# control-toolbox/CTDirect.jl

Measured on AMD Instinct MI355X. Metric: NLP callback evals/s (constraints+sparse Jac), N-step Goddard, 1/2/4/8 GPU, higher is better.
Workload: dtype f64; 1 GPU; cfg2_weak: goddard / gauss_legendre_2, 10000 time steps per GPU (global grid 10000 steps, time-step sharded); fused cons!+jac_coord! on HBM-resident x; BASELINE.json configs[1] per GPU; nvar_per_gpu=110004, ncon_per_gpu=90004, nnzj_per_gpu=1110028

## Files before the change

### ctdirect.jl_amd/csrc/ctd_engine.hip

```cpp
#include <hip/hip_runtime.h>
#include <hip/hiprtc.h>
#include <dlfcn.h>

#include <cstdio>
#include <functional>
#include <map>
#include <mutex>
#include <cstdlib>
#include <cstring>
#include <memory>
#include <new>
#include <string>
#include <vector>

#include "../../include/ctdirect_hip.h"
#include "ctd_host.hpp"
#include "ctd_kernels.hpp"
#include "ctd_hess_kernels.hpp"
#include "ctd_hess_step.hpp"
#include "ctd_iter_kernels.hpp"
#include "ctd_prod_kernels.hpp"
#include "ctd_hprod_kernels.hpp"
#include "ctd_kkt_kernels.hpp"
#include "ctd_jit.hpp"

using namespace ctd;

namespace ctd {
#define CTD_EXTERN_ALL(ID, P) \
    CTD_EXTERN_LAUNCHERS(P) CTD_EXTERN_HESS(P) CTD_EXTERN_HESS_STEP(P) CTD_EXTERN_ITER(P) CTD_EXTERN_PROD(P) CTD_EXTERN_HPROD(P) CTD_EXTERN_KKT(P)
CTD_REGISTRY(CTD_EXTERN_ALL)
}

template <class T = double> struct DevBuf {
    T* p = nullptr;
    int64_t cap = 0;
    DevBuf() = default;
    DevBuf(const DevBuf&) = delete;
    DevBuf& operator=(const DevBuf&) = delete;
    ~DevBuf() { release(); }
    void release() { if (p) (void)hipFree(p); p = nullptr; cap = 0; }
    hipError_t ensure(int64_t n) {
        if (p && n <= cap) return hipSuccess;
        release();
        const hipError_t e = hipMalloc((void**)&p, sizeof(T) * (size_t)(n > 1 ? n : 1));
        if (e == hipSuccess) cap = n; else p = nullptr;
        return e;
    }
    int32_t grow(ctd_handle* h, int64_t need, const char* fn);
};

enum JitFamily { JIT_FIRST, JIT_BATCH, JIT_PROD, JIT_HPROD, JIT_HESS, JIT_PROD_SHARD, JIT_HPROD_SHARD, JIT_KKT, kJitFamilies };
struct JitModule {
    hipModule_t mod = nullptr;
    hipFunction_t f[5] = {};
};

struct ctd_handle {
    Model model;
    int device = -1;
    hipStream_t stream = nullptr;
    bool own_stream = false;
    int64_t step_begin = 0, step_end = 0;
    int tile = 0, block = 256;
    KParams kp;
    size_t lds_bytes = 0;
    int grid = 0;
    DevBuf<double> d_tau;
    DevBuf<uint32_t> d_tmpl, d_vtmpl;
    DevBuf<uint16_t> d_pos;
    DevBuf<int64_t> d_edge_idx;
    DevBuf<uint32_t> d_edge_code;
    DevBuf<> d_x, d_c, d_vals;
    DevBuf<> d_partial;
    DevBuf<> d_obj;
    DevBuf<> d_g;
    DevBuf<> d_gpartial;
    int obj_blocks = 0;
    hipEvent_t ev0 = nullptr, ev1 = nullptr;
    const RtOcp* rt = nullptr;
    JitModule jit[kJitFamilies];
    bool hess_ready = false;
    HParams hp;
    int hess_tile = 0;
    size_t hess_lds_bytes = 0;
    DevBuf<uint32_t> d_htptr, d_hterms, d_hvptr, d_hvterms, d_heptr, d_hevptr, d_heterms;
    DevBuf<int64_t> d_hedge_idx;
    DevBuf<double> d_hpair_c;
    DevBuf<uint32_t> d_hcpos, d_hzpos;
    DevBuf<int32_t> d_hssrc, d_hschunk;
    DevBuf<double> d_hsck;
    bool hess_step = false;
    SParams sp{};
    HParams hp_step{};
    size_t hess_step_lds = 0;
    DevBuf<uint32_t> d_htasks, d_hptasks, d_hbtasks;
    DevBuf<> d_hpartials, d_y, d_hvals;
    DevBuf<XHalo> d_halo;
    XHalo halo_host{};
    DevBuf<> d_stitch_send, d_stitch_recv;
    int64_t hpart_member = 0;
    double out_mb = 0.0;
    DevBuf<> d_ppartial, d_pdir, d_pout;
    DevBuf<> d_hppartial;
    DevBuf<> d_kktpartial, d_kdy, d_ksx, d_ksc, d_krc;
    std::string err;
};

constexpr double kWtMB = 64.0;
constexpr double kHessWtMB = 16.0;

static thread_local std::string g_create_err;

static int32_t fail(ctd_handle* h, int32_t code, const std::string& msg) {
    if (h) h->err = msg; else g_create_err = msg;
    return code;
}

#define HIP_TRY(h, expr)                                                                          \
    do {                                                                                          \
        hipError_t e_ = (expr);                                                                   \
        if (e_ != hipSuccess)                                                                     \
            return fail(h, CTD_EHIP, std::string(#expr) + ": " + hipGetErrorString(e_));          \
    } while (0)

struct DeviceGuard {
    int prev = -1;
    bool switched = false;
    hipError_t err = hipSuccess;
    DeviceGuard() = default;
    explicit DeviceGuard(int dev) { (void)bind(dev); }
    hipError_t bind(int dev) {
        err = hipGetDevice(&prev);
        if (err == hipSuccess && prev != dev) { err = hipSetDevice(dev); switched = (err == hipSuccess); }
        return err;
    }
    ~DeviceGuard() { if (switched) (void)hipSetDevice(prev); }
    DeviceGuard(const DeviceGuard&) = delete;
    DeviceGuard& operator=(const DeviceGuard&) = delete;
};

struct OnDevice {
    DeviceGuard dg;
    int32_t st = CTD_OK;
    explicit OnDevice(ctd_handle* h, const char* fn = nullptr) {
        if (!h) st = CTD_EINVAL;
        else if (h->device < 0)
            st = fail(h, CTD_ENODEVICE, std::string(fn ? fn : "") + (fn ? ": " : "") +
                                            "compute call on a host-only handle (device = -1); there is no CPU fallback");
        else if (dg.bind(h->device) != hipSuccess) st = fail(h, CTD_EHIP, std::string("dg_.err: ") + hipGetErrorString(dg.err));
    }
};

template <class T> int32_t DevBuf<T>::grow(ctd_handle* h, int64_t need, const char* fn) {
    if (need <= cap && p) return CTD_OK;
    hipStreamCaptureStatus cs = hipStreamCaptureStatusNone;
    if (hipStreamIsCapturing(h->stream, &cs) == hipSuccess && cs != hipStreamCaptureStatusNone)
        return fail(h, CTD_EINVAL, std::string(fn) + ": this batch needs larger partial-sum buffers, which cannot be allocated while the "
                                   "stream is capturing; make one call with the same batch size before the capture");
    (void)hipGetLastError();
    HIP_TRY(h, hipStreamSynchronize(h->stream));
    HIP_TRY(h, ensure(need));
    return CTD_OK;
}

template <class T> static hipError_t upload(DevBuf<T>& dst, const std::vector<T>& src) {
    dst.release();
    if (src.empty()) return hipSuccess;
    const hipError_t e = dst.ensure((int64_t)src.size());
    if (e != hipSuccess) return e;
    return hipMemcpy(dst.p, src.data(), src.size() * sizeof(T), hipMemcpyHostToDevice);
}

static int env_int(const char* name, int dflt) {
    const char* s = std::getenv(name);
    return (s && *s) ? std::atoi(s) : dflt;
}

static void destroy_handle(ctd_handle* h) {
    DeviceGuard dg;
    if (h->device >= 0) {
        (void)dg.bind(h->device);
        (void)hipStreamSynchronize(h->stream);
        if (h->ev0) (void)hipEventDestroy(h->ev0);
        if (h->ev1) (void)hipEventDestroy(h->ev1);
        if (h->own_stream && h->stream) (void)hipStreamDestroy(h->stream);
        for (JitModule& m : h->jit)
            if (m.mod) (void)hipModuleUnload(m.mod);
    }
    delete h;
}

namespace {
std::string jit_include_dir() {
    const char* env = std::getenv("CTD_JIT_INCLUDE");
    if (env && *env) return env;
    Dl_info info;
    if (dladdr((const void*)&destroy_handle, &info) && info.dli_fname) {
        std::string path(info.dli_fname);
        const size_t slash = path.find_last_of('/');
        return (slash == std::string::npos ? std::string(".") : path.substr(0, slash)) + "/csrc";
    }
    return "csrc";
}

std::mutex g_jit_mu;
std::map<std::string, std::pair<std::string, std::vector<std::string>>> g_jit_cache;

int32_t jit_compile(const RtOcp& ro, const char* header, const std::vector<std::string>& exprs, const char* fp_contract,
                    std::string& code, std::vector<std::string>& lowered, std::string& err) {
    std::string key = ro.name + "|" + std::to_string((size_t)&ro) + "|" + header;
    for (const std::string& e : exprs) key += "|" + e;
    std::vector<std::string> extra;
    if (const char* ex = std::getenv("CTD_JIT_EXTRA")) {
        std::string cur;
        for (const char* c = ex;; ++c) {
            if (*c == ' ' || *c == 0) { if (!cur.empty()) extra.push_back(cur); cur.clear(); if (*c == 0) break; }
// ... 40 lines not shown
    (void)hiprtcDestroyProgram(&prog);
    std::lock_guard<std::mutex> lk(g_jit_mu);
    g_jit_cache[key] = {code, lowered};
    return CTD_OK;
}

std::vector<std::string> jit_first_exprs(int sc, int s) {
    const std::string P = "ctd::UserOCP", a = std::to_string(sc), b = std::to_string((sc == SC_IRK || sc == SC_MIDPOINT) && s > 0 ? s : 1);
    return {"ctd::cons_jac_kernel<" + P + ", " + a + ", " + b + ", false>", "ctd::obj_partial_kernel<" + P + ", " + a + ">",
            "ctd::obj_finish_kernel<" + P + ">", "ctd::grad_units_kernel<" + P + ", " + a + ", " + b + ">",
            "ctd::grad_finish_kernel<" + P + ">"};
}
std::vector<std::string> jit_hess_exprs(int sc, int s) {
    const std::string P = "ctd::UserOCP", a = std::to_string(sc), b = std::to_string((sc == SC_IRK || sc == SC_MIDPOINT) && s > 0 ? s : 1);
    return {"ctd::hess_kernel<" + P + ", " + a + ", " + b + ", false>", "ctd::hess_finish_kernel<" + P + ">"};
}
std::vector<std::string> jit_batch_exprs(int sc, int s) {
    const std::string b = std::to_string((sc == SC_IRK || sc == SC_MIDPOINT) && s > 0 ? s : 1);
    return {"ctd::cons_jac_batch_kernel<ctd::UserOCP, " + std::to_string(sc) + ", " + b + ">"};
}
std::vector<std::string> prod_exprs(int sc, int s, const std::string& sh) {
    const std::string a = std::to_string(sc), b = std::to_string(sc == SC_IRK && s > 0 ? s : 1);
    return {"ctd::jprod_kernel<ctd::UserOCP, " + a + ", " + b + sh + ">", "ctd::jtprod_units_kernel<ctd::UserOCP, " + a + ", " + b + sh + ">",
            "ctd::jtprod_finish_kernel<ctd::UserOCP" + sh + ">"};
}
std::vector<std::string> hprod_exprs(int sc, int s, const std::string& sh) {
    const std::string a = std::to_string(sc), b = std::to_string(sc == SC_IRK && s > 0 ? s : 1);
    return {"ctd::hprod_units_kernel<ctd::UserOCP, " + a + ", " + b + sh + ">", "ctd::hprod_finish_kernel<ctd::UserOCP" + sh + ">"};
}
std::vector<std::string> jit_kkt_exprs(int sc, int s) {
    const std::string a = std::to_string(sc), b = std::to_string(sc == SC_IRK && s > 0 ? s : 1);
    return {"ctd::kktprod_units_kernel<ctd::UserOCP, " + a + ", " + b + ">", "ctd::kktprod_finish_kernel<ctd::UserOCP>"};
}
std::vector<std::string> jit_prod_exprs(int sc, int s) { return prod_exprs(sc, s, ""); }
std::vector<std::string> jit_hprod_exprs(int sc, int s) { return hprod_exprs(sc, s, ""); }
std::vector<std::string> jit_prod_shard_exprs(int sc, int s) { return prod_exprs(sc, s, ", true"); }
std::vector<std::string> jit_hprod_shard_exprs(int sc, int s) { return hprod_exprs(sc, s, ", true"); }

const struct { const char* header; const char* fp_contract; std::vector<std::string> (*exprs)(int sc, int s); } kJit[kJitFamilies] = {
    {"ctd_kernels.hpp", "off", jit_first_exprs},
    {"ctd_kernels.hpp", "off", jit_batch_exprs},
    {"ctd_prod_kernels.hpp", "off", jit_prod_exprs},
    {"ctd_hprod_kernels.hpp", "off", jit_hprod_exprs},
    {"ctd_hess_kernels.hpp", "fast", jit_hess_exprs},
    {"ctd_prod_kernels.hpp", "off", jit_prod_shard_exprs},
    {"ctd_hprod_kernels.hpp", "off", jit_hprod_shard_exprs},
    {"ctd_kkt_kernels.hpp", "off", jit_kkt_exprs},
};

hipError_t jit_launch(hipFunction_t f, int grid, int block, size_t lds, hipStream_t st, void** args, hipEvent_t e0 = nullptr,
                      hipEvent_t e1 = nullptr, int batch = 1) {
    if (e0 || e1)
        return hipExtModuleLaunchKernel(f, (uint32_t)grid * (uint32_t)block, (uint32_t)batch, 1, (uint32_t)block, 1, 1, lds, st, args, nullptr, e0, e1, 0);
    return hipModuleLaunchKernel(f, (uint32_t)grid, (uint32_t)batch, 1, (uint32_t)block, 1, 1, (uint32_t)lds, st, args, nullptr);
}
}

static int32_t jit_load(ctd_handle* h, JitFamily fam) {
    JitModule& m = h->jit[fam];
    if (!h->rt || m.mod) return CTD_OK;
    ctd_handle* eh = fam == JIT_FIRST ? nullptr : h;
    const Layout& L = h->model.L;
    std::string code, err;
    std::vector<std::string> names;
    const int32_t st = jit_compile(*h->rt, kJit[fam].header, kJit[fam].exprs(L.sc, L.sc == SC_MIDPOINT ? L.cs : L.s), kJit[fam].fp_contract,
                                   code, names, err);
    if (st) return fail(eh, st, err);
    hipError_t e = hipModuleLoadData(&m.mod, code.data());
    for (size_t i = 0; e == hipSuccess && i < names.size(); ++i) e = hipModuleGetFunction(&m.f[i], m.mod, names[i].c_str());
    if (e == hipSuccess) return CTD_OK;
    if (m.mod) (void)hipModuleUnload(m.mod);
    m = JitModule{};
    return fail(eh, CTD_EHIP, std::string(kJit[fam].header) + " module: " + hipGetErrorString(e));
}

template <class T> struct Staged { T* host; DevBuf<>& buf; int64_t n; };

template <class Enqueue>
static int32_t host_call(ctd_handle* h, std::initializer_list<Staged<const double>> in, Enqueue&& enqueue,
                         std::initializer_list<Staged<double>> out) {
    for (const auto& a : in) if (a.host) HIP_TRY(h, a.buf.ensure(a.n));
    for (const auto& a : out) if (a.host) HIP_TRY(h, a.buf.ensure(a.n));
    for (const auto& a : in) if (a.host) HIP_TRY(h, hipMemcpyAsync(a.buf.p, a.host, sizeof(double) * a.n, hipMemcpyHostToDevice, h->stream));
    if (const int32_t st = enqueue()) return st;
    for (const auto& a : out) if (a.host) HIP_TRY(h, hipMemcpyAsync(a.host, a.buf.p, sizeof(double) * a.n, hipMemcpyDeviceToHost, h->stream));
    HIP_TRY(h, hipStreamSynchronize(h->stream));
    return CTD_OK;
}

template <class K>
static int32_t enqueue_prod_units(ctd_handle* h, const char* fn, typename K::Params& a, int dirs, int jc, DevBuf<>& partial,
                                  const JitModule& jm, int f0, const double* x_dev, bool shard) {
    ProdParams& pp = K::prod(a);
    pp.nch = (int32_t)((dirs + jc - 1) / jc);
    const int64_t blocks = ((pp.unit_end - pp.unit_begin) * (int64_t)pp.nch + 255) / 256;
    if (blocks > 0x7fffffff) return fail(h, CTD_EINVAL, std::string(fn) + ": grid too large");
    pp.nblocks = (int32_t)blocks;
    const int32_t st = partial.grow(h, blocks * kMaxNV, fn);
    if (st) return st;
    pp.partial = partial.p;
    hipError_t e = hipErrorInvalidValue;
    if (h->rt) {
        void* args[] = {&a, &x_dev};
        e = jit_launch(jm.f[f0], (int)blocks, 256, 0, h->stream, args);
        if (e == hipSuccess) e = jit_launch(jm.f[f0 + 1], 1, 64, 0, h->stream, args);
    }
    for_problem(h->model.problem, [&](auto tag) {
        using P = typename decltype(tag)::type;
        if constexpr (K::kShardForm)
            e = shard ? launch_prod_units<P, K, true>(a, x_dev, h->stream) : launch_prod_units<P, K, false>(a, x_dev, h->stream);
        else e = launch_prod_units<P, K, false>(a, x_dev, h->stream);
    });
    if (e != hipSuccess) return fail(h, CTD_EHIP, std::string(fn) + ": kernel launch: " + hipGetErrorString(e));
    return CTD_OK;
}

extern "C" {

const char* ctd_strerror(int32_t st) {
    switch (st) {
        case CTD_OK: return "ok";
        case CTD_EINVAL: return "invalid argument";
        case CTD_EGRID: return "given time grid is not strictly increasing";
        case CTD_ESCHEME: return "unknown discretization method";
        case CTD_EPATTERN: return "sparsity pattern not available";
        case CTD_EPROBLEM: return "problem not in the compiled registry";
        case CTD_ENODEVICE: return "no HIP device bound to this handle (there is no CPU fallback)";
        case CTD_EHIP: return "HIP runtime error";
        case CTD_ENOMEM: return "out of memory";
        default: return "unknown status";
    }
}

const char* ctd_last_error(const ctd_handle* h) { return h ? h->err.c_str() : g_create_err.c_str(); }

int32_t ctd_create(const ctd_desc* desc, ctd_handle** out) {
    if (!desc || !out) return fail(nullptr, CTD_EINVAL, "ctd_create: null argument");
    *out = nullptr;
    struct Del { void operator()(ctd_handle* p) const { if (p) destroy_handle(p); } };
    std::unique_ptr<ctd_handle, Del> h(new (std::nothrow) ctd_handle());
    if (!h) return fail(nullptr, CTD_ENOMEM, "ctd_create: out of memory");
    HostDesc hd{desc->problem, desc->scheme, desc->pattern_mode, desc->grid_size, desc->time_grid, desc->time_grid_len,
                desc->control_steps > 1 ? desc->control_steps : 1, desc->value_order};
    if (desc->reserved0 != 0) return fail(nullptr, CTD_EINVAL, "ctd_create: ctd_desc.reserved0 must be 0 (zero-initialise the descriptor: memset / ctd_desc d = {0})");
    std::string err;
    int st;
    try {
        st = build_model(hd, h->model, err);
    } catch (const std::bad_alloc&) {
        return fail(nullptr, CTD_ENOMEM, "ctd_create: out of memory while building the model");
    }
    if (st) return fail(nullptr, st, err);
    const Model& mo = h->model;
    if (mo.L.cs > 3 && desc->device >= 0 && !runtime_ocp(mo.problem))
        return fail(nullptr, CTD_EINVAL, "ctd_create: control_steps > 3 needs an OCP registered at run time (ctd_register_ocp); the compiled registry holds the midpoint kernels for 1, 2 and 3 controls per step");
    h->step_begin = desc->step_begin;
    h->step_end = desc->step_end;
    if (h->step_begin == 0 && h->step_end == 0) h->step_end = mo.L.N;
    if (h->step_begin < 0 || h->step_end > mo.L.N || h->step_begin >= h->step_end)
        return fail(nullptr, CTD_EINVAL, "ctd_create: shard [step_begin, step_end) is not inside [0, N)");
    h->tile = env_int("CTD_TILE", 0);
    if (h->tile <= 0) h->tile = default_tile(mo, h->step_end - h->step_begin);
    int maxb = 256;
    for_problem(mo.problem, [&](auto tag) { maxb = decltype(tag)::type::MAXB; });
    h->rt = runtime_ocp(mo.problem);
    if (h->rt) maxb = h->rt->maxb;
    h->block = env_int("CTD_BLOCK", 0);
    if (h->block <= 0) {
        h->block = 256;
        const int64_t ntl = (h->step_end - h->step_begin + h->tile - 1) / h->tile;
        if (ntl <= 512 && mo.nch_dyn <= 1 && mo.Lseg > 0 && 320 / mo.Lseg > 256 / mo.Lseg && mo.Lseg * (320 / mo.Lseg) * 10 >= 320 * 9) h->block = 320;
    }
    if (h->block < 64 || (h->block % 64)) h->block = 256;
    if (h->block > maxb) h->block = maxb;
    mo.fill_kparams(h->kp, h->step_begin, h->step_end, h->tile);
    h->lds_bytes = (size_t)lds_doubles(h->kp) * sizeof(double);
    const int debug_stop = env_int("CTD_DEBUG_STOP", 0);
    const size_t lds_cap = h->rt ? 64 * 1024 : 80 * 1024;
    while (h->lds_bytes > lds_cap && h->tile > 1) {
        h->tile = (h->tile + 1) / 2;
        mo.fill_kparams(h->kp, h->step_begin, h->step_end, h->tile);
        h->lds_bytes = (size_t)lds_doubles(h->kp) * sizeof(double);
    }
    const bool long_mid = mo.L.sc == SC_MIDPOINT && mo.L.cs == 1;
    if (desc->device >= 0 && !h->rt && env_int("CTD_TILE", 0) <= 0 && mo.nch_dyn <= 1 && (mo.L.sc == SC_IRK || long_mid) && h->tile >= 16) {
        DeviceGuard dgq(desc->device);
        if (dgq.err == hipSuccess) {
            auto resident = [&](int tile, size_t& lds) {
                KParams kq;
                mo.fill_kparams(kq, h->step_begin, h->step_end, tile);
                lds = (size_t)lds_doubles(kq) * sizeof(double);
                int r = 0;
                for_problem(mo.problem, [&](auto tag) { r = occupancy_cons_jac<typename decltype(tag)::type>(kq, h->block, lds); });
                (void)hipGetLastError();
                return r;
            };
            size_t l0 = 0;
            const int r0 = resident(h->tile, l0);
            const int64_t ns = h->step_end - h->step_begin, cap = 256 * (int64_t)r0;
            if (r0 > 0 && (ns + h->tile - 1) / h->tile >= env_int("CTD_LONG_GRID_ROUNDS", 8) * cap && maxb >= 512 && env_int("CTD_BLOCK", 0) <= 0 &&
                env_int("CTD_LONG_GRID", 1)) {
                int tbest = h->tile;
                for (int tt = h->tile + 1; tt <= 256; ++tt) {
                    KParams kq;
                    mo.fill_kparams(kq, h->step_begin, h->step_end, tt);
                    if ((size_t)lds_doubles(kq) * sizeof(double) > (long_mid ? 74u : 64u) * 1024) break;
                    tbest = tt;
                }
                if (tbest > h->tile) {
                    h->tile = tbest;
                    h->block = 512;
                    mo.fill_kparams(h->kp, h->step_begin, h->step_end, h->tile);
                    h->lds_bytes = (size_t)lds_doubles(h->kp) * sizeof(double);
                }
            } else if (mo.L.sc == SC_IRK && r0 > 0 && (ns + h->tile - 1) / h->tile > cap) {
                int tmax = 48;
                for (; tmax > h->tile; --tmax) { size_t l = 0; if (resident(tmax, l) >= r0 && l <= lds_cap) break; }
                const int64_t rounds = (ns + (int64_t)tmax * cap - 1) / ((int64_t)tmax * cap);
                const int64_t tb = (ns + rounds * cap - 1) / (rounds * cap);
                if (tb > h->tile && tb <= tmax) {
                    h->tile = (int)tb;
                    mo.fill_kparams(h->kp, h->step_begin, h->step_end, h->tile);
                    h->lds_bytes = (size_t)lds_doubles(h->kp) * sizeof(double);
                }
            }
        }
    }
    h->grid = h->kp.ntiles + h->kp.has_edge;
    h->kp.debug_stop = debug_stop;
    h->out_mb = 8.0 * ((double)(h->step_end - h->step_begin) * (mo.L.cb + mo.Lseg + (double)mo.L.nv * mo.vr)) / 1.0e6;
    h->kp.wt_store = h->out_mb <= kWtMB ? 1 : 0;
    h->device = desc->device;
    if (h->device >= 0) {
        int ndev = 0;
        if (hipGetDeviceCount(&ndev) != hipSuccess || h->device >= ndev)
            return fail(nullptr, CTD_ENODEVICE, "ctd_create: HIP device not available");
        ctd_handle* hp = h.get();
        if (h->lds_bytes > 160 * 1024) return fail(nullptr, CTD_EINVAL, "ctd_create: tile does not fit the 160 KiB LDS");
        DeviceGuard dg_(hp->device); HIP_TRY(nullptr, dg_.err);
        if (desc->stream_mode == CTD_STREAM_GIVEN) { hp->stream = (hipStream_t)desc->stream; hp->own_stream = false; }
        else { HIP_TRY(nullptr, hipStreamCreateWithFlags(&hp->stream, hipStreamNonBlocking)); hp->own_stream = true; }
        HIP_TRY(nullptr, upload(hp->d_tau, mo.tau));
        HIP_TRY(nullptr, upload(hp->d_tmpl, mo.tmpl));
        HIP_TRY(nullptr, upload(hp->d_vtmpl, mo.vtmpl));
        HIP_TRY(nullptr, upload(hp->d_edge_idx, mo.edge_idx));
        HIP_TRY(nullptr, upload(hp->d_edge_code, mo.edge_code));
        hp->kp.tau = hp->d_tau.p;
        hp->kp.tmpl = hp->d_tmpl.p;
        hp->kp.vtmpl = hp->d_vtmpl.p;
        {
            const int S = mo.L.s, r_dyn = S * mo.nch_dyn, r_path = mo.nch_path;
            int lgT = 0;
            while ((1 << lgT) < hp->tile) ++lgT;
            const int leadbase = (((r_dyn + r_path) << lgT) + 63) & ~63;
            const int early_lanes = mo.n_early + mo.c_early + mo.L.nv * mo.vr_early;
            if (env_int("CTD_EARLY", 0) && mo.n_early > 0 && !hp->rt && mo.fused && hp->tile <= 32 && leadbase + 64 <= hp->block && early_lanes <= 64 &&
                mo.n_late > 0 && mo.n_late <= hp->block) {
                HIP_TRY(nullptr, upload(hp->d_pos, mo.pos_order));
                hp->kp.pos = hp->d_pos.p;
                hp->kp.n_late = mo.n_late; hp->kp.n_early = mo.n_early; hp->kp.c_early = mo.c_early; hp->kp.vr_early = mo.vr_early;
                hp->kp.div_late = make_fastdiv((uint32_t)mo.n_late);
            }
        }
        hp->kp.edge_idx = hp->d_edge_idx.p;
        hp->kp.edge_code = hp->d_edge_code.p;
        hp->obj_blocks = 256;
        HIP_TRY(nullptr, hp->d_partial.ensure(hp->obj_blocks));
        HIP_TRY(nullptr, hp->d_obj.ensure(1));
        HIP_TRY(nullptr, hipEventCreate(&hp->ev0));
        HIP_TRY(nullptr, hipEventCreate(&hp->ev1));
        if (hp->rt) {
            if (hp->lds_bytes > 64 * 1024) return fail(nullptr, CTD_EINVAL, "ctd_create: one step of this run-time OCP does not fit 64 KiB of LDS");
            const int32_t jst = jit_load(hp, JIT_FIRST);
            if (jst) return jst;
        }
        {
            const bool direct = mo.fused && mo.L.sc != SC_TRAPEZE;
            const int mt = env_int("CTD_MULTI_TILE", 0);
            if (!direct && mt > 0 && kMultiTileLoop && !hp->rt) {
                int per_cu = mt > 1 ? mt : 0, cus = 256;
                if (hipDeviceGetAttribute(&cus, hipDeviceAttributeMultiprocessorCount, hp->device) != hipSuccess) cus = 256;
                if (per_cu == 0) {
                    if (hp->rt) {
                        if (hipModuleOccupancyMaxActiveBlocksPerMultiprocessor(&per_cu, hp->jit[JIT_FIRST].f[0], hp->block, hp->lds_bytes) != hipSuccess) per_cu = 0;
                    } else {
                        for_problem(mo.problem, [&](auto tag) {
                            using P = typename decltype(tag)::type;
                            per_cu = occupancy_cons_jac<P>(hp->kp, hp->block, hp->lds_bytes);
                        });
                    }
                }
                const int64_t cap = (int64_t)per_cu * cus - hp->kp.has_edge;
                if (cap > 0 && hp->kp.ntiles > cap) {
                    hp->kp.wg_stride = (int)cap;
                    hp->grid = hp->kp.wg_stride + hp->kp.has_edge;
                }
            }
        }
    }
    *out = h.release();
    return CTD_OK;
}

int32_t ctd_register_ocp(const ctd_ocp_def* def, int32_t* problem_id) {
    if (!def || !problem_id) return fail(nullptr, CTD_EINVAL, "ctd_register_ocp: null argument");
    std::string err;
    int id = -1;
    const int st = register_runtime_ocp(def, &id, err);
    if (st) return fail(nullptr, st, "ctd_register_ocp: " + err);
    *problem_id = id;
    return CTD_OK;
}

int32_t ctd_ocp_source(int32_t problem_id, char* buf, int64_t cap) {
// ... 236 lines not shown
}
}

int32_t ctd_shard_steps(int64_t N, int32_t n_shards, int32_t k, int64_t* begin, int64_t* end) {
    if (N < 1 || n_shards < 1 || n_shards > N || k < 0 || k >= n_shards || !begin || !end) return CTD_EINVAL;
    *begin = shard_begin(N, n_shards, k);
    *end = k + 1 == n_shards ? N : shard_begin(N, n_shards, k + 1);
    return CTD_OK;
}

int32_t ctd_stitch_c(ctd_handle* h, void* nccl_comm, int32_t n_ranks, int32_t rank, double* c_dev) {
    if (!h) return CTD_EINVAL;
    if (h->device < 0) return fail(h, CTD_ENODEVICE, "host-only handle");
    if (!nccl_comm || !c_dev || n_ranks < 1 || rank < 0 || rank >= n_ranks) return fail(h, CTD_EINVAL, "ctd_stitch_c: bad argument");
    const Layout& L = h->model.L;
    const int64_t N = L.N;
    const int G = n_ranks;
    if (G > N || h->step_begin != shard_begin(N, G, rank) || h->step_end != (rank + 1 == G ? N : shard_begin(N, G, rank + 1)))
        return fail(h, CTD_EINVAL, "ctd_stitch_c: the handle's shard is not block `rank` of the balanced split of the grid over n_ranks (ctd_shard_steps)");
    nccl_resolve();
    if (!g_nccl_allgather) return fail(h, CTD_ERCCL, "ctd_stitch_c: librccl (ncclAllGather) not found in this process; set CTD_RCCL_LIB");
    DeviceGuard dg_(h->device); HIP_TRY(h, dg_.err);
    const int64_t tail = L.ncon - N * L.cb;
    auto check = [&](int rc, const char* what) -> int32_t {
        if (rc == 0) return CTD_OK;
        return fail(h, CTD_ERCCL, std::string(what) + ": " + (g_nccl_errstr ? g_nccl_errstr(rc) : "RCCL error ") + " (" + std::to_string(rc) + ")");
    };
    constexpr int kNcclDouble = 8;
    if (N % G == 0 && tail == 0) {
        const int64_t S = (N / G) * L.cb;
        return check(g_nccl_allgather(c_dev + rank * S, c_dev, (size_t)S, kNcclDouble, nccl_comm, h->stream), "ncclAllGather");
    }
    const int64_t smax = ((N + G - 1) / G) * L.cb + tail;
    if (h->d_stitch_recv.cap < (int64_t)G * smax) {
        h->d_stitch_send.release();
        h->d_stitch_recv.release();
        HIP_TRY(h, h->d_stitch_send.ensure(smax));
        HIP_TRY(h, h->d_stitch_recv.ensure((int64_t)G * smax));
        HIP_TRY(h, hipMemsetAsync(h->d_stitch_send.p, 0, sizeof(double) * smax, h->stream));
    }
    const int64_t own = (h->step_end - h->step_begin) * L.cb, mytail = rank + 1 == G ? tail : 0;
    const int64_t np = own + mytail;
    stitch_pack_kernel<<<(unsigned)((np + 255) / 256), 256, 0, h->stream>>>(c_dev, h->d_stitch_send.p, h->step_begin * L.cb, own, N * L.cb, mytail);
    HIP_TRY(h, hipGetLastError());
    const int32_t st = check(g_nccl_allgather(h->d_stitch_send.p, h->d_stitch_recv.p, (size_t)smax, kNcclDouble, nccl_comm, h->stream), "ncclAllGather");
    if (st) return st;
    stitch_unpack_kernel<<<(unsigned)((L.ncon + 255) / 256), 256, 0, h->stream>>>(h->d_stitch_recv.p, c_dev, L.ncon, N, L.cb, G, smax);
    HIP_TRY(h, hipGetLastError());
    return CTD_OK;
}

int32_t ctd_ipc_export(int32_t device, const void* dev_ptr, void* handle64, int64_t* offset) {
    if (!dev_ptr || !handle64 || !offset) return CTD_EINVAL;
    static_assert(sizeof(hipIpcMemHandle_t) == 64, "CTD_IPC_HANDLE_BYTES");
    DeviceGuard dg(device);
    hipError_t e = dg.err;
    hipDeviceptr_t base = nullptr;
    size_t size = 0;
    if (e == hipSuccess) e = hipMemGetAddressRange(&base, &size, (hipDeviceptr_t)dev_ptr);
    hipIpcMemHandle_t hd;
    if (e == hipSuccess) e = hipIpcGetMemHandle(&hd, (void*)base);
    if (e != hipSuccess) { g_create_err = std::string("ctd_ipc_export: ") + hipGetErrorString(e); (void)hipGetLastError(); return CTD_EHIP; }
    std::memcpy(handle64, &hd, sizeof(hd));
    *offset = (int64_t)((const char*)dev_ptr - (const char*)base);
    return CTD_OK;
}
int32_t ctd_ipc_open(int32_t device, const void* handle64, void** base) {
    if (!handle64 || !base) return CTD_EINVAL;
    *base = nullptr;
    DeviceGuard dg(device);
    hipError_t e = dg.err;
    hipIpcMemHandle_t hd;
    std::memcpy(&hd, handle64, sizeof(hd));
    if (e == hipSuccess) e = hipIpcOpenMemHandle(base, hd, hipIpcMemLazyEnablePeerAccess);
    if (e != hipSuccess) { g_create_err = std::string("ctd_ipc_open: ") + hipGetErrorString(e); (void)hipGetLastError(); return CTD_ERCCL; }
    return CTD_OK;
}
int32_t ctd_ipc_probe(int32_t device, const void* ptr, size_t bytes) {
    if (!ptr || bytes == 0 || bytes > 64) return CTD_EINVAL;
    DeviceGuard dg(device);
    hipError_t e = dg.err;
    void* tmp = nullptr;
    if (e == hipSuccess) e = hipMalloc(&tmp, 64);
    if (e == hipSuccess) e = hipMemcpy(tmp, ptr, bytes, hipMemcpyDeviceToDevice);
    if (e == hipSuccess) e = hipDeviceSynchronize();
    if (tmp) (void)hipFree(tmp);
    if (e != hipSuccess) { g_create_err = std::string("ctd_ipc_probe: ") + hipGetErrorString(e); (void)hipGetLastError(); return CTD_ERCCL; }
    return CTD_OK;
}
int32_t ctd_ipc_close(int32_t device, void* base) {
    if (!base) return CTD_OK;
    DeviceGuard dg(device);
    return (dg.err == hipSuccess && hipIpcCloseMemHandle(base) == hipSuccess) ? CTD_OK : CTD_EHIP;
}

int32_t ctd_launch_info(const ctd_handle* h, int64_t* o) {
    if (!h || !o) return CTD_EINVAL;
    o[0] = h->grid; o[1] = h->block; o[2] = (int64_t)h->lds_bytes; o[3] = h->tile; o[4] = h->model.Lseg;
    o[5] = (int64_t)h->model.edge_idx.size();
    o[6] = (h->model.fused && h->model.L.sc != SC_TRAPEZE) ? 1 : 0;
    o[7] = 0;
    if (h->device >= 0) {
        DeviceGuard dg(h->device);
        int per_cu = 0;
        if (dg.err == hipSuccess) {
            if (h->rt) { if (hipModuleOccupancyMaxActiveBlocksPerMultiprocessor(&per_cu, h->jit[JIT_FIRST].f[0], h->block, h->lds_bytes) != hipSuccess) per_cu = 0; }
            else for_problem(h->model.problem, [&](auto tag) {
                using P = typename decltype(tag)::type;
                per_cu = occupancy_cons_jac<P>(h->kp, h->block, h->lds_bytes);
            });
        }
        (void)hipGetLastError();
        o[7] = per_cu;
    }
    return CTD_OK;
}


struct Batch {
    int32_t n;
    int64_t ldx, ldy, ldc, ldv, ldg, ldh;
};

static int32_t enqueue_cons_jac(ctd_handle* h, const double* x_dev, double* c_dev, double* vals_dev, hipEvent_t te0 = nullptr,
                                hipEvent_t te1 = nullptr, const Batch* bt = nullptr) {
    const OnDevice on(h);
    if (on.st) return on.st;
    if (!x_dev) return fail(h, CTD_EINVAL, "x is null");
    KParams kp = h->kp;
    kp.c = c_dev;
    kp.vals = vals_dev;
    hipError_t e = hipErrorInvalidValue;
    if (bt) {
        BatchLd bl{bt->ldx, bt->ldc, bt->ldv};
        kp.wt_store = h->out_mb * bt->n <= kWtMB ? 1 : 0;
        if (h->rt) {
            if (const int32_t jst = jit_load(h, JIT_BATCH)) return jst;
            void* args[] = {&kp, &x_dev, &bl};
            e = jit_launch(h->jit[JIT_BATCH].f[0], h->grid, h->block, h->lds_bytes, h->stream, args, nullptr, nullptr, bt->n);
        }
        for_problem(h->model.problem, [&](auto tag) {
            using P = typename decltype(tag)::type;
            e = launch_cons_jac_batch<P>(kp, x_dev, bl, h->grid, h->block, h->lds_bytes, h->stream, bt->n);
        });
        if (e != hipSuccess) return fail(h, CTD_EHIP, std::string("kernel launch: ") + hipGetErrorString(e));
        return CTD_OK;
    }
    if (h->rt) {
        void* args[] = {&kp, &x_dev};
        e = jit_launch(h->jit[JIT_FIRST].f[0], h->grid, h->block, h->lds_bytes, h->stream, args, te0, te1);
    }
    for_problem(h->model.problem, [&](auto tag) {
        using P = typename decltype(tag)::type;
        e = launch_cons_jac<P>(kp, x_dev, h->grid, h->block, h->lds_bytes, h->stream, te0, te1);
    });
    if (e != hipSuccess) return fail(h, CTD_EHIP, std::string("kernel launch: ") + hipGetErrorString(e));
    return CTD_OK;
}

int32_t ctd_cons_jac_dev_async(ctd_handle* h, const double* x_dev, double* c_dev, double* vals_dev) {
    return enqueue_cons_jac(h, x_dev, c_dev, vals_dev);
}

int32_t ctd_set_stream(ctd_handle* h, void* stream) {
    if (!h) return CTD_EINVAL;
    if (h->device < 0) return fail(h, CTD_ENODEVICE, "host-only handle");
    if (h->own_stream && h->stream) { (void)hipStreamSynchronize(h->stream); (void)hipStreamDestroy(h->stream); }
    h->stream = (hipStream_t)stream;
    h->own_stream = false;
    return CTD_OK;
}

int32_t ctd_sync(ctd_handle* h) {
    if (!h) return CTD_EINVAL;
    if (h->device < 0) return fail(h, CTD_ENODEVICE, "host-only handle");
    HIP_TRY(h, hipStreamSynchronize(h->stream));
    return CTD_OK;
}

int32_t ctd_cons_jac_dev(ctd_handle* h, const double* x_dev, double* c_dev, double* vals_dev) {
    int32_t st = enqueue_cons_jac(h, x_dev, c_dev, vals_dev);
    if (st) return st;
    return ctd_sync(h);
}

static int32_t host_cons_jac(ctd_handle* h, const double* x, double* c, double* vals) {
    const OnDevice on(h);
    if (on.st) return on.st;
    if (!x) return fail(h, CTD_EINVAL, "x is null");
    const Model& mo = h->model;
    return host_call(h, {{x, h->d_x, mo.L.nvar}},
                     [&] { return enqueue_cons_jac(h, h->d_x.p, c ? h->d_c.p : nullptr, vals ? h->d_vals.p : nullptr); },
                     {{c, h->d_c, mo.L.ncon}, {vals, h->d_vals, mo.nnzj}});
}

int32_t ctd_host_alloc(void** ptr, size_t bytes) {
    if (!ptr) return CTD_EINVAL;
    *ptr = nullptr;
    const hipError_t e = hipHostMalloc(ptr, bytes ? bytes : 8, hipHostMallocDefault);
    if (e != hipSuccess) { g_create_err = std::string("ctd_host_alloc: ") + hipGetErrorString(e); return CTD_EHIP; }
    return CTD_OK;
}
int32_t ctd_host_free(void* ptr) {
    if (!ptr) return CTD_OK;
    return hipHostFree(ptr) == hipSuccess ? CTD_OK : CTD_EHIP;
}

int32_t ctd_cons(ctd_handle* h, const double* x, double* c) {
    if (h && !c) return fail(h, CTD_EINVAL, "c is null");
    return host_cons_jac(h, x, c, nullptr);
}
int32_t ctd_jac_coord(ctd_handle* h, const double* x, double* vals) {
    if (h && !vals) return fail(h, CTD_EINVAL, "vals is null");
    return host_cons_jac(h, x, nullptr, vals);
}
int32_t ctd_cons_jac(ctd_handle* h, const double* x, double* c, double* vals) {
    if (h && (!c || !vals)) return fail(h, CTD_EINVAL, "c or vals is null");
    return host_cons_jac(h, x, c, vals);
}

static int fill_obj_params(ctd_handle* h, double* f_dev, ObjParams& op);

static int32_t enqueue_obj(ctd_handle* h, const double* x_dev, double* f_dev, const Batch* bt = nullptr) {
    const OnDevice on(h);
    if (on.st) return on.st;
    if (!x_dev || !f_dev) return fail(h, CTD_EINVAL, "null argument");
    const Layout& L = h->model.L;
    ObjParams op;
    const int blocks = fill_obj_params(h, f_dev, op);
    const bool lagrange = h->model.info.lagrange;
    const int nb = bt ? bt->n : 1;
    if (bt) {
        const int32_t st = h->d_partial.grow(h, (int64_t)nb * (blocks > 0 ? blocks : 1), "ctd_obj_batch_dev_async");
        if (st) return st;
        op.partial = h->d_partial.p;
        op.ldx = bt->ldx;
    }
    hipError_t e = hipErrorInvalidValue;
    if (h->rt) {
        void* args[] = {&op, &x_dev};
        e = lagrange ? jit_launch(h->jit[JIT_FIRST].f[1], blocks, 256, 0, h->stream, args, nullptr, nullptr, nb) : hipSuccess;
        if (e == hipSuccess) e = jit_launch(h->jit[JIT_FIRST].f[2], 1, 64, 0, h->stream, args, nullptr, nullptr, nb);
    }
    for_problem(h->model.problem, [&](auto tag) {
        using P = typename decltype(tag)::type;
        e = launch_obj<P>(op, x_dev, lagrange ? blocks : 0, 256, h->stream, nb);
    });
    if (e != hipSuccess) return fail(h, CTD_EHIP, std::string("kernel launch: ") + hipGetErrorString(e));
    return CTD_OK;
}

static int fill_obj_params(ctd_handle* h, double* f_dev, ObjParams& op) {
    const Layout& L = h->model.L;
    std::memset(&op, 0, sizeof(op));
    op.L = L;
    op.tau = h->d_tau.p;
    const bool last = h->step_end == L.N;
    op.unit_begin = h->step_begin;
    op.unit_end = (L.sc == SC_TRAPEZE && last) ? L.N + 1 : h->step_end;
    op.add_mayer = last ? 1 : 0;
    op.partial = h->d_partial.p;
    op.out = f_dev;
    op.halo = h->kp.halo;
    op.near = h->kp.near;
    const int64_t units = op.unit_end - op.unit_begin;
    int blocks = (int)((units + 255) / 256);
    if (blocks > h->obj_blocks) blocks = h->obj_blocks;
    if (blocks < 1) blocks = 1;
    const bool lagrange = h->model.info.lagrange;
    op.nblocks = lagrange ? blocks : 0;
    return lagrange ? blocks : 0;
}

int32_t ctd_obj_dev_async(ctd_handle* h, const double* x_dev, double* f_dev) { return enqueue_obj(h, x_dev, f_dev); }

int32_t ctd_obj_dev(ctd_handle* h, const double* x_dev, double* f_host) {
    if (h && !f_host) return fail(h, CTD_EINVAL, "null argument");
    const OnDevice on(h);
    if (on.st) return on.st;
    return host_call(h, {}, [&] { return enqueue_obj(h, x_dev, h->d_obj.p); }, {{f_host, h->d_obj, 1}});
}

static int32_t enqueue_grad(ctd_handle* h, const double* x_dev, double* g_dev, GradParams* only_params = nullptr, bool shard = false,
                            const Batch* bt = nullptr);
int32_t ctd_grad_dev_async(ctd_handle* h, const double* x_dev, double* g_dev) { return enqueue_grad(h, x_dev, g_dev); }
int32_t ctd_grad_shard_dev_async(ctd_handle* h, const double* x_dev, double* g_dev) { return enqueue_grad(h, x_dev, g_dev, nullptr, true); }
int32_t ctd_grad_dev(ctd_handle* h, const double* x_dev, double* g_dev) {
    int32_t st = enqueue_grad(h, x_dev, g_dev);
    if (st) return st;
    HIP_TRY(h, hipStreamSynchronize(h->stream));
    return CTD_OK;
}

__global__ void zero_rows_kernel(double* __restrict__ p, int64_t ld, int64_t len) {
    double* row = p + (int64_t)blockIdx.y * ld;
    for (int64_t e = (int64_t)blockIdx.x * blockDim.x + threadIdx.x; e < len; e += (int64_t)gridDim.x * blockDim.x) row[e] = 0.0;
}

static int32_t enqueue_grad(ctd_handle* h, const double* x_dev, double* g_dev, GradParams* only_params, bool shard, const Batch* bt) {
    const OnDevice on(h);
    if (on.st) return on.st;
    if (!x_dev || !g_dev) return fail(h, CTD_EINVAL, "null argument");
    const Layout& L = h->model.L;
    const bool last = h->step_end == L.N, first = h->step_begin == 0;
    const int64_t all_units = (L.sc == SC_IRK) ? L.N : L.N + 1;
    const int64_t ub = shard ? h->step_begin : 0, ue = shard ? ((L.sc != SC_IRK && last) ? L.N + 1 : h->step_end) : all_units;
    const int64_t units = ue - ub;
// ... 945 lines not shown
```

### ctdirect.jl_amd/csrc/ctd_kernel_body.hpp

```cpp
#pragma once
#include "ctd_layout.hpp"


namespace ctd {

#if defined(CTD_SUBSTAMPS) && defined(__HIP_DEVICE_COMPILE__)
#ifndef CTD_SUB_WAVE0
#define CTD_SUB_WAVE0 0
#endif
#define CTD_SUB(kp, id)                                                                                              \
    do {                                                                                                             \
        __builtin_amdgcn_sched_barrier(0);                                                                           \
        __builtin_amdgcn_s_waitcnt(0);                                                                               \
        if ((kp).stamps && (threadIdx.x & 63) == 0 && threadIdx.x >= 64 * CTD_SUB_WAVE0 && threadIdx.x < 64 * CTD_SUB_WAVE0 + 128) \
            (kp).stamps[(size_t)gridDim.x * 12 + ((size_t)blockIdx.x * 2 + (threadIdx.x >> 6) - CTD_SUB_WAVE0) * 8 + (id)] = clock64(); \
        __builtin_amdgcn_sched_barrier(0);                                                                           \
    } while (0)
#else
#define CTD_SUB(kp, id) do { } while (0)
#endif
#if defined(CTD_SUBSTAMPS_EMIT) && defined(__HIP_DEVICE_COMPILE__)
#define CTD_SUBE(kp, id)                                                                                             \
    do {                                                                                                             \
        __builtin_amdgcn_sched_barrier(0);                                                                           \
        if ((kp).stamps && (threadIdx.x & 63) == 0 && threadIdx.x < 128)                                             \
            (kp).stamps[(size_t)gridDim.x * 12 + ((size_t)blockIdx.x * 2 + (threadIdx.x >> 6)) * 8 + (id)] = clock64(); \
        __builtin_amdgcn_sched_barrier(0);                                                                           \
    } while (0)
#else
#define CTD_SUBE(kp, id) do { } while (0)
#endif

struct BlockCtx {
    int is_edge;
    int edge_part;
    int direct;
    int nslots;
    int in_stride;
    int64_t a, b;
    int64_t lo;
    double* in;
    double* v;
    double* tau;
    double* rec;
    const uint32_t* codes;
    const uint32_t* vcodes;
    const XHalo* halo;
    const double* xu;
};

CTD_HD const XHalo* block_halo(const KParams& kp, const BlockCtx& cx) {
    if (!kp.halo) return nullptr;
    if (cx.is_edge) return kp.halo;
    return (cx.lo < kp.step_begin || cx.b + kp.HH >= kp.step_end) ? kp.halo : nullptr;
}

constexpr int kMaxStagedCodes = 1024;
CTD_HD bool codes_staged(const KParams& kp) { return kp.stage_codes != 0; }
inline int wgs_per_cu(int64_t lds_bytes) {
    const int64_t g = (lds_bytes + 1279) / 1280 * 1280;
    return g > 0 ? (int)((160 * 1024) / g) : 32;
}
CTD_HD int code_doubles(const KParams& kp) { return codes_staged(kp) ? (kp.Lseg + kp.L.nv * kp.vr + 1) / 2 : 0; }

CTD_HD int64_t slot_index(const KParams& kp, const BlockCtx& cx, int k) {
    return cx.is_edge ? kp.edge_steps[k] : cx.lo + k;
}

CTD_HD BlockCtx make_ctx(const KParams& kp, int block, double* lds) {
    BlockCtx cx;
    cx.direct = 0;
    const Layout& L = kp.L;
    cx.codes = codes_staged(kp) ? reinterpret_cast<const uint32_t*>(lds) : kp.tmpl;
    cx.vcodes = codes_staged(kp) ? cx.codes + kp.Lseg : kp.vtmpl;
    lds += code_doubles(kp);
    cx.edge_part = 0;
    if (block < kp.has_edge) {
        cx.is_edge = 1;
        cx.edge_part = block;
        cx.nslots = kp.n_edge_slots;
        cx.in_stride = edge_in_stride(L);
        cx.a = cx.b = cx.lo = 0;
        cx.in = lds;
        cx.v = cx.in + cx.nslots * cx.in_stride;
        cx.tau = cx.v + kMaxNV;
        cx.rec = cx.tau + 2 * kMaxEdgeSlots + 2;
    } else {
        const int tile = block - kp.has_edge;
        const int cap = kp.T + kp.HL + kp.HH;
        cx.is_edge = 0;
        cx.a = kp.step_begin + (int64_t)tile * kp.T;
        cx.b = cx.a + kp.T < kp.step_end ? cx.a + kp.T : kp.step_end;
        cx.lo = cx.a - kp.HL;
        cx.nslots = (int)(cx.b - cx.a) + kp.HL + kp.HH;
        cx.in_stride = tile_in_stride(L);
        cx.in = lds;
        cx.v = cx.in + (cap + 1) * tile_in_stride(L) + L.n + L.m;
        cx.tau = cx.v + kMaxNV;
        cx.rec = cx.tau + cap + 2;
    }
    cx.xu = nullptr;
    cx.halo = block_halo(kp, cx);
    return cx;
}

CTD_HD BlockCtx make_direct_ctx(const KParams& kp, int block, double* lds, const double* xu) {
    BlockCtx cx;
    const Layout& L = kp.L;
    cx.direct = 1;
    cx.codes = kp.tmpl;
    cx.vcodes = kp.vtmpl;
    cx.in_stride = L.blk;
    cx.v = const_cast<double*>(xu) + L.v_off;
    cx.tau = nullptr;
    cx.rec = lds + code_doubles(kp);
    cx.xu = xu;
    cx.halo = nullptr;
    cx.edge_part = 0;
    if (block < kp.has_edge) {
        cx.is_edge = 1;
        cx.edge_part = block;
        cx.nslots = kp.n_edge_slots;
        cx.a = cx.b = cx.lo = 0;
        cx.in = const_cast<double*>(xu);
        cx.halo = kp.halo;
        return cx;
    }
    const int tile = block - kp.has_edge;
    cx.is_edge = 0;
    cx.a = kp.step_begin + (int64_t)tile * kp.T;
    cx.b = cx.a + kp.T < kp.step_end ? cx.a + kp.T : kp.step_end;
    cx.lo = cx.a - kp.HL;
    cx.nslots = (int)(cx.b - cx.a) + kp.HL + kp.HH;
    cx.in = const_cast<double*>(xu) + cx.lo * (int64_t)L.blk;
    cx.halo = block_halo(kp, cx);
    return cx;
}

CTD_HD const double* slot_base(const KParams& kp, const BlockCtx& cx, int k) {
    if (cx.direct && cx.halo) {
        const int64_t g = slot_index(kp, cx, k) * (int64_t)cx.in_stride;
        return xnear(kp.near, cx.xu, g) + g;
    }
    if (cx.direct && cx.is_edge) return cx.in + kp.edge_steps[k] * (int64_t)cx.in_stride;
    return cx.in + k * cx.in_stride;
}
CTD_HD const double* slot_next(const KParams& kp, const BlockCtx& cx, int k) {
    if (cx.direct && cx.halo) {
        const int64_t g = (slot_index(kp, cx, k) + 1) * (int64_t)cx.in_stride;
        return xnear(kp.near, cx.xu, g) + g;
    }
    return slot_base(kp, cx, k) + ((cx.direct || cx.is_edge) ? kp.L.blk : cx.in_stride);
}
CTD_HD const double* slot_prev(const KParams& kp, const BlockCtx& cx, int k) {
    if (cx.direct && cx.halo) {
        const int64_t g = (slot_index(kp, cx, k) - 1) * (int64_t)cx.in_stride;
        return xnear(kp.near, cx.xu, g) + g;
    }
    return slot_base(kp, cx, k) - ((cx.direct || cx.is_edge) ? kp.L.blk : cx.in_stride);
}

inline int64_t lds_doubles(const KParams& kp) {
    const Layout& L = kp.L;
    const int64_t cap = kp.T + kp.HL + kp.HH;
    int64_t tile = code_doubles(kp) + (cap + 1) * tile_in_stride(L) + L.n + L.m + kMaxNV + cap + 2 + cap * kp.R.stride;
    int64_t edge = code_doubles(kp) + (int64_t)kp.n_edge_slots * edge_in_stride(L) + kMaxNV + 2 * kMaxEdgeSlots + 2 +
                   (int64_t)(kp.n_edge_slots + 1) * kp.R.stride + kp.R.bsize;
    return tile > edge ? tile : edge;
}

CTD_HD double tau_global(const KParams& kp, int64_t i) {
    if (i < 0) i = 0;
    if (i > kp.L.N) i = kp.L.N;
    return kp.tau ? kp.tau[i] : (double)i / (double)kp.L.N;
}
CTD_HD double slot_tau(const KParams& kp, const BlockCtx& cx, int k, int d) {
    if (cx.direct) return tau_global(kp, slot_index(kp, cx, k) + d);
    return cx.is_edge ? cx.tau[2 * k + d] : cx.tau[k + d];
}
CTD_HD double final_tau(const KParams& kp, const BlockCtx& cx) {
    return cx.direct ? tau_global(kp, kp.L.N) : cx.tau[2 * cx.nslots];
}

template <class P> CTD_HD double time_of(const KParams& kp, const double* v, double tau) {
    const double t0 = (P::IT0 >= 0) ? v[P::IT0 >= 0 ? P::IT0 : 0] : kp.L.t0;
    const double tf = (P::ITF >= 0) ? v[P::ITF >= 0 ? P::ITF : 0] : kp.L.tf;
    return t0 + tau * (tf - t0);
}
template <class P> CTD_HD double dtime_of(double tau, int k) {
    const double dt0 = (P::IT0 == k) ? 1.0 : 0.0;
    const double dtf = (P::ITF == k) ? 1.0 : 0.0;
    return dt0 + tau * (dtf - dt0);
}

template <class P> struct DynNZ {
    static constexpr bool sparse = false;
    static constexpr int nF = -1, nG = -1;
    CTD_HD static constexpr int fx(int, int) { return -1; }
    CTD_HD static constexpr int gu(int, int) { return -1; }
};
template <class P, int SC, int S> struct RL {
    static constexpr int cb = (SC == SC_IRK ? P::NX * (1 + S) : P::NX) + P::NPATH;
    static constexpr RecLayout R = make_rec_layout(P::NX, P::NU, P::NV, P::NPATH, P::NBC, SC == SC_IRK ? S : 0, cb,
                                                   SC == SC_MIDPOINT ? P::NU * S : P::NU, DynNZ<P>::nF, DynNZ<P>::nG);
    CTD_HD static constexpr int F(int r, int c) {
        if (DynNZ<P>::sparse) { const int s = DynNZ<P>::fx(r, c); return s < 0 ? -1 : R.oF + s; }
        return R.oF + r * R.ldx + c;
    }
    CTD_HD static constexpr int G(int r, int c, int jb = 0) {
        if (DynNZ<P>::sparse) { const int s = DynNZ<P>::gu(r, c); return s < 0 ? -1 : R.oG + jb * DynNZ<P>::nG + s; }
        return R.oG + r * R.ldg + jb * P::NU + c;
    }
};
template <int SC, int S> struct StagePoints { static constexpr int value = SC == SC_IRK ? S : 1; };

template <class P> struct Dirs {
    static constexpr int DYN = P::NX + P::NU + (P::DYN_T ? 1 : 0) + (P::DYN_V ? P::NV : 0);
    static constexpr int PATH = P::NX + P::NU + (P::PATH_T ? 1 : 0) + (P::PATH_V ? P::NV : 0);
    static constexpr int BND = 2 * P::NX + P::NV;
    static constexpr int DC = P::DC;
    static constexpr int NCH_DYN = (DYN + DC - 1) / DC;
    static constexpr int NCH_PATH = (PATH + DC - 1) / DC;
    static constexpr int NCH_BND = (BND + DC - 1) / DC;
    static constexpr bool FUSED = (NCH_DYN == 1) && (P::NPATH == 0 || NCH_PATH == 1);
    static constexpr bool FREE = (P::IT0 >= 0) || (P::ITF >= 0);
};

template <class P, int SC> struct DirectTile { static constexpr bool value = Dirs<P>::FUSED && SC != SC_TRAPEZE; };

CTD_HD void load_codes(const KParams& kp, const BlockCtx& cx, int tid, int nthr) {
    if (!codes_staged(kp)) return;
    uint32_t* dst = const_cast<uint32_t*>(cx.codes);
    for (int e = tid; e < kp.Lseg; e += nthr) dst[e] = kp.tmpl[e];
    const int nvc = kp.L.nv * kp.vr;
    for (int e = tid; e < nvc; e += nthr) dst[kp.Lseg + e] = kp.vtmpl[e];
}

template <class P, int SC, int S, bool LOAD_V = true>
CTD_HD void phase_load(const KParams& kp, const BlockCtx& cx, const double* __restrict__ xu, int tid, int nthr) {
    const Layout& L = kp.L;
    if (cx.is_edge) {
        const int per = cx.in_stride;
        for (int e = tid; e < cx.nslots * per; e += nthr) {
            const int k = e / per, o = e - k * per;
            int64_t g = kp.edge_steps[k] * L.blk + o;
            if (o >= L.blk + L.n + L.m)
                g = (kp.edge_steps[k] >= 1 ? kp.edge_steps[k] - 1 : 0) * (int64_t)L.blk + L.n + (o - (L.blk + L.n + L.m));
            cx.in[e] = (g < L.v_off) ? (cx.halo ? xnear(kp.near, xu, g) : xu)[g] : 0.0;
        }
        for (int e = tid; e <= 2 * cx.nslots; e += nthr)
            cx.tau[e] = (e == 2 * cx.nslots) ? tau_global(kp, L.N) : tau_global(kp, kp.edge_steps[e >> 1] + (e & 1));
    } else {
        const int64_t g0 = (cx.lo < 0 ? 0 : cx.lo) * (int64_t)L.blk;
        int64_t g1 = (cx.lo + cx.nslots) * (int64_t)L.blk + L.n + L.m;
        if (g1 > L.v_off) g1 = L.v_off;
        const double* __restrict__ src = xu + g0;
        const int cnt = (int)(g1 - g0);
        const int eo0 = (int)(g0 - cx.lo * (int64_t)L.blk), padw = cx.in_stride - L.blk;
        auto at = [&](int e) -> double& { const int eo = eo0 + e; return cx.in[eo + (int)fast_div((uint32_t)eo, kp.div_blk) * padw]; };
        const bool codes = LOAD_V && codes_staged(kp);
        const int nvc = kp.L.nv * kp.vr;
        if (cx.halo) {
            for (int e = tid; e < cnt; e += nthr) at(e) = xnear(kp.near, xu, g0 + e)[g0 + e];
            if (LOAD_V && tid < kMaxNV) cx.v[tid] = (tid < P::NV) ? xu[L.v_off + tid] : 0.0;
            if (codes) {
                uint32_t* cd = const_cast<uint32_t*>(cx.codes);
                for (int e = tid; e < kp.Lseg; e += nthr) cd[e] = kp.tmpl[e];
                for (int e = tid; e < nvc; e += nthr) cd[kp.Lseg + e] = kp.vtmpl[e];
            }
            for (int e = tid; e <= cx.nslots + 1; e += nthr) cx.tau[e] = tau_global(kp, cx.lo + e);
            return;
        }
        const double x0 = tid < cnt ? src[tid] : 0.0;
        const double x1 = tid + nthr < cnt ? src[tid + nthr] : 0.0;
        const double vv = (LOAD_V && tid < P::NV) ? xu[L.v_off + tid] : 0.0;
        const uint32_t c0 = (codes && tid < kp.Lseg) ? kp.tmpl[tid] : 0u;
        const uint32_t c1 = (codes && tid < nvc) ? kp.vtmpl[tid] : 0u;
        const double tau_e = tid <= cx.nslots + 1 ? tau_global(kp, cx.lo + tid) : 0.0;
        if (tid < cnt) at(tid) = x0;
        if (tid + nthr < cnt) at(tid + nthr) = x1;
        if (LOAD_V && tid < kMaxNV) cx.v[tid] = vv;
        if (codes) {
            uint32_t* cd = const_cast<uint32_t*>(cx.codes);
            if (tid < kp.Lseg) cd[tid] = c0;
            if (tid < nvc) cd[kp.Lseg + tid] = c1;
            for (int e = tid + nthr; e < kp.Lseg; e += nthr) cd[e] = kp.tmpl[e];
            for (int e = tid + nthr; e < nvc; e += nthr) cd[kp.Lseg + e] = kp.vtmpl[e];
        }
        for (int e = tid + 2 * nthr; e < cnt; e += nthr) at(e) = src[e];
        if (tid <= cx.nslots + 1) cx.tau[tid] = tau_e;
        for (int e = tid + nthr; e <= cx.nslots + 1; e += nthr) cx.tau[e] = tau_global(kp, cx.lo + e);
        return;
    }
    if (LOAD_V && tid < kMaxNV) cx.v[tid] = (tid < P::NV) ? xu[L.v_off + tid] : 0.0;
}

struct TileIn { double x0, x1, tau; };
template <class P>
CTD_HD TileIn load_issue(const KParams& kp, const BlockCtx& cx, const double* __restrict__ xu, int tid, int nthr) {
    TileIn t{0.0, 0.0, 0.0};
    if (cx.halo) return t;
    const Layout& L = kp.L;
    const int64_t g0 = (cx.lo < 0 ? 0 : cx.lo) * (int64_t)L.blk;
    int64_t g1 = (cx.lo + cx.nslots) * (int64_t)L.blk + L.n + L.m;
    if (g1 > L.v_off) g1 = L.v_off;
    const double* __restrict__ src = xu + g0;
    const int cnt = (int)(g1 - g0);
    if (tid < cnt) t.x0 = src[tid];
    if (tid + nthr < cnt) t.x1 = src[tid + nthr];
    if (tid <= cx.nslots + 1) t.tau = tau_global(kp, cx.lo + tid);
    return t;
}
template <class P, int SC, int S>
CTD_HD void load_commit(const KParams& kp, const BlockCtx& cx, const double* __restrict__ xu, const TileIn& t, int tid, int nthr) {
    if (cx.halo) { phase_load<P, SC, S, false>(kp, cx, xu, tid, nthr); return; }
    const Layout& L = kp.L;
    const int64_t g0 = (cx.lo < 0 ? 0 : cx.lo) * (int64_t)L.blk;
    int64_t g1 = (cx.lo + cx.nslots) * (int64_t)L.blk + L.n + L.m;
    if (g1 > L.v_off) g1 = L.v_off;
    const double* __restrict__ src = xu + g0;
    const int cnt = (int)(g1 - g0);
    const int eo0 = (int)(g0 - cx.lo * (int64_t)L.blk), padw = cx.in_stride - L.blk;
    auto at = [&](int e) -> double& { const int eo = eo0 + e; return cx.in[eo + (int)fast_div((uint32_t)eo, kp.div_blk) * padw]; };
    if (tid < cnt) at(tid) = t.x0;
    if (tid + nthr < cnt) at(tid + nthr) = t.x1;
    for (int e = tid + 2 * nthr; e < cnt; e += nthr) at(e) = src[e];
    if (tid <= cx.nslots + 1) cx.tau[tid] = t.tau;
    for (int e = tid + nthr; e <= cx.nslots + 1; e += nthr) cx.tau[e] = tau_global(kp, cx.lo + e);
}

template <class P> CTD_HD void fill_const_coefs(const KParams& kp, double* C) {
#pragma unroll
    for (int e = 0; e < kNC; ++e) C[e] = 0.0;
    C[C_ONE] = 1.0; C[C_NEG1] = -1.0;
#pragma unroll
    for (int j = 0; j < 3; ++j) C[C_B + j] = kp.L.b[j];
}

template <class P, int SC, int S>
CTD_HD void fin_lead(const KParams& kp, const BlockCtx& cx, int k, int row = -1) {
    constexpr int n = P::NX, nv = P::NV;
    const Layout& L = kp.L;
    constexpr RecLayout R = RL<P, SC, S>::R;
    const int64_t i = slot_index(kp, cx, k);
    double* rec = cx.rec + k * R.stride;
    double* C = rec + R.oC;
    if (row <= 0) fill_const_coefs<P>(kp, C);
    if (i < 0 || i >= L.N) return;
    const double tau0 = slot_tau(kp, cx, k, 0), tau1 = slot_tau(kp, cx, k, 1);
    const double h = time_of<P>(kp, cx.v, tau1) - time_of<P>(kp, cx.v, tau0);
    if (SC == SC_IRK) {
        const double* base = slot_base(kp, cx, k);
        const double* nxt = slot_next(kp, cx, k);
        const double* K = base + n + L.cu;
        if (row <= 0) {
#pragma unroll
            for (int j = 0; j < S; ++j) {
#pragma unroll
                for (int l = 0; l < S; ++l) C[C_HA + 3 * j + l] = -(h * L.a[3 * j + l]);
                C[C_HB + j] = -(h * L.b[j]);
            }
        }
        if (row >= 0) {
            const int r = row;
            double sumbk = L.b[0] * K[r];
#pragma unroll
            for (int j = 1; j < S; ++j) sumbk = sumbk + L.b[j] * K[j * n + r];
            rec[R.oR + r] = nxt[r] - (base[r] + h * sumbk);
#pragma unroll
            for (int kk = 0; kk < nv; ++kk) {
                const double dh = Dirs<P>::FREE ? dtime_of<P>(tau1, kk) - dtime_of<P>(tau0, kk) : 0.0;
                rec[R.oSv + r * nv + kk] = -(dh * sumbk);
            }
            return;
        }
#pragma unroll
        for (int r = 0; r < n; ++r) {
            double sumbk = L.b[0] * K[r];
#pragma unroll
            for (int j = 1; j < S; ++j) sumbk = sumbk + L.b[j] * K[j * n + r];
            rec[R.oR + r] = nxt[r] - (base[r] + h * sumbk);
#pragma unroll
            for (int kk = 0; kk < nv; ++kk) {
                const double dh = Dirs<P>::FREE ? dtime_of<P>(tau1, kk) - dtime_of<P>(tau0, kk) : 0.0;
                rec[R.oSv + r * nv + kk] = -(dh * sumbk);
            }
        }
    } else if (SC == SC_MIDPOINT) {
        C[C_NHH] = -(0.5 * (h / (double)S));
        C[C_NH] = -(h / (double)S);
    } else {
        C[C_NHH] = -(0.5 * h);
    }
}

template <class P, int SC, int S>
CTD_HD void fin_stage(const KParams& kp, const BlockCtx& cx, int k, int j, double* ev, int r0 = 0, int rstep = 1) {
    constexpr int n = P::NX, nv = P::NV;
    auto mine = [&](int r) { return rstep == 1 || (r % rstep) == r0; };
    constexpr bool FREE = Dirs<P>::FREE;
    const Layout& L = kp.L;
    constexpr RecLayout R = RL<P, SC, S>::R;
    const int64_t i = slot_index(kp, cx, k);
    if (i < 0) return;
    if (SC == SC_TRAPEZE ? (i > L.N) : (i >= L.N)) return;
    double* rec = cx.rec + k * R.stride;
    const double* base = slot_base(kp, cx, k);
    const double tau0 = slot_tau(kp, cx, k, 0), tau1 = slot_tau(kp, cx, k, 1);
    double dti[nv > 0 ? nv : 1], dh[nv > 0 ? nv : 1];
#pragma unroll
    for (int kk = 0; kk < nv; ++kk) {
        dti[kk] = FREE ? dtime_of<P>(tau0, kk) : 0.0;
        dh[kk] = FREE ? dtime_of<P>(tau1, kk) - dti[kk] : 0.0;
    }
    if (SC == SC_IRK) {
        const double* K = base + n + L.cu;
#pragma unroll
        for (int r = 0; r < n; ++r)
            if (mine(r)) rec[R.oR + n + j * n + r] = K[j * n + r] - ev[R.of + r];
#pragma unroll
        for (int kk = 0; kk < nv; ++kk) {
            double dx[n > 0 ? n : 1];
#pragma unroll
            for (int c = 0; c < n; ++c) {
                double acc = 0.0;
#pragma unroll
                for (int l = 0; l < S; ++l) acc = acc + (dh[kk] * butcher_a<S>(L, j, l)) * K[l * n + c];
                dx[c] = acc;
            }
            const double dtij = dti[kk] + butcher_c<S>(L, j) * dh[kk];
#pragma unroll
            for (int r = 0; r < n; ++r) {
                if (!mine(r)) continue;
                double w = P::DYN_V ? ev[R.oW + r * nv + kk] : 0.0;
                if (P::DYN_T && FREE) w = w + ev[R.oft + r] * dtij;
                if (FREE) {
#pragma unroll
                    for (int c = 0; c < n; ++c)
                        if (RL<P, SC, S>::F(r, c) >= 0) w = w + ev[RL<P, SC, S>::F(r, c)] * dx[c];
                }
                ev[R.oW + r * nv + kk] = w;
            }
        }
    } else if (SC == SC_MIDPOINT) {
        const double h = (time_of<P>(kp, cx.v, tau1) - time_of<P>(kp, cx.v, tau0)) / (double)S;
        const double* nxt = slot_next(kp, cx, k);
#pragma unroll
        for (int r = 0; r < n; ++r) {
            if (!mine(r)) continue;
            const double f = ev[R.of + r];
            rec[R.oR + r] = nxt[r] - (base[r] + h * f);
#pragma unroll
            for (int kk = 0; kk < nv; ++kk) {
                double w = P::DYN_V ? ev[R.oW + r * nv + kk] : 0.0;
                if (P::DYN_T && FREE)
                    w = w + ev[R.oft + r] * (L.euler == 0 ? 0.5 * (dti[kk] + (dti[kk] + dh[kk])) : (L.euler == 1 ? dti[kk] : dti[kk] + dh[kk]));
                ev[R.oW + r * nv + kk] = w;
                rec[R.oSv + r * nv + kk] = -((S > 1 ? dh[kk] / (double)S : dh[kk]) * f + h * w);
            }
        }
    } else {
#pragma unroll
        for (int r = 0; r < n; ++r)
#pragma unroll
            for (int kk = 0; kk < nv; ++kk) {
                if (!mine(r)) continue;
                double w = P::DYN_V ? ev[R.oW + r * nv + kk] : 0.0;
                if (P::DYN_T && FREE) w = w + ev[R.oft + r] * dti[kk];
                ev[R.oW + r * nv + kk] = w;
            }
    }
}

template <class P, int S>
CTD_HD void fin_stage_row(const KParams& kp, const BlockCtx& cx, int k, int j, int r) {
    constexpr int n = P::NX, nv = P::NV;
    constexpr bool FREE = Dirs<P>::FREE;
    constexpr RecLayout R = RL<P, SC_IRK, S>::R;
    const Layout& L = kp.L;
    const int64_t i = slot_index(kp, cx, k);
    if (i < 0 || i >= L.N) return;
    double* rec = cx.rec + k * R.stride;
    double* ev = rec + R.oEval + j * R.eval_sz;
    const double* K = slot_base(kp, cx, k) + n + L.cu;
    const double tau0 = slot_tau(kp, cx, k, 0), tau1 = slot_tau(kp, cx, k, 1);
    rec[R.oR + n + j * n + r] = K[j * n + r] - ev[R.of + r];
#pragma unroll
    for (int kk = 0; kk < nv; ++kk) {
        const double dti = FREE ? dtime_of<P>(tau0, kk) : 0.0;
        const double dh = FREE ? dtime_of<P>(tau1, kk) - dti : 0.0;
        double w = P::DYN_V ? ev[R.oW + r * nv + kk] : 0.0;
        if (P::DYN_T && FREE) w = w + ev[R.oft + r] * (dti + butcher_c<S>(L, j) * dh);
        if (FREE) {
#pragma unroll
            for (int c = 0; c < n; ++c) {
                double acc = 0.0;
#pragma unroll
                for (int l = 0; l < S; ++l) acc = acc + (dh * butcher_a<S>(L, j, l)) * K[l * n + c];
                const int sl = RL<P, SC_IRK, S>::F(r, c);
                if (sl >= 0) w = w + ev[sl] * acc;
            }
        }
        ev[R.oW + r * nv + kk] = w;
    }
}

template <class P, int SC, int S>
CTD_HD void fin_path(const KParams& kp, double* rec, double tau) {
    constexpr int nv = P::NV, np = P::NPATH;
    constexpr RecLayout R = RL<P, SC, S>::R;
#pragma unroll
    for (int r = 0; r < np; ++r)
#pragma unroll
        for (int kk = 0; kk < nv; ++kk) {
            double pv = P::PATH_V ? rec[R.oPv + r * nv + kk] : 0.0;
            if (P::PATH_T && Dirs<P>::FREE) pv = pv + rec[R.oPt + r] * dtime_of<P>(tau, kk);
            rec[R.oPv + r * nv + kk] = pv;
        }
}

template <class P>
CTD_HD void fin_trapeze_step(const KParams& kp, const BlockCtx& cx, int k) {
    constexpr int n = P::NX, nv = P::NV;
    const Layout& L = kp.L;
    constexpr RecLayout R = RL<P, SC_TRAPEZE, 1>::R;
    const int64_t i = slot_index(kp, cx, k);
    if (i < 0 || i >= L.N || k + 1 >= cx.nslots) return;
    if (slot_index(kp, cx, k + 1) != i + 1) return;
    double* rec = cx.rec + k * R.stride;
    const double* nxt = rec + R.stride;
    const double* base = slot_base(kp, cx, k);
    const double* xnext = slot_next(kp, cx, k);
    const double tau0 = slot_tau(kp, cx, k, 0), tau1 = slot_tau(kp, cx, k, 1);
    const double half_h = 0.5 * (time_of<P>(kp, cx.v, tau1) - time_of<P>(kp, cx.v, tau0));
    const double* e0 = rec + R.oEval;
    const double* e1 = nxt + R.oEval;
#pragma unroll
    for (int r = 0; r < n; ++r) {
        const double fs = e0[R.of + r] + e1[R.of + r];
        rec[R.oR + r] = xnext[r] - (base[r] + half_h * fs);
#pragma unroll
        for (int kk = 0; kk < nv; ++kk) {
            const double dhalf = Dirs<P>::FREE ? 0.5 * (dtime_of<P>(tau1, kk) - dtime_of<P>(tau0, kk)) : 0.0;
            rec[R.oSv + r * nv + kk] = -(dhalf * fs + half_h * (e0[R.oW + r * nv + kk] + e1[R.oW + r * nv + kk]));
        }
    }
}

template <class P, int S> CTD_HD void node_control(const KParams& kp, const double* base, double* u) {
    const Layout& L = kp.L;
    if (L.stagewise) {
#pragma unroll
        for (int c = 0; c < P::NU; ++c) u[c] = L.b[0] * base[P::NX + c];
#pragma unroll
        for (int j = 1; j < S; ++j)
#pragma unroll
            for (int c = 0; c < P::NU; ++c) u[c] = u[c] + L.b[j] * base[P::NX + j * P::NU + c];
    } else {
#pragma unroll
        for (int c = 0; c < P::NU; ++c) u[c] = base[P::NX + c];
    }
}

template <class P, int S> CTD_HD void path_control(const KParams& kp, const BlockCtx& cx, int k, int64_t i, double* u) {
    const Layout& L = kp.L;
    const double* base = slot_base(kp, cx, k);
    if (L.euler == 2 && i >= 1 && (cx.is_edge || k >= 1)) {
        const double* up = (cx.is_edge && !cx.direct) ? base + L.blk + P::NX + P::NU : slot_prev(kp, cx, k) + P::NX;
#pragma unroll
        for (int c = 0; c < P::NU; ++c) u[c] = up[c];
    } else {
        node_control<P, S>(kp, base, u);
    }
}

template <class P> struct SymDyn {
    static constexpr bool value = P::HAS_SYM_DYN;
    static constexpr int parts = P::DYN_PARTS;
    CTD_HD static void eval(const double* p, double* ev) { if constexpr (P::HAS_SYM_DYN) P::dyn_sym(p, ev); }
    CTD_HD static void eval_part(int q, const double* p, double* ev) {
        if constexpr (P::HAS_SYM_DYN && P::DYN_PARTS > 1) P::dyn_sym_part(q, p, ev);
        else eval(p, ev);
    }
};
template <class P> struct SymPath {
    static constexpr bool value = P::HAS_SYM_PATH;
    CTD_HD static void eval(const double* p, double* px, double* val) { if constexpr (P::HAS_SYM_PATH) P::path_sym(p, px, val); }
};
template <class P> struct SymLag {
    static constexpr bool value = P::HAS_SYM_LAG;
    CTD_HD static void eval(const double* p, double* out) { if constexpr (P::HAS_SYM_LAG) P::lag_sym(p, out); }
};
template <class P> struct SymStage;
template <class P> struct SymPathH { static constexpr bool value = false; CTD_HD static void eval(const double*, double*) {} };

template <class P, class RLT, bool SPLIT>
CTD_HD void eval_point(const KParams& kp, const double* vv, int q, double t, const double* xv, const double* uv, double* ev) {
    constexpr int n = P::NX, m = P::NU, nv = P::NV, DC = P::DC;
    using D = Dual<DC>;
    constexpr RecLayout R = RLT::R;
    struct { const double* v; } cx{vv};
    if constexpr (SymDyn<P>::value) {
        constexpr bool split = SPLIT && SymDyn<P>::parts > 1 && SymDyn<P>::parts == Dirs<P>::NCH_DYN;
        if (!split && q != 0) return;
        CTD_SUB(kp, 6);
        double prm[1 + n + m + nv];
        prm[0] = t;
#pragma unroll
        for (int c = 0; c < n; ++c) prm[1 + c] = xv[c];
#pragma unroll
        for (int c = 0; c < m; ++c) prm[1 + n + c] = uv[c];
#pragma unroll
        for (int c = 0; c < nv; ++c) prm[1 + n + m + c] = cx.v[c];
        if constexpr (split) SymDyn<P>::eval_part(q, prm, ev);
        else SymDyn<P>::eval(prm, ev);
        return;
    }
    D X[n > 0 ? n : 1], U[m > 0 ? m : 1], V[nv > 0 ? nv : 1], Tt, out[n > 0 ? n : 1];
    const int g0 = q * DC;
    constexpr int gT = n + m, gV = n + m + (P::DYN_T ? 1 : 0);
#pragma unroll
    for (int c = 0; c < n; ++c) {
        X[c].v = xv[c];
#pragma unroll
        for (int d = 0; d < DC; ++d) X[c].d[d] = (g0 + d == c) ? 1.0 : 0.0;
    }
#pragma unroll
    for (int c = 0; c < m; ++c) {
        U[c].v = uv[c];
#pragma unroll
        for (int d = 0; d < DC; ++d) U[c].d[d] = (g0 + d == n + c) ? 1.0 : 0.0;
    }
    Tt.v = t;
#pragma unroll
    for (int d = 0; d < DC; ++d) Tt.d[d] = (P::DYN_T && g0 + d == gT) ? 1.0 : 0.0;
#pragma unroll
    for (int c = 0; c < nv; ++c) {
        V[c].v = cx.v[c];
#pragma unroll
        for (int d = 0; d < DC; ++d) V[c].d[d] = (P::DYN_V && g0 + d == gV + c) ? 1.0 : 0.0;
    }
    P::template dynamics<D>(out, Tt, X, U, V);
#pragma unroll
    for (int d = 0; d < DC; ++d) {
        const int g = g0 + d;
        if (g < n) {
#pragma unroll
            for (int r = 0; r < n; ++r) ev[R.oF + r * R.ldx + g] = out[r].d[d];
        } else if (g < n + m) {
#pragma unroll
            for (int r = 0; r < n; ++r) ev[R.oG + r * R.ldg + (g - n)] = out[r].d[d];
        } else if (P::DYN_T && g == n + m) {
#pragma unroll
            for (int r = 0; r < n; ++r) ev[R.oft + r] = out[r].d[d];
        } else if (P::DYN_V && g < Dirs<P>::DYN) {
            const int kk = g - n - m - (P::DYN_T ? 1 : 0);
#pragma unroll
            for (int r = 0; r < n; ++r) ev[R.oW + r * nv + kk] = out[r].d[d];
        }
    }
    if (q == 0) {
#pragma unroll
        for (int r = 0; r < n; ++r) ev[R.of + r] = out[r].v;
    }
}

template <class P, int SC, int S, bool SPLIT = false>
CTD_HD void eval_dynamics(const KParams& kp, const BlockCtx& cx, int k, int j, int q, double* ev) {
    constexpr int n = P::NX, m = P::NU, nv = P::NV;
    const Layout& L = kp.L;
    constexpr RecLayout R = RL<P, SC, S>::R;
    const int64_t i = slot_index(kp, cx, k);
    if (i < 0) return;
    if (SC == SC_TRAPEZE ? (i > L.N) : (i >= L.N)) return;
    const double* base = slot_base(kp, cx, k);
    const double ti = time_of<P>(kp, cx.v, slot_tau(kp, cx, k, 0));
    double xv[n > 0 ? n : 1], uv[m > 0 ? m : 1];
    double t;
    if (SC == SC_TRAPEZE) {
        t = ti;
#pragma unroll
        for (int c = 0; c < n; ++c) xv[c] = base[c];
#pragma unroll
        for (int c = 0; c < m; ++c) uv[c] = base[n + c];
    } else if (SC == SC_MIDPOINT) {
        const double tip1 = time_of<P>(kp, cx.v, slot_tau(kp, cx, k, 1));
        const double* nxt = slot_next(kp, cx, k);
        if (L.euler == 0) {
            t = 0.5 * (ti + tip1);
#pragma unroll
            for (int c = 0; c < n; ++c) xv[c] = 0.5 * (base[c] + nxt[c]);
        } else {
            t = (L.euler == 1) ? ti : tip1;
#pragma unroll
            for (int c = 0; c < n; ++c) xv[c] = (L.euler == 1) ? base[c] : nxt[c];
        }
#pragma unroll
        for (int c = 0; c < m; ++c) uv[c] = base[n + c];
    } else {
        const double h = time_of<P>(kp, cx.v, slot_tau(kp, cx, k, 1)) - ti;
        t = ti + butcher_c<S>(L, j) * h;
        const double* K = base + n + L.cu;
#pragma unroll
        for (int c = 0; c < n; ++c) {
            double x = base[c];
#pragma unroll
            for (int l = 0; l < S; ++l) x = x + h * butcher_a<S>(L, j, l) * K[l * n + c];
            xv[c] = x;
        }
        const double* U = base + n + (L.stagewise ? j * m : 0);
#pragma unroll
        for (int c = 0; c < m; ++c) uv[c] = U[c];
    }
    if constexpr (SC == SC_MIDPOINT && S > 1) {
        using RL1 = RL<P, SC_MIDPOINT, 1>;
        constexpr RecLayout R1 = RL1::R;
        constexpr int DC = P::DC, NP = Dirs<P>::NCH_DYN;
        constexpr bool sym = SymDyn<P>::value;
        constexpr bool symsplit = sym && SPLIT && SymDyn<P>::parts > 1 && SymDyn<P>::parts == NP;
        constexpr int gT = n + m, gV = n + m + (P::DYN_T ? 1 : 0);
        if (sym && !symsplit && q != 0) return;
        auto dir = [&](int g) { return sym || (g >= q * DC && g < (q + 1) * DC); };
        for (int jj = 0; jj < S; ++jj) {
            double tmp[R1.eval_sz];
#pragma unroll
            for (int e = 0; e < R1.eval_sz; ++e) tmp[e] = 0.0;
#pragma unroll
            for (int c = 0; c < m; ++c) uv[c] = base[n + jj * m + c];
            eval_point<P, RL1, SPLIT>(kp, cx.v, q, t, xv, uv, tmp);
#pragma unroll
            for (int r = 0; r < n; ++r) {
                if (symsplit && (r % NP) != q) continue;
#pragma unroll
                for (int c = 0; c < n; ++c)
                        if (dir(c) && RL1::F(r, c) >= 0)
                        ev[RL<P, SC, S>::F(r, c)] = (jj == 0 ? 0.0 : ev[RL<P, SC, S>::F(r, c)]) + tmp[RL1::F(r, c)];
#pragma unroll
                for (int c = 0; c < m; ++c)
                    if (dir(n + c) && RL1::G(r, c) >= 0) ev[RL<P, SC, S>::G(r, c, jj)] = tmp[RL1::G(r, c)];
                if (P::DYN_T && dir(gT)) ev[R.oft + r] = (jj == 0 ? 0.0 : ev[R.oft + r]) + tmp[R1.oft + r];
                if (P::DYN_V) {
#pragma unroll
                    for (int kk = 0; kk < nv; ++kk)
                        if (dir(gV + kk)) ev[R.oW + r * nv + kk] = (jj == 0 ? 0.0 : ev[R.oW + r * nv + kk]) + tmp[R1.oW + r * nv + kk];
                }
                if (sym || q == 0) ev[R.of + r] = (jj == 0 ? 0.0 : ev[R.of + r]) + tmp[R1.of + r];
            }
        }
        return;
    }
    eval_point<P, RL<P, SC, S>, SPLIT>(kp, cx.v, q, t, xv, uv, ev);
}

template <class P, int SC, int S>
CTD_HD void eval_path(const KParams& kp, double* rec, double t, const double* xv, const double* uv, const double* vv, int q,
                      int value_off) {
    constexpr int n = P::NX, m = P::NU, nv = P::NV, np = P::NPATH, DC = P::DC;
    using D = Dual<DC>;
    constexpr RecLayout R = RL<P, SC, S>::R;
    if constexpr (SymPath<P>::value) {
        if (q != 0) return;
        double prm[1 + n + m + nv];
        prm[0] = t;
#pragma unroll
        for (int c = 0; c < n; ++c) prm[1 + c] = xv[c];
#pragma unroll
        for (int c = 0; c < m; ++c) prm[1 + n + c] = uv[c];
#pragma unroll
        for (int c = 0; c < nv; ++c) prm[1 + n + m + c] = vv[c];
        SymPath<P>::eval(prm, rec + R.oPx, rec + value_off);
        return;
    }
    D X[n > 0 ? n : 1], U[m > 0 ? m : 1], V[nv > 0 ? nv : 1], Tt, out[np > 0 ? np : 1];
    const int g0 = q * DC;
    constexpr int gT = n + m, gV = n + m + (P::PATH_T ? 1 : 0);
#pragma unroll
    for (int c = 0; c < n; ++c) {
        X[c].v = xv[c];
#pragma unroll
        for (int d = 0; d < DC; ++d) X[c].d[d] = (g0 + d == c) ? 1.0 : 0.0;
    }
#pragma unroll
    for (int c = 0; c < m; ++c) {
        U[c].v = uv[c];
#pragma unroll
        for (int d = 0; d < DC; ++d) U[c].d[d] = (g0 + d == n + c) ? 1.0 : 0.0;
    }
    Tt.v = t;
#pragma unroll
    for (int d = 0; d < DC; ++d) Tt.d[d] = (P::PATH_T && g0 + d == gT) ? 1.0 : 0.0;
#pragma unroll
    for (int c = 0; c < nv; ++c) {
        V[c].v = vv[c];
#pragma unroll
        for (int d = 0; d < DC; ++d) V[c].d[d] = (P::PATH_V && g0 + d == gV + c) ? 1.0 : 0.0;
    }
    P::template path<D>(out, Tt, X, U, V);
#pragma unroll
    for (int d = 0; d < DC; ++d) {
        const int g = g0 + d;
        if (g < n) {
#pragma unroll
            for (int r = 0; r < np; ++r) rec[R.oPx + r * R.ldx + g] = out[r].d[d];
        } else if (g < n + m) {
#pragma unroll
            for (int r = 0; r < np; ++r) rec[R.oPu + r * R.ldu + (g - n)] = out[r].d[d];
        } else if (P::PATH_T && g == n + m) {
#pragma unroll
            for (int r = 0; r < np; ++r) rec[R.oPt + r] = out[r].d[d];
        } else if (P::PATH_V && g < Dirs<P>::PATH) {
            const int kk = g - n - m - (P::PATH_T ? 1 : 0);
#pragma unroll
            for (int r = 0; r < np; ++r) rec[R.oPv + r * nv + kk] = out[r].d[d];
        }
    }
    if (q == 0) {
#pragma unroll
        for (int r = 0; r < np; ++r) rec[value_off + r] = out[r].v;
    }
}

template <class P, int SC, int S, bool REG = false>
CTD_HD void eval_step_path(const KParams& kp, const BlockCtx& cx, int k, int q) {
    constexpr int n = P::NX, m = P::NU, np = P::NPATH;
    constexpr RecLayout R = RL<P, SC, S>::R;
    constexpr int eqs = RL<P, SC, S>::cb - P::NPATH;
    const Layout& L = kp.L;
    const int64_t i = slot_index(kp, cx, k);
    if (i < 0 || i >= L.N) return;
    const double* base = slot_base(kp, cx, k);
    double uv[m > 0 ? m : 1];
    path_control<P, S>(kp, cx, k, i, uv);
    double xv[n > 0 ? n : 1];
#pragma unroll
    for (int c = 0; c < n; ++c) xv[c] = base[c];
    double* rec = cx.rec + k * R.stride;
    const double tau = slot_tau(kp, cx, k, 0);
    if constexpr (REG) {
        double lrec[R.oR + eqs + (np > 0 ? np : 1)];
#pragma unroll
        for (int e = R.oPx; e < R.oR; ++e) lrec[e] = 0.0;
        eval_path<P, SC, S>(kp, lrec, time_of<P>(kp, cx.v, tau), xv, uv, cx.v, q, R.oR + eqs);
        if (Dirs<P>::FUSED) fin_path<P, SC, S>(kp, lrec, tau);
#pragma unroll
        for (int e = R.oPx; e < R.oR; ++e) rec[e] = lrec[e];
#pragma unroll
        for (int r = 0; r < np; ++r) rec[R.oR + eqs + r] = lrec[R.oR + eqs + r];
    } else {
        eval_path<P, SC, S>(kp, rec, time_of<P>(kp, cx.v, tau), xv, uv, cx.v, q, R.oR + L.eqs);
        if (Dirs<P>::FUSED) fin_path<P, SC, S>(kp, rec, tau);
    }
}

template <class P, int SC, int S>
CTD_HD void eval_final_path(const KParams& kp, const BlockCtx& cx, int q) {
    constexpr int n = P::NX, m = P::NU;
    constexpr RecLayout R = RL<P, SC, S>::R;
    const Layout& L = kp.L;
    const double* base = slot_base(kp, cx, kp.edge_slot_last);
    const double* nxt = slot_next(kp, cx, kp.edge_slot_last);
    double xv[n > 0 ? n : 1], uv[m > 0 ? m : 1];
#pragma unroll
    for (int c = 0; c < n; ++c) xv[c] = nxt[c];
    if (SC == SC_TRAPEZE) {
#pragma unroll
        for (int c = 0; c < m; ++c) uv[c] = nxt[n + c];
    } else node_control<P, S>(kp, base, uv);
    double* rec = cx.rec + kp.edge_fp * R.stride;
    const double tau = final_tau(kp, cx);
    eval_path<P, SC, S>(kp, rec, time_of<P>(kp, cx.v, tau), xv, uv, cx.v, q, R.oR);
    if (Dirs<P>::FUSED) fin_path<P, SC, S>(kp, rec, tau);
}

template <class P, int SC, int S>
CTD_HD void eval_boundary(const KParams& kp, const BlockCtx& cx, int q) {
    constexpr int n = P::NX, nv = P::NV, nb = P::NBC, DC = P::DC;
    using D = Dual<DC>;
    const Layout& L = kp.L;
    constexpr RecLayout R = RL<P, SC, S>::R;
    const double* b0 = slot_base(kp, cx, kp.edge_slot_first);
    const double* bf = slot_next(kp, cx, kp.edge_slot_last);
    D X0[n > 0 ? n : 1], XF[n > 0 ? n : 1], V[nv > 0 ? nv : 1], out[nb > 0 ? nb : 1];
    const int g0 = q * DC;
#pragma unroll
    for (int c = 0; c < n; ++c) {
        X0[c].v = b0[c];
        XF[c].v = bf[c];
#pragma unroll
        for (int d = 0; d < DC; ++d) {
            X0[c].d[d] = (g0 + d == c) ? 1.0 : 0.0;
            XF[c].d[d] = (g0 + d == n + c) ? 1.0 : 0.0;
        }
    }
#pragma unroll
    for (int c = 0; c < nv; ++c) {
        V[c].v = cx.v[c];
#pragma unroll
        for (int d = 0; d < DC; ++d) V[c].d[d] = (g0 + d == 2 * n + c) ? 1.0 : 0.0;
    }
    P::template boundary<D>(out, X0, XF, V);
    double* rec = cx.rec + kp.edge_b * R.stride;
#pragma unroll
    for (int d = 0; d < DC; ++d) {
        const int g = g0 + d;
        if (g < n) {
#pragma unroll
            for (int r = 0; r < nb; ++r) rec[R.oB0 + r * R.ldx + g] = out[r].d[d];
        } else if (g < 2 * n) {
#pragma unroll
            for (int r = 0; r < nb; ++r) rec[R.oBf + r * R.ldx + (g - n)] = out[r].d[d];
        } else if (g < 2 * n + nv) {
#pragma unroll
            for (int r = 0; r < nb; ++r) rec[R.oBv + r * nv + (g - 2 * n)] = out[r].d[d];
        }
    }
    if (q == 0) {
#pragma unroll
        for (int r = 0; r < nb; ++r) rec[R.oBval + r] = out[r].v;
    }
}

template <class P, int SC, int S = 1> struct RegEval {
    static constexpr bool value = DirectTile<P, SC>::value && (P::NX * (P::NX + P::NU * (SC == SC_MIDPOINT ? S : 1) + P::NV + 2) <= 64);
};

template <class P, int SC, int S>
CTD_HD bool fin_folded(const BlockCtx& cx) {
    constexpr bool path_ok = P::NPATH == 0 || SymPath<P>::value || Dirs<P>::NCH_PATH == 1;
    return !Dirs<P>::FUSED && SymDyn<P>::value && path_ok && !cx.is_edge;
}

constexpr int kSplitMinParts = 4;

template <class P, int SC, int S>
CTD_HD bool edge_sym_layout(const BlockCtx& cx, int nthr) {
    constexpr int r_path = (P::NPATH > 0) ? Dirs<P>::NCH_PATH : 0;
    constexpr int n_b = (P::NBC > 0) ? Dirs<P>::NCH_BND : 0;
    constexpr bool parts = SymDyn<P>::parts >= kSplitMinParts && SymDyn<P>::parts == Dirs<P>::NCH_DYN;
    return SymDyn<P>::value && !Dirs<P>::FUSED && cx.is_edge && cx.nslots <= 8 && nthr >= 256 && r_path <= 4 && n_b <= 32 &&
           StagePoints<SC, S>::value * 8 <= 32 && (!parts || Dirs<P>::NCH_DYN * 64 <= nthr);
}

template <class P, int SC, int S>
CTD_HD bool split_eval(const BlockCtx& cx, int nthr) {
    constexpr bool ok = SymDyn<P>::value && SymDyn<P>::parts >= kSplitMinParts && SymDyn<P>::parts == Dirs<P>::NCH_DYN && !Dirs<P>::FUSED;
    constexpr int NP = Dirs<P>::NCH_DYN;
    constexpr int r_path = (P::NPATH > 0) ? Dirs<P>::NCH_PATH : 0;
    return ok && !cx.is_edge && StagePoints<SC, S>::value * cx.nslots + ((P::NPATH > 0) ? cx.nslots : 0) <= 64 && r_path <= NP && NP * 64 <= nthr;
}

CTD_HD void emit_store(double* p, double v, int wt = 0) {
#if defined(__HIP_DEVICE_COMPILE__)
    if (wt) { __hip_atomic_store(p, v, __ATOMIC_RELAXED, __HIP_MEMORY_SCOPE_AGENT); return; }
#endif
    *p = v;
}

template <bool B> CTD_HD double* out_c(const KParams& kp, const BatchLd& bl) { return member_out<B>(kp.c, bl.ldc); }
template <bool B> CTD_HD double* out_vals(const KParams& kp, const BatchLd& bl) { return member_out<B>(kp.vals, bl.ldv); }

template <int NB> struct EmitPreT { uint32_t b; uint32_t v[kMaxNV]; int64_t eidx; uint32_t more[NB > 1 ? NB - 1 : 1]; int kpos; uint32_t eb; int ek; int have; };
using EmitPre = EmitPreT<1>;
template <class P, int SC, int S, int NB, bool B = false>
CTD_HD void early_emit(const KParams& kp, const BlockCtx& cx, int l, const EmitPreT<NB>& pre, const BatchLd bl = BatchLd{}) {
    constexpr RecLayout R = RL<P, SC, S>::R;
    const int stride = R.stride;
    const int nsteps = (int)(cx.b - cx.a), slot0 = (int)(cx.a - cx.lo);
    const int ne = kp.n_early, nc = kp.c_early, vre = kp.vr_early;
    if (l < ne) {
        if (!kp.vals) return;
        const int64_t ra = cx.a > kp.reg_first ? cx.a : kp.reg_first, rb = cx.b < kp.reg_last ? cx.b : kp.reg_last;
        const int nreg = (int)(rb - ra);
        if (nreg <= 0) return;
        const uint32_t code = pre.eb;
        const int bt = code_beta(code);
        const double beta = bt == 0 ? 0.0 : (bt == 1 ? 1.0 : -1.0);
        const int sl0 = (int)(ra - cx.lo);
        const double* pc = cx.rec + sl0 * stride + R.oC + code_ci(code);
        const double* pd = cx.rec + sl0 * stride + code_di(code);
        double* out = out_vals<B>(kp, bl) + kp.seg_base + (ra - kp.reg_first) * (int64_t)kp.Lseg + pre.ek;
        const int last = nreg - 1;
        for (int s0 = 0; s0 < nreg; s0 += 4) {
            double a[4], b[4];
#pragma unroll
            for (int u = 0; u < 4; ++u) {
                const int s = s0 + u < last ? s0 + u : last;
                a[u] = pc[s * stride];
                b[u] = pd[s * stride];
            }
#pragma unroll
            for (int u = 0; u < 4; ++u)
                if (s0 + u < nreg) emit_store(&out[(s0 + u) * kp.Lseg], a[u] * b[u] + beta, kp.wt_store);
        }
    } else if (l < ne + nc) {
        if (!kp.c) return;
        const int r = l - ne;
        double* out = out_c<B>(kp, bl) + cx.a * (int64_t)kp.L.cb + r;
        const double* src = cx.rec + slot0 * stride + R.oR + r;
        for (int s = 0; s < nsteps; ++s) emit_store(&out[s * kp.L.cb], src[s * stride], kp.wt_store);
    } else if (l < ne + nc + P::NV * vre) {
        if (!kp.vals) return;
        const int e = l - ne - nc, kk = e / vre;
        const uint32_t code = pre.eb;
        const double* pc = cx.rec + slot0 * stride + R.oC + code_ci(code);
        const double* pd = cx.rec + slot0 * stride + code_di(code);
        double* out = out_vals<B>(kp, bl) + kp.vcol_base[kk] + cx.a * (int64_t)kp.vr + pre.ek;
        for (int s = 0; s < nsteps; ++s) emit_store(&out[s * kp.vr], pc[s * stride] * pd[s * stride], kp.wt_store);
    }
}

template <class P, int SC, int S> CTD_HD int early_leadbase(const KParams& kp) {
    constexpr int r_dyn = StagePoints<SC, S>::value * Dirs<P>::NCH_DYN, r_path = (P::NPATH > 0) ? Dirs<P>::NCH_PATH : 0;
    int lgT = 0;
    while ((1 << lgT) < kp.T) ++lgT;
    return (((r_dyn + r_path) << lgT) + 63) & ~63;
}

template <class P, int SC, int S, bool REG = false, int NB = 1, bool B = false>
CTD_HD void phase_eval(const KParams& kp, const BlockCtx& cx, int tid, int nthr, const EmitPreT<NB>* epre = nullptr,
                       const BatchLd bl = BatchLd{}) {
    constexpr bool FUSED = Dirs<P>::FUSED;
    constexpr RecLayout R = RL<P, SC, S>::R;
    const int ns = cx.nslots;
    constexpr int r_dyn = StagePoints<SC, S>::value * Dirs<P>::NCH_DYN;
    constexpr int r_path = (P::NPATH > 0) ? Dirs<P>::NCH_PATH : 0;
    constexpr int r_lead = FUSED ? 1 : 0;
    if (cx.is_edge) {
        constexpr int n_fp = (P::NPATH > 0) ? Dirs<P>::NCH_PATH : 0;
        constexpr int n_b = (P::NBC > 0) ? Dirs<P>::NCH_BND : 0;
        if constexpr (SymDyn<P>::value && !FUSED) {
            if (edge_sym_layout<P, SC, S>(cx, nthr)) {
                constexpr int NP = Dirs<P>::NCH_DYN;
                constexpr bool parts = SymDyn<P>::parts >= kSplitMinParts && SymDyn<P>::parts == NP;
                constexpr int NPW = parts ? NP : 1;
                const int wave = tid >> 6, l = tid & 63;
                if (wave < NPW && l < StagePoints<SC, S>::value * 8) {
                    const int j = l >> 3, k = l & 7;
                    if (k < ns) {
                        double* ev = cx.rec + k * R.stride + R.oEval + j * R.eval_sz;
                        if constexpr (parts) {
                            eval_dynamics<P, SC, S, true>(kp, cx, k, j, wave, ev);
                            fin_stage<P, SC, S>(kp, cx, k, j, ev, wave, NP);
                        } else {
                            eval_dynamics<P, SC, S>(kp, cx, k, j, 0, ev);
                            fin_stage<P, SC, S>(kp, cx, k, j, ev);
                        }
                    }
                } else if (l >= 32) {
                    const int a = wave - (parts ? 0 : 1), t = l - 32;
                    if (a == 0) { if (t < r_path * 8 && (t & 7) < ns) eval_step_path<P, SC, S>(kp, cx, t & 7, t >> 3); }
                    else if (a == 1) {
                        if (t < n_fp) eval_final_path<P, SC, S>(kp, cx, t);
                        else if (t >= 8 && t < 10) fill_const_coefs<P>(kp, cx.rec + (t == 8 ? kp.edge_fp : kp.edge_b) * R.stride + R.oC);
                    } else if (a == 2) { if (t < n_b) eval_boundary<P, SC, S>(kp, cx, t); }
                }
                for (int k = tid; k < ns + 2; k += nthr) cx.rec[k * R.stride] = 1.0;
                return;
            }
        }
        constexpr int seg0 = 0;
        constexpr int seg1 = seg0 + ((r_dyn * 8 + 63) & ~63);
        constexpr int seg2 = seg1 + ((r_path * 8 + n_fp + 63) & ~63);
        constexpr int seg3 = seg2 + ((r_lead * 8 + 2 + 63) & ~63);
        constexpr int segE = seg3 + ((n_b + 63) & ~63);
        const bool wide = ns <= 8 && segE <= nthr;
        const int total = wide ? segE : (r_dyn + r_path + r_lead) * ns + n_fp + n_b + 2;
        for (int task = tid; task < total; task += nthr) {
            int kind, k = 0, role = 0;
            if (wide) {
                if (task < seg1) { const int l = task - seg0; kind = 0; role = l >> 3; k = l & 7; if (role >= r_dyn) continue; }
                else if (task < seg2) {
                    const int l = task - seg1;
                    if (l < r_path * 8) { kind = 1; role = l >> 3; k = l & 7; }
                    else if (l < r_path * 8 + n_fp) { kind = 3; role = l - r_path * 8; }
                    else continue;
                } else if (task < seg3) {
                    const int l = task - seg2;
                    if (l < r_lead * 8) { kind = 2; k = l & 7; }
                    else if (l < r_lead * 8 + 2) { kind = 5; role = l - r_lead * 8; }
                    else continue;
                } else { const int l = task - seg3; if (l >= n_b) continue; kind = 4; role = l; }
                if (k >= ns) continue;
            } else {
                int t = task;
                if (t < r_dyn * ns) { kind = 0; role = t / ns; k = t - role * ns; }
                else if ((t -= r_dyn * ns) < r_path * ns) { kind = 1; role = t / ns; k = t - role * ns; }
                else if ((t -= r_path * ns) < r_lead * ns) { kind = 2; k = t; }
                else if ((t -= r_lead * ns) < n_fp) { kind = 3; role = t; }
                else if ((t -= n_fp) < n_b) { kind = 4; role = t; }
                else { kind = 5; role = t - n_b; }
            }
            if (kind == 0) {
                const int j = role / Dirs<P>::NCH_DYN, q = role % Dirs<P>::NCH_DYN;
                double* ev = cx.rec + k * R.stride + R.oEval + j * R.eval_sz;
                eval_dynamics<P, SC, S>(kp, cx, k, j, q, ev);
                if (FUSED) fin_stage<P, SC, S>(kp, cx, k, j, ev);
            } else if (kind == 1) eval_step_path<P, SC, S>(kp, cx, k, role);
            else if (kind == 2) fin_lead<P, SC, S>(kp, cx, k);
            else if (kind == 3) eval_final_path<P, SC, S>(kp, cx, role);
            else if (kind == 4) eval_boundary<P, SC, S>(kp, cx, role);
            else fill_const_coefs<P>(kp, cx.rec + (role == 0 ? kp.edge_fp : kp.edge_b) * R.stride + R.oC);
        }
        for (int k = tid; k < ns + 2; k += nthr) cx.rec[k * R.stride] = 1.0;
        return;
    }
    CTD_SUB(kp, 0);
    if constexpr (SymDyn<P>::value && SymDyn<P>::parts >= kSplitMinParts && SymDyn<P>::parts == Dirs<P>::NCH_DYN && !FUSED) {
        if (split_eval<P, SC, S>(cx, nthr)) {
            constexpr int NP = Dirs<P>::NCH_DYN;
            const int nd = StagePoints<SC, S>::value * ns;
            const int wave = tid >> 6, l = tid & 63;
            const bool fold = fin_folded<P, SC, S>(cx);
            auto fin_path_slot = [&](int k) {
                const int64_t i = slot_index(kp, cx, k);
                if (i >= 0 && i < kp.L.N) fin_path<P, SC, S>(kp, cx.rec + k * R.stride, slot_tau(kp, cx, k, 0));
            };
            if (wave < NP) {
#if !defined(CTD_ABL) || CTD_ABL != 2
                if (l < nd) {
                    const int j = l / ns, k = l - j * ns;
                    double* ev = cx.rec + k * R.stride + R.oEval + j * R.eval_sz;
                    eval_dynamics<P, SC, S, true>(kp, cx, k, j, wave, ev);
                    if (fold) fin_stage<P, SC, S>(kp, cx, k, j, ev, wave, NP);
                }
#endif
                CTD_SUB(kp, 2);
#if !defined(CTD_ABL) || CTD_ABL != 3
                if (SC == SC_IRK) {
                    if (l < nd)
                        for (int t = l * NP + wave; t < ns * P::NX; t += nd * NP) fin_lead<P, SC, S>(kp, cx, t / P::NX, t % P::NX);
                } else if (l < ns && wave == NP - 1) {
                    fin_lead<P, SC, S>(kp, cx, l);
                }
#endif
                CTD_SUB(kp, 3);
#if !defined(CTD_ABL) || CTD_ABL != 1
                if (l >= nd && l < nd + ns) {
                    constexpr int PW = NP > 1 ? 1 : 0;
                    if (SymPath<P>::value ? wave == PW : wave < r_path) {
                        eval_step_path<P, SC, S>(kp, cx, l - nd, SymPath<P>::value ? 0 : wave);
                        if (fold) fin_path_slot(l - nd);
                    }
                }
#endif
                CTD_SUB(kp, 4);
            }
            for (int k = tid; k < ns; k += nthr) cx.rec[k * R.stride] = 1.0;
            CTD_SUB(kp, 5);
            return;
        }
    }
    const int lg = ns <= 1 ? 0 : 32 - __builtin_clz((unsigned)(ns - 1));
    const int mask = (1 << lg) - 1;
    if constexpr (FUSED && SC == SC_IRK) {
        if (kp.n_early > 0 && epre != nullptr) {
            int lgT = 0;
            while ((1 << lgT) < kp.T) ++lgT;
            const int nb = (r_dyn + r_path) << lgT, leadbase = (nb + 63) & ~63;
            const int tmask = (1 << lgT) - 1;
            if (tid < nb) {
                const int k = tid & tmask, role = tid >> lgT;
                if (k < ns) {
                    if (role < r_dyn) {
                        const int j = role / Dirs<P>::NCH_DYN, q = role % Dirs<P>::NCH_DYN;
                        double* ev = cx.rec + k * R.stride + R.oEval + j * R.eval_sz;
                        if constexpr (REG) {
                            double evr[R.eval_sz];
#pragma unroll
                            for (int e = 0; e < R.eval_sz; ++e) evr[e] = 0.0;
                            eval_dynamics<P, SC, S>(kp, cx, k, j, q, evr);
                            fin_stage<P, SC, S>(kp, cx, k, j, evr);
                            const int64_t i = slot_index(kp, cx, k);
                            if (i >= 0 && i < kp.L.N) {
#pragma unroll
                                for (int e = 0; e < R.eval_sz; ++e) ev[e] = evr[e];
                            }
                        } else {
                            eval_dynamics<P, SC, S>(kp, cx, k, j, q, ev);
                            fin_stage<P, SC, S>(kp, cx, k, j, ev);
                        }
                    } else {
                        eval_step_path<P, SC, S, REG>(kp, cx, k, role - r_dyn);
                    }
                }
            } else if ((tid >> 6) == (leadbase >> 6)) {
                const int k = tid - leadbase;
                if (k < ns) {
                    fin_lead<P, SC, S>(kp, cx, k);
                    cx.rec[k * R.stride] = 1.0;
                }
#if defined(__HIP_DEVICE_COMPILE__)
                __builtin_amdgcn_fence(__ATOMIC_RELEASE, "wavefront");
                __builtin_amdgcn_wave_barrier();
                __builtin_amdgcn_fence(__ATOMIC_ACQUIRE, "wavefront");
                early_emit<P, SC, S, NB, B>(kp, cx, tid & 63, *epre, bl);
#endif
            }
            for (int k = tid; k < ns; k += nthr) cx.rec[k * R.stride] = 1.0;
            return;
        }
    }
    const bool fold_g = fin_folded<P, SC, S>(cx);
    const int total = (r_dyn + r_path + ((FUSED || fold_g) ? 1 : 0)) << lg;
    for (int task = tid; task < total; task += nthr) {
        const int k = task & mask, role = task >> lg;
        if (k >= ns) continue;
        if (role < r_dyn) {
            const int j = role / Dirs<P>::NCH_DYN, q = role % Dirs<P>::NCH_DYN;
            double* ev = cx.rec + k * R.stride + R.oEval + j * R.eval_sz;
            if constexpr (REG) {
                double evr[R.eval_sz];
#pragma unroll
                for (int e = 0; e < R.eval_sz; ++e) evr[e] = 0.0;
                CTD_SUB(kp, 1);
                eval_dynamics<P, SC, S>(kp, cx, k, j, q, evr);
                CTD_SUB(kp, 2);
                fin_stage<P, SC, S>(kp, cx, k, j, evr);
                CTD_SUB(kp, 3);
                const int64_t i = slot_index(kp, cx, k);
                if (i >= 0 && i < kp.L.N) {
#pragma unroll
                    for (int e = 0; e < R.eval_sz; ++e) ev[e] = evr[e];
                }
                CTD_SUB(kp, 4);
            } else {
                eval_dynamics<P, SC, S>(kp, cx, k, j, q, ev);
                if (FUSED || (fold_g && q == 0)) fin_stage<P, SC, S>(kp, cx, k, j, ev);
            }
        } else if (role < r_dyn + r_path) {
            eval_step_path<P, SC, S, REG>(kp, cx, k, role - r_dyn);
            if (fold_g) {
                const int64_t i = slot_index(kp, cx, k);
                if (i >= 0 && i < kp.L.N) fin_path<P, SC, S>(kp, cx.rec + k * R.stride, slot_tau(kp, cx, k, 0));
            }
        } else {
            CTD_SUB(kp, 1);
            fin_lead<P, SC, S>(kp, cx, k);
            CTD_SUB(kp, 4);
        }
    }
    for (int k = tid; k < ns; k += nthr) cx.rec[k * R.stride] = 1.0;
    CTD_SUB(kp, 5);
}

template <class P, int SC, int S>
CTD_HD void phase_fin(const KParams& kp, const BlockCtx& cx, int tid, int nthr) {
    if (Dirs<P>::FUSED) return;
    if (fin_folded<P, SC, S>(cx)) return;
    constexpr RecLayout R = RL<P, SC, S>::R;
    const int ns = cx.nslots;
    constexpr int rows = (SC == SC_IRK && P::NX > 4) ? P::NX : 1;
    const bool split = split_eval<P, SC, S>(cx, nthr);
    const bool esl = edge_sym_layout<P, SC, S>(cx, nthr);
    const int n_stage = esl ? 0 : StagePoints<SC, S>::value * ns * rows, n_lead = split ? 0 : ns, n_path = (P::NPATH > 0 && !split) ? ns : 0;
    const int n_fp = (cx.is_edge && P::NPATH > 0) ? 1 : 0;
    for (int task = tid; task < n_stage + n_lead + n_path + n_fp; task += nthr) {
        int t = task;
        if (t < n_stage) {
            const int k = t % ns, jr = t / ns;
            if (rows > 1) fin_stage_row<P, S>(kp, cx, k, jr / rows, jr % rows);
            else fin_stage<P, SC, S>(kp, cx, k, jr, cx.rec + k * R.stride + R.oEval + jr * R.eval_sz);
            if (split && P::NPATH > 0 && jr == 0) {
                const int64_t i = slot_index(kp, cx, k);
                if (i >= 0 && i < kp.L.N) fin_path<P, SC, S>(kp, cx.rec + k * R.stride, slot_tau(kp, cx, k, 0));
            }
            continue;
        }
        t -= n_stage;
        if (t < n_lead) { fin_lead<P, SC, S>(kp, cx, t); continue; }
        t -= n_lead;
        if (t < n_path) {
            const int64_t i = slot_index(kp, cx, t);
            if (i >= 0 && i < kp.L.N) fin_path<P, SC, S>(kp, cx.rec + t * R.stride, slot_tau(kp, cx, t, 0));
            continue;
        }
        fin_path<P, SC, S>(kp, cx.rec + kp.edge_fp * R.stride, final_tau(kp, cx));
    }
}

template <class P, int SC, int S>
CTD_HD void phase_fin2(const KParams& kp, const BlockCtx& cx, int tid, int nthr) {
    if (SC == SC_TRAPEZE && !cx.is_edge)
        for (int k = tid; k < cx.nslots; k += nthr) fin_trapeze_step<P>(kp, cx, k);
}

CTD_HD double eval_code(int oC, const double* rec_c, const double* rec_d, uint32_t code) {
    const double coef = rec_c[oC + code_ci(code)];
    const double data = rec_d[code_di(code)];
    const int bt = code_beta(code);
    const double beta = bt == 0 ? 0.0 : (bt == 1 ? 1.0 : -1.0);
    return coef * data + beta;
}

CTD_HD int edge_share_begin(const KParams& kp, const BlockCtx& cx, int ntot) {
    const int E = kp.has_edge > 1 ? kp.has_edge : 1, per = (ntot + E - 1) / E;
    const int lo = cx.edge_part * per;
    return lo < ntot ? lo : ntot;
}
CTD_HD int edge_share_end(const KParams& kp, const BlockCtx& cx, int ntot) {
    const int E = kp.has_edge > 1 ? kp.has_edge : 1, per = (ntot + E - 1) / E;
    const int hi = (cx.edge_part + 1) * per;
    return hi < ntot ? hi : ntot;
}

template <class P, int SC, int S> struct EmitN {
    static constexpr int n = P::NX, m = P::NU, nv = P::NV, p = P::NPATH, s = SC == SC_IRK ? S : 0;
    static constexpr int seg = SC == SC_IRK ? n * (2 * n + s * n + nv) + s * n * (n + s * m + s * n + nv) + p * (n + s * m + nv)
                                            : n * (2 * n + 2 * m * (SC == SC_MIDPOINT ? S : 1) + nv) + p * (n + 2 * m + nv);
#ifndef CTD_PRE_MAX
#define CTD_PRE_MAX 1
#endif
    static constexpr int value = (seg + 255) / 256 < 1 ? 1 : ((seg + 255) / 256 > CTD_PRE_MAX ? CTD_PRE_MAX : (seg + 255) / 256);
};
template <class P, int NB = 1>
CTD_HD EmitPreT<NB> emit_prefetch(const KParams& kp, const BlockCtx& cx, int tid, int nthr) {
    EmitPreT<NB> pre;
    pre.b = 0u;
    pre.eidx = 0;
    pre.have = 1;
    pre.kpos = 0; pre.eb = 0u; pre.ek = 0;
#pragma unroll
    for (int q = 0; q < (NB > 1 ? NB - 1 : 1); ++q) pre.more[q] = 0u;
#pragma unroll
    for (int kk = 0; kk < kMaxNV; ++kk) pre.v[kk] = 0u;
    if (cx.is_edge) {
        const int n1 = kp.edge_end - kp.edge_begin, ntot = n1 + (kp.edge2_end - kp.edge2_begin);
        const int w = edge_share_begin(kp, cx, ntot) + tid;
        if (w < edge_share_end(kp, cx, ntot)) {
            const int e = w < n1 ? kp.edge_begin + w : kp.edge2_begin + (w - n1);
            pre.b = kp.edge_code[e];
            pre.eidx = kp.edge_idx[e];
        }
        return pre;
    }
    const int Ls = kp.Lseg;
    pre.kpos = 0; pre.eb = 0u; pre.ek = 0;
    if (kp.n_early > 0) {
        const int q = tid - (int)fast_div((uint32_t)tid, kp.div_late) * kp.n_late;
        pre.kpos = kp.pos[q];
        pre.b = kp.tmpl[pre.kpos];
        const int l = tid & 63;
        if (l < kp.n_early) { pre.ek = kp.pos[kp.n_late + l]; pre.eb = kp.tmpl[pre.ek]; }
        else if (l >= kp.n_early + kp.c_early && l < kp.n_early + kp.c_early + P::NV * kp.vr_early) {
            const int e = l - kp.n_early - kp.c_early, kk = e / kp.vr_early;
            pre.ek = e - kk * kp.vr_early;
            pre.eb = kp.vtmpl[kk * kp.vr + pre.ek];
        }
    } else if (Ls > 0 && Ls <= nthr) {
        const int k = tid - (int)fast_div((uint32_t)tid, kp.div_Lseg) * Ls;
        pre.b = kp.tmpl[k];
    } else if (Ls > nthr) {
        pre.b = kp.tmpl[tid];
        if constexpr (NB > 1) {
#pragma unroll
            for (int q = 0; q < NB - 1; ++q)
                if (tid + (q + 1) * nthr < Ls) pre.more[q] = kp.tmpl[tid + (q + 1) * nthr];
        }
    }
    const int vr = kp.vr;
#pragma unroll
    for (int kk = 0; kk < kMaxNV; ++kk) {
        if (kk < P::NV && vr > 0 && vr <= nthr) {
            const int k = tid - (int)fast_div((uint32_t)tid, kp.div_vr) * vr;
            pre.v[kk] = kp.vtmpl[kk * vr + k];
        }
    }
    return pre;
}

template <class P, int SC, int S, int NB = 1, bool B = false>
CTD_HD void phase_emit_impl(const KParams& kp, const BlockCtx& cx, int tid, int nthr, const EmitPreT<NB> pre_v, const bool hp,
                            const BatchLd bl = BatchLd{}) {
    const Layout& L = kp.L;
    constexpr RecLayout R = RL<P, SC, S>::R;
    const EmitPreT<NB>* pre_ = &pre_v;
    if (cx.is_edge) {
        const int n1 = kp.edge_end - kp.edge_begin, nall = n1 + (kp.edge2_end - kp.edge2_begin);
        const int wlo = edge_share_begin(kp, cx, nall), ntot = edge_share_end(kp, cx, nall);
        for (int w0 = wlo + tid; w0 < ntot; w0 += 4 * nthr) {
            uint32_t code[4];
            int64_t idx[4];
#pragma unroll
            for (int u = 0; u < 4; ++u) {
                const int w = w0 + u * nthr;
                const int e = w < n1 ? kp.edge_begin + w : kp.edge2_begin + (w - n1);
                const bool have = hp && w == wlo + tid;
                code[u] = have ? pre_->b : (w < ntot ? kp.edge_code[e] : 0u);
                idx[u] = have ? pre_->eidx : (w < ntot ? kp.edge_idx[e] : 0);
            }
#pragma unroll
            for (int u = 0; u < 4; ++u) {
                if (w0 + u * nthr >= ntot) break;
                const double val = eval_code(R.oC, cx.rec + code_crec(code[u]) * R.stride, cx.rec + code_drec_raw(code[u]) * R.stride, code[u]);
                if (idx[u] & kEdgeCBit) { if (kp.c) out_c<B>(kp, bl)[idx[u] & ~kEdgeCBit] = val; }
                else if (kp.vals) out_vals<B>(kp, bl)[idx[u]] = val;
            }
        }
        return;
    }
    const int nsteps = (int)(cx.b - cx.a);
    const int slot0 = (int)(cx.a - cx.lo);
    CTD_SUBE(kp, 0);
    const int stride = R.stride;
    if (kp.c) {
        const int cb = L.cb;
        double* out = out_c<B>(kp, bl) + cx.a * (int64_t)cb;
        const int par = (int)fast_div((uint32_t)nthr, kp.div_cb);
        if (par >= 1) {
            if (tid < par * cb) {
                const int g = (int)fast_div((uint32_t)tid, kp.div_cb), r = tid - g * cb;
                const double* src = cx.rec + (slot0 + g) * stride + R.oR + r;
                if (r >= kp.c_early)
                    for (int s = g; s < nsteps; s += par, src += par * stride) emit_store(&out[s * cb + r], *src, kp.wt_store);
            }
        } else {
            for (int r = tid; r < cb; r += nthr) {
                const double* src = cx.rec + slot0 * stride + R.oR + r;
                for (int s = 0; s < nsteps; ++s, src += stride) emit_store(&out[s * cb + r], *src, kp.wt_store);
            }
        }
    }
    CTD_SUBE(kp, 1);
    if (!kp.vals) return;
    {
        const int64_t ra = cx.a > kp.reg_first ? cx.a : kp.reg_first;
        const int64_t rb = cx.b < kp.reg_last ? cx.b : kp.reg_last;
        if (rb > ra) {
            const int Ls = kp.Lseg;
            const int nreg = (int)(rb - ra);
            double* out = out_vals<B>(kp, bl) + kp.seg_base + (ra - kp.reg_first) * (int64_t)Ls;
            const int sl0 = (int)(ra - cx.lo);
            const bool late_only = kp.n_early > 0;
            const int Lw = late_only ? kp.n_late : Ls;
            const int par = (int)fast_div((uint32_t)nthr, late_only ? kp.div_late : kp.div_Lseg);
            if (par >= 1) {
                if (tid < par * Lw) {
                    const int g = (int)fast_div((uint32_t)tid, late_only ? kp.div_late : kp.div_Lseg);
                    const int k = late_only ? (hp ? pre_->kpos : (int)kp.pos[tid - g * Lw]) : tid - g * Ls;
                    const uint32_t code = hp ? pre_->b : cx.codes[k];
                    const int bt = code_beta(code);
                    const double beta = bt == 0 ? 0.0 : (bt == 1 ? 1.0 : -1.0);
                    const double* pc = cx.rec + (sl0 - code_crec(code)) * stride + R.oC + code_ci(code);
                    const double* pd = cx.rec + (sl0 - code_drec(code)) * stride + code_di(code);
                    const int last = nreg - 1;
                    for (int s0 = g; s0 < nreg; s0 += 4 * par) {
                        double a[4], b[4];
#pragma unroll
                        for (int u = 0; u < 4; ++u) {
                            const int s = s0 + u * par < last ? s0 + u * par : last;
                            a[u] = pc[s * stride];
                            b[u] = pd[s * stride];
                        }
#pragma unroll
                        for (int u = 0; u < 4; ++u) {
                            const int s = s0 + u * par;
                            if (s < nreg) emit_store(&out[s * Ls + k], a[u] * b[u] + beta, kp.wt_store);
                        }
                    }
                }
            } else {
                uint32_t code = (hp && tid < Ls) ? pre_->b : (tid < Ls ? cx.codes[tid] : 0u);
                int q = 0;
                for (int k = tid; k < Ls; k += nthr, ++q) {
                    uint32_t nxt = 0u;
                    bool have = false;
                    if constexpr (NB > 1) {
                        if (hp && q < NB - 1) {
                            have = true;
#pragma unroll
                            for (int e = 0; e < NB - 1; ++e)
                                if (e == q) nxt = pre_->more[e];
                        }
                    }
                    if (!have) nxt = k + nthr < Ls ? cx.codes[k + nthr] : 0u;
                    const int bt = code_beta(code);
                    const double beta = bt == 0 ? 0.0 : (bt == 1 ? 1.0 : -1.0);
                    const double* pc = cx.rec + (sl0 - code_crec(code)) * stride + R.oC + code_ci(code);
                    const double* pd = cx.rec + (sl0 - code_drec(code)) * stride + code_di(code);
                    const int last = nreg - 1;
                    for (int s0 = 0; s0 < nreg; s0 += 4) {
                        double a[4], b[4];
#pragma unroll
                        for (int u = 0; u < 4; ++u) {
                            const int s = s0 + u < last ? s0 + u : last;
                            a[u] = pc[s * stride];
                            b[u] = pd[s * stride];
                        }
#pragma unroll
                        for (int u = 0; u < 4; ++u)
                            if (s0 + u < nreg) emit_store(&out[(s0 + u) * Ls + k], a[u] * b[u] + beta, kp.wt_store);
                    }
                    code = nxt;
                }
            }
        }
    }
    CTD_SUBE(kp, 2);
    if (kp.vr > 0) {
        const int vr = kp.vr;
        const int par = (int)fast_div((uint32_t)nthr, kp.div_vr);
#pragma unroll
        for (int kk = 0; kk < P::NV; ++kk) {
            double* out = out_vals<B>(kp, bl) + kp.vcol_base[kk] + cx.a * (int64_t)vr;
            const uint32_t* codes = cx.vcodes + kk * vr;
            if (par >= 1) {
                if (tid < par * vr) {
                    const int g = (int)fast_div((uint32_t)tid, kp.div_vr), k = tid - g * vr;
                    const uint32_t code = hp ? pre_->v[kk] : codes[k];
                    const double* pc = cx.rec + (slot0 + g) * stride + R.oC + code_ci(code);
                    const double* pd = cx.rec + (slot0 + g) * stride + code_di(code);
                    const int adv = par * stride;
                    if (k >= kp.vr_early)
                        for (int s = g; s < nsteps; s += par, pc += adv, pd += adv) emit_store(&out[s * vr + k], (*pc) * (*pd), kp.wt_store);
                }
            } else {
                for (int k = tid; k < vr; k += nthr) {
                    const uint32_t code = codes[k];
                    const double* pc = cx.rec + slot0 * stride + R.oC + code_ci(code);
                    const double* pd = cx.rec + slot0 * stride + code_di(code);
                    for (int s = 0; s < nsteps; ++s, pc += stride, pd += stride) emit_store(&out[s * vr + k], (*pc) * (*pd), kp.wt_store);
                }
            }
        }
    }
    CTD_SUBE(kp, 3);
}
template <class P, int SC, int S, int NB = 1, bool B = false>
CTD_HD void phase_emit(const KParams& kp, const BlockCtx& cx, int tid, int nthr, const EmitPreT<NB>* pre = nullptr,
                       const BatchLd bl = BatchLd{}) {
    if (pre != nullptr) phase_emit_impl<P, SC, S, NB, B>(kp, cx, tid, nthr, *pre, pre->have != 0, bl);
    else phase_emit_impl<P, SC, S, NB, B>(kp, cx, tid, nthr, EmitPreT<NB>{}, false, bl);
}

}

#if !defined(__HIPCC_RTC__)
#include "ctd_problems.hpp"
#include "ctd_sym_registry.hpp"
#endif
```

### ctdirect.jl_amd/csrc/ctd_kernels.hpp

```cpp
#pragma once
#if !defined(__HIPCC_RTC__)
#include <hip/hip_runtime.h>
#include <hip/hip_ext.h>
#endif

#include "ctd_kernel_body.hpp"
#if !defined(__HIPCC_RTC__)
#include "ctd_problems.hpp"
#endif

namespace ctd {

#ifndef CTD_MULTI_TILE_LOOP
#define CTD_MULTI_TILE_LOOP 0
#endif
constexpr bool kMultiTileLoop = CTD_MULTI_TILE_LOOP != 0;

template <bool DBG>
__device__ __forceinline__ void ctd_stamp(const KParams& kp, int slot) {
    if constexpr (DBG) {
        if (kp.stamps && threadIdx.x == 0) {
            unsigned long long* p = kp.stamps + ((size_t)blockIdx.x * 6 + slot) * 2;
            p[0] = wall_clock64();
            p[1] = clock64();
        }
    }
}

template <int S>
__device__ __forceinline__ void ctd_pin_kernargs(const KParams& kp, const double* xu) {
#if defined(__HIP_DEVICE_COMPILE__)
    asm volatile("" ::"s"(kp.has_edge), "s"(kp.ntiles), "s"(kp.T), "s"(kp.HL), "s"(kp.HH), "s"(kp.step_begin),
                 "s"(kp.step_end), "s"(kp.L.blk), "s"(kp.L.N), "s"(kp.L.v_off), "s"(kp.L.cu), "s"(kp.L.stagewise), "s"(kp.L.nv),
                 "s"(kp.L.cb), "s"(kp.L.eqs), "s"(kp.L.euler), "s"(kp.tau), "s"(kp.L.t0), "s"(kp.L.tf), "s"(xu), "s"(blockDim.x));
    asm volatile("" ::"s"(kp.tmpl), "s"(kp.vtmpl), "s"(kp.Lseg), "s"(kp.vr), "s"(kp.div_cb.M), "s"(kp.div_Lseg.M), "s"(kp.div_vr.M),
                 "s"(kp.div_cb.d), "s"(kp.div_Lseg.d), "s"(kp.div_vr.d), "s"(kp.seg_base), "s"(kp.reg_first), "s"(kp.reg_last),
                 "s"(kp.vcol_base[0]), "s"(kp.c), "s"(kp.vals), "s"(kp.halo), "s"(kp.pos), "s"(kp.n_early), "s"(kp.n_late));
    if (S >= 1) asm volatile("" ::"s"(kp.L.a[0]), "s"(kp.L.b[0]), "s"(kp.L.c[0]));
    if (S >= 2) asm volatile("" ::"s"(kp.L.a[1]), "s"(kp.L.a[3]), "s"(kp.L.a[4]), "s"(kp.L.b[1]), "s"(kp.L.c[1]));
    if (S >= 3) asm volatile("" ::"s"(kp.L.a[2]), "s"(kp.L.a[5]), "s"(kp.L.a[6]), "s"(kp.L.a[7]), "s"(kp.L.a[8]), "s"(kp.L.b[2]), "s"(kp.L.c[2]));
#endif
}

__device__ __forceinline__ void ctd_pin_emit_kernargs(const KParams& kp) {
#if defined(__HIP_DEVICE_COMPILE__)
    asm volatile("" ::"s"(kp.c), "s"(kp.vals), "s"(kp.L.cb), "s"(kp.Lseg), "s"(kp.vr), "s"(kp.div_cb.M), "s"(kp.div_Lseg.M), "s"(kp.div_vr.M),
                 "s"(kp.div_cb.d), "s"(kp.div_Lseg.d), "s"(kp.div_vr.d), "s"(kp.seg_base), "s"(kp.reg_first), "s"(kp.reg_last),
                 "s"(kp.vcol_base[0]), "s"(kp.n_early), "s"(kp.c_early), "s"(kp.vr_early), "s"(kp.n_late), "s"(kp.div_late.M), "s"(kp.div_late.d));
#endif
}

template <class P, int SC, int S, bool DBG, bool B = false>
__device__ __forceinline__ void cons_jac_body(const KParams& kp, const double* __restrict__ xu, int block, double* ctd_lds,
                                              const BatchLd bl = BatchLd{}) {
    if constexpr (B) xu += batch_member() * bl.ldx;
    ctd_pin_kernargs<SC == SC_IRK ? S : 0>(kp, xu);
    ctd_stamp<DBG>(kp, 0);
    if (DBG && kp.debug_stop == 1) return;
    const int tid = (int)threadIdx.x, nthr = (int)blockDim.x;
    if constexpr (DirectTile<P, SC>::value) {
        const BlockCtx cx = make_direct_ctx(kp, block, ctd_lds, xu);
        const EmitPre pre = emit_prefetch<P>(kp, cx, tid, nthr);
        ctd_stamp<DBG>(kp, 1);
        phase_eval<P, SC, S, RegEval<P, SC, S>::value, 1, B>(kp, cx, tid, nthr, &pre, bl);
        ctd_pin_emit_kernargs(kp);
        __syncthreads();
        ctd_stamp<DBG>(kp, 2);
        ctd_stamp<DBG>(kp, 3);
        if (DBG && kp.debug_stop >= 2 && kp.debug_stop <= 4) return;
        phase_emit<P, SC, S, 1, B>(kp, cx, tid, nthr, &pre, bl);
        ctd_stamp<DBG>(kp, 4);
        if (DBG && kp.stamps) {
            __builtin_amdgcn_s_waitcnt(0);
            __syncthreads();
            ctd_stamp<DBG>(kp, 5);
        }
        return;
    }
    BlockCtx cx = make_ctx(kp, block, ctd_lds);
    constexpr int NB = EmitN<P, SC, S>::value;
    EmitPreT<NB> pre = {};
    const bool use_pre = !cx.is_edge && !codes_staged(kp);
    if (use_pre) pre = emit_prefetch<P, NB>(kp, cx, tid, nthr);
    phase_load<P, SC, S>(kp, cx, xu, tid, nthr);
    const int nblk = kp.ntiles + kp.has_edge;
    for (;;) {
        __syncthreads();
        ctd_stamp<DBG>(kp, 1);
        if (DBG && kp.debug_stop == 2) return;
        phase_eval<P, SC, S, false, 1, B>(kp, cx, tid, nthr, nullptr, bl);
        ctd_pin_emit_kernargs(kp);
        __syncthreads();
        ctd_stamp<DBG>(kp, 2);
        if (DBG && kp.debug_stop == 3) return;
        if (!Dirs<P>::FUSED && !fin_folded<P, SC, S>(cx)) {
            phase_fin<P, SC, S>(kp, cx, tid, nthr);
            __syncthreads();
        }
        if (SC == SC_TRAPEZE) {
            phase_fin2<P, SC, S>(kp, cx, tid, nthr);
            __syncthreads();
        }
        ctd_stamp<DBG>(kp, 3);
        if (DBG && kp.debug_stop == 4) return;
        block += kp.wg_stride;
        const bool more = kMultiTileLoop && kp.wg_stride > 0 && !cx.is_edge && block < nblk;
        BlockCtx nx = cx;
        TileIn tin{0.0, 0.0, 0.0};
        if (more) {
            nx = make_ctx(kp, block, ctd_lds);
            tin = load_issue<P>(kp, nx, xu, tid, nthr);
        }
        phase_emit_impl<P, SC, S, NB, B>(kp, cx, tid, nthr, pre, use_pre, bl);
        ctd_stamp<DBG>(kp, 4);
        if (!more) break;
        load_commit<P, SC, S>(kp, nx, xu, tin, tid, nthr);
        cx = nx;
    }
    if (DBG && kp.stamps) {
        __builtin_amdgcn_s_waitcnt(0);
        __syncthreads();
        ctd_stamp<DBG>(kp, 5);
    }
}

template <class P, int SC, int S> struct MinWaves {
    static constexpr int value = (P::NX <= 12 && !(SC == SC_MIDPOINT && S > 1)) ? 4 : 1;
};

template <class P, int SC, int S, bool DBG>
__global__ void __launch_bounds__(P::MAXB, (MinWaves<P, SC, S>::value)) cons_jac_kernel(const KParams kp, const double* __restrict__ xu) {
    extern __shared__ double ctd_lds[];
    cons_jac_body<P, SC, S, DBG>(kp, xu, (int)blockIdx.x, ctd_lds);
}
template <class P, int SC, int S>
__global__ void __launch_bounds__(P::MAXB, (MinWaves<P, SC, S>::value)) cons_jac_batch_kernel(const KParams kp, const double* __restrict__ xu,
                                                                                          const BatchLd bl) {
    extern __shared__ double ctd_lds[];
    cons_jac_body<P, SC, S, false, true>(kp, xu, (int)blockIdx.x, ctd_lds, bl);
}

struct ObjParams {
    Layout L;
    const double* tau;
    int64_t unit_begin, unit_end;
    int32_t add_mayer;
    double* partial;
    double* out;
    int32_t nblocks;
    const XHalo* halo;
    XNear near;
    int64_t ldx;
};

template <class P> __device__ double obj_time(const ObjParams& op, const double* v, int64_t i) {
    const double t0 = (P::IT0 >= 0) ? v[P::IT0 >= 0 ? P::IT0 : 0] : op.L.t0;
    const double tf = (P::ITF >= 0) ? v[P::ITF >= 0 ? P::ITF : 0] : op.L.tf;
    const double tau = op.tau ? op.tau[i] : (double)i / (double)op.L.N;
    return t0 + tau * (tf - t0);
}

template <class P, int SC>
__device__ double lagrange_unit(const ObjParams& op, const double* __restrict__ xu, const double* v, int64_t i) {
    constexpr int n = P::NX, m = P::NU;
    const Layout& L = op.L;
    const double* base = xu + i * (int64_t)L.blk;
    const int64_t gn = (i + 1) * (int64_t)L.blk;
    const double* nxt = ((op.halo && i + 1 >= op.unit_end) ? xnear(op.near, xu, gn) : xu) + gn;
    double x[n > 0 ? n : 1], u[m > 0 ? m : 1];
    if (SC == SC_TRAPEZE) {
        double w;
        if (i == 0) w = (obj_time<P>(op, v, 1) - obj_time<P>(op, v, 0)) / 2.0;
        else if (i == L.N) w = (obj_time<P>(op, v, L.N) - obj_time<P>(op, v, L.N - 1)) / 2.0;
        else w = (obj_time<P>(op, v, i + 1) - obj_time<P>(op, v, i - 1)) / 2.0;
        for (int c = 0; c < n; ++c) x[c] = base[c];
        for (int c = 0; c < m; ++c) u[c] = base[n + c];
        return w * P::template lagrange<double>(obj_time<P>(op, v, i), x, u, v);
    }
    const double ti = obj_time<P>(op, v, i), tip1 = obj_time<P>(op, v, i + 1);
    const double h = tip1 - ti;
    if (SC == SC_MIDPOINT) {
        if (L.cs > 1) {
            const double hi = h / (double)L.cs;
            for (int c = 0; c < n; ++c) x[c] = 0.5 * (base[c] + nxt[c]);
            double val = 0.0;
            for (int j = 1; j <= L.cs; ++j) {
                for (int c = 0; c < m; ++c) u[c] = base[n + (j - 1) * m + c];
                const double term = hi * P::template lagrange<double>(ti + ((double)j - 0.5) * hi, x, u, v);
                val = (j == 1) ? term : val + term;
            }
            return val;
        }
        for (int c = 0; c < m; ++c) u[c] = base[n + c];
        if (L.euler == 0) {
            for (int c = 0; c < n; ++c) x[c] = 0.5 * (base[c] + nxt[c]);
            return h * P::template lagrange<double>(0.5 * (ti + tip1), x, u, v);
        }
        for (int c = 0; c < n; ++c) x[c] = (L.euler == 1) ? base[c] : nxt[c];
        return h * P::template lagrange<double>(L.euler == 1 ? ti : tip1, x, u, v);
    }
    const double* K = base + n + L.cu;
    double local = 0.0;
    for (int j = 0; j < L.s; ++j) {
        for (int c = 0; c < n; ++c) {
            double xc = base[c];
            for (int l = 0; l < L.s; ++l) xc = xc + h * L.a[3 * j + l] * K[l * n + c];
            x[c] = xc;
        }
        const double* U = base + n + (L.stagewise ? j * m : 0);
        for (int c = 0; c < m; ++c) u[c] = U[c];
        const double term = L.b[j] * P::template lagrange<double>(ti + L.c[j] * h, x, u, v);
        local = (j == 0) ? term : local + term;
    }
    return h * local;
}

template <class P, int SC>
__device__ __forceinline__ void obj_partial_body(const ObjParams& op, const double* __restrict__ xu, int block, int nblocks, double* wsum,
                                                 int64_t mb = 0) {
    double v[P::NV > 0 ? P::NV : 1];
    for (int k = 0; k < P::NV; ++k) v[k] = xu[op.L.v_off + k];
    double acc = 0.0;
    if (P::HAS_LAGRANGE) {
        for (int64_t i = op.unit_begin + (int64_t)block * blockDim.x + threadIdx.x; i < op.unit_end;
             i += (int64_t)nblocks * blockDim.x)
            acc += lagrange_unit<P, SC>(op, xu, v, i);
    }
    for (int off = 32; off > 0; off >>= 1) acc += __shfl_down(acc, off, 64);
    const int lane = threadIdx.x & 63, wave = threadIdx.x >> 6;
    if (lane == 0) wsum[wave] = acc;
    __syncthreads();
    if (threadIdx.x == 0) {
        double s = 0.0;
        for (int w = 0; w < (int)(blockDim.x >> 6); ++w) s += wsum[w];
        op.partial[mb * nblocks + block] = s;
    }
}
template <class P, int SC>
__global__ void __launch_bounds__(256) obj_partial_kernel(const ObjParams op, const double* __restrict__ xu) {
    __shared__ double wsum[4];
    const int64_t mb = batch_member();
    obj_partial_body<P, SC>(op, xu + mb * op.ldx, (int)blockIdx.x, (int)gridDim.x, wsum, mb);
}

template <class P>
__device__ __forceinline__ void obj_finish_body(const ObjParams& op, const double* __restrict__ xu, int64_t mb = 0) {
    if (threadIdx.x >= 64) return;
    const double* part = op.partial + mb * op.nblocks;
    double s = 0.0;
    for (int b = threadIdx.x; b < op.nblocks; b += 64) s += part[b];
    for (int off = 32; off > 0; off >>= 1) s += __shfl_down(s, off, 64);
    if (threadIdx.x != 0) return;
    double mayer = 0.0;
    if (P::HAS_MAYER && op.add_mayer) {
        constexpr int n = P::NX, nv = P::NV;
        double x0[n > 0 ? n : 1], xf[n > 0 ? n : 1], v[nv > 0 ? nv : 1];
        const int64_t gf = op.L.N * (int64_t)op.L.blk;
        const double* xa = op.halo ? xnear(op.near, xu, 0) : xu;
        const double* xb = op.halo ? xnear(op.near, xu, gf) : xu;
        for (int c = 0; c < n; ++c) { x0[c] = xa[c]; xf[c] = xb[gf + c]; }
        for (int k = 0; k < nv; ++k) v[k] = xu[op.L.v_off + k];
        mayer = P::template mayer<double>(x0, xf, v);
    }
    op.out[mb] = mayer + s;
}
template <class P>
__global__ void obj_finish_kernel(const ObjParams op, const double* __restrict__ xu) {
    if (blockIdx.x != 0) return;
    const int64_t mb = batch_member();
    obj_finish_body<P>(op, xu + mb * op.ldx, mb);
}

struct GradParams {
    Layout L;
    const double* tau;
    double* g;
    double* partial;
    int32_t nblocks;
    int64_t unit_begin, unit_end;
    int32_t owns_first, owns_last;
    const XHalo* halo;
    XNear near;
    int64_t ldx, ldg;
};
CTD_HD const double* grad_block(const GradParams& gp, const double* xu, int64_t st) {
    const int64_t g = st * (int64_t)gp.L.blk;
// ... 163 lines not shown
                                const double d0 = FREE ? dtime_of<P>(t0, k) : 0.0, d1 = FREE ? dtime_of<P>(t1, k) : 0.0;
                                const double dhi = (d1 - d0) / cs;
                                gv[k] = gv[k] + dhi * val + hi * ((P::LAG_V ? lv[k] : 0.0) + ((P::LAG_T && FREE) ? lt * (d0 + w * dhi) : 0.0));
                            }
                        }
                    }
                }
            } else {
            if (i < L.N) {
                const double t0 = grad_tau<P>(gp, i), t1 = grad_tau<P>(gp, i + 1);
                const double ta = grad_time<P>(gp, v, t0), tb = grad_time<P>(gp, v, t1), h = tb - ta;
                for (int c = 0; c < n; ++c) x[c] = L.euler == 0 ? 0.5 * (base[c] + nextb[c]) : (L.euler == 1 ? base[c] : nextb[c]);
                for (int c = 0; c < m; ++c) u[c] = base[n + c];
                lagrange_partials<P, 0>(L.euler == 0 ? 0.5 * (ta + tb) : (L.euler == 1 ? ta : tb), x, u, v, val, lx, lu, lt, lv);
                if (wa != 0.0) for (int c = 0; c < n; ++c) gx[c] = h * (wa * lx[c]);
                for (int c = 0; c < m; ++c) g[i * L.blk + n + c] = h * lu[c];
                for (int k = 0; k < nv; ++k) {
                    const double d0 = FREE ? dtime_of<P>(t0, k) : 0.0, d1 = FREE ? dtime_of<P>(t1, k) : 0.0;
                    const double dts = L.euler == 0 ? 0.5 * (d0 + d1) : (L.euler == 1 ? d0 : d1);
                    gv[k] = (d1 - d0) * val + h * ((P::LAG_V ? lv[k] : 0.0) + ((P::LAG_T && FREE) ? lt * dts : 0.0));
                }
            }
            if (i >= 1 && wb != 0.0) {
                const double* pb = grad_block(gp, xu, i - 1);
                const double ta = grad_time<P>(gp, v, grad_tau<P>(gp, i - 1)), tb = grad_time<P>(gp, v, grad_tau<P>(gp, i));
                const double h = tb - ta;
                for (int c = 0; c < n; ++c) x[c] = L.euler == 0 ? 0.5 * (pb[c] + base[c]) : base[c];
                for (int c = 0; c < m; ++c) u[c] = pb[n + c];
                double val2 = 0.0, lt2 = 0.0, lu2[m > 0 ? m : 1], lv2[nv > 0 ? nv : 1];
                lagrange_partials<P, 0>(L.euler == 0 ? 0.5 * (ta + tb) : tb, x, u, v, val2, lx, lu2, lt2, lv2);
                for (int c = 0; c < n; ++c) gx[c] = gx[c] + h * (wb * lx[c]);
            }
            }
            for (int c = 0; c < n; ++c) g[i * L.blk + c] = gx[c];
        } else {
            const double t0 = grad_tau<P>(gp, i), t1 = grad_tau<P>(gp, i + 1);
            const double ti = grad_time<P>(gp, v, t0), h = grad_time<P>(gp, v, t1) - ti;
            const double* K = base + n + L.cu;
            double gx[n > 0 ? n : 1], gK[S][n > 0 ? n : 1], gu[m > 0 ? m : 1];
            for (int c = 0; c < n; ++c) { gx[c] = 0.0; for (int l = 0; l < S; ++l) gK[l][c] = 0.0; }
            for (int c = 0; c < m; ++c) gu[c] = 0.0;
            double sum_bl = 0.0;
#pragma unroll 1
            for (int j = 0; j < S; ++j) {
                double sa[n > 0 ? n : 1];
                for (int c = 0; c < n; ++c) {
                    double xc = base[c], acc = 0.0;
#pragma unroll
                    for (int l = 0; l < S; ++l) { xc = xc + h * L.a[3 * j + l] * K[l * n + c]; acc = acc + L.a[3 * j + l] * K[l * n + c]; }
                    x[c] = xc; sa[c] = acc;
                }
                const double* U = base + n + (L.stagewise ? j * m : 0);
                for (int c = 0; c < m; ++c) u[c] = U[c];
                lagrange_partials<P, 0>(ti + L.c[j] * h, x, u, v, val, lx, lu, lt, lv);
                const double hb = h * L.b[j];
                for (int c = 0; c < n; ++c) {
                    gx[c] = gx[c] + hb * lx[c];
#pragma unroll
                    for (int l = 0; l < S; ++l) gK[l][c] = gK[l][c] + hb * (h * L.a[3 * j + l]) * lx[c];
                }
                if (L.stagewise) { for (int c = 0; c < m; ++c) g[i * L.blk + n + j * m + c] = hb * lu[c]; }
                else { for (int c = 0; c < m; ++c) gu[c] = gu[c] + hb * lu[c]; }
                sum_bl = sum_bl + L.b[j] * val;
                for (int k = 0; k < nv; ++k) {
                    const double d0 = FREE ? dtime_of<P>(t0, k) : 0.0, dh = FREE ? dtime_of<P>(t1, k) - d0 : 0.0;
                    double e = P::LAG_V ? lv[k] : 0.0;
                    if (P::LAG_T && FREE) e = e + lt * (d0 + L.c[j] * dh);
                    if (FREE) for (int c = 0; c < n; ++c) e = e + lx[c] * (dh * sa[c]);
                    gv[k] = gv[k] + hb * e;
                }
            }
            for (int k = 0; k < nv; ++k) {
                const double dh = FREE ? dtime_of<P>(t1, k) - dtime_of<P>(t0, k) : 0.0;
                gv[k] = gv[k] + dh * sum_bl;
            }
            for (int c = 0; c < n; ++c) g[i * L.blk + c] = gx[c];
            if (!L.stagewise) for (int c = 0; c < m; ++c) g[i * L.blk + n + c] = gu[c];
#pragma unroll
            for (int l = 0; l < S; ++l)
                for (int c = 0; c < n; ++c) g[i * L.blk + n + L.cu + l * n + c] = gK[l][c];
        }
    }
    const int lane = threadIdx.x & 63, wave = threadIdx.x >> 6;
    for (int k = 0; k < nv; ++k) {
        double a = gv[k];
        for (int off = 32; off > 0; off >>= 1) a += __shfl_down(a, off, 64);
        if (lane == 0) wsum[wave][k] = a;
    }
    __syncthreads();
    if (threadIdx.x == 0)
        for (int k = 0; k < nv; ++k) {
            double sacc = 0.0;
            for (int w = 0; w < (int)(blockDim.x >> 6); ++w) sacc += wsum[w][k];
            gp.partial[((size_t)mb * gp.nblocks + block) * kMaxNV + k] = sacc;
        }
}
template <class P, int SC, int S>
__global__ void __launch_bounds__(256) __attribute__((amdgpu_waves_per_eu(2))) grad_units_kernel(const GradParams gp, const double* __restrict__ xu) {
    __shared__ double wsum[4][kMaxNV];
    const int64_t mb = batch_member();
    grad_units_body<P, SC, S>(gp, xu + mb * gp.ldx, (int)blockIdx.x, wsum, mb);
}

template <class P>
__device__ __forceinline__ void grad_finish_body(const GradParams& gp, const double* __restrict__ xu, int64_t mb = 0) {
    if (threadIdx.x >= 64) return;
    constexpr int n = P::NX, nv = P::NV;
    const Layout& L = gp.L;
    const double* part = gp.partial + (size_t)mb * gp.nblocks * kMaxNV;
    double* const g = gp.g + mb * gp.ldg;
    double gvs[nv > 0 ? nv : 1];
    for (int k = 0; k < nv; ++k) {
        double sacc = 0.0;
        for (int b = threadIdx.x; b < gp.nblocks; b += 64) sacc += part[(size_t)b * kMaxNV + k];
        for (int off = 32; off > 0; off >>= 1) sacc += __shfl_down(sacc, off, 64);
        gvs[k] = sacc;
    }
    if (threadIdx.x != 0) return;
    if (P::HAS_MAYER && (gp.owns_first || gp.owns_last)) {
        double x0[n > 0 ? n : 1], xf[n > 0 ? n : 1], v[nv > 0 ? nv : 1], g0x[n > 0 ? n : 1], gfx[n > 0 ? n : 1], gmv[nv > 0 ? nv : 1];
        const double* b0 = grad_block(gp, xu, 0);
        const double* bf = grad_block(gp, xu, L.N);
        for (int c = 0; c < n; ++c) { x0[c] = b0[c]; xf[c] = bf[c]; g0x[c] = 0.0; gfx[c] = 0.0; }
        for (int k = 0; k < nv; ++k) { v[k] = xu[L.v_off + k]; gmv[k] = 0.0; }
        mayer_partials<P, 0>(x0, xf, v, g0x, gfx, gmv);
        for (int c = 0; c < n; ++c) {
            if (gp.owns_first) g[c] += g0x[c];
            if (gp.owns_last) g[L.N * (int64_t)L.blk + c] += gfx[c];
        }
        if (gp.owns_last) for (int k = 0; k < nv; ++k) gvs[k] += gmv[k];
    }
    for (int k = 0; k < nv; ++k) g[L.v_off + k] = gvs[k];
}
template <class P>
__global__ void grad_finish_kernel(const GradParams gp, const double* __restrict__ xu) {
    if (blockIdx.x != 0) return;
    const int64_t mb = batch_member();
    grad_finish_body<P>(gp, xu + mb * gp.ldx, mb);
}

#if !defined(__HIPCC_RTC__)
template <class P>
hipError_t launch_grad(const GradParams& gp, const double* xu, int grid, hipStream_t st, int batch) {
    const dim3 g(grid > 0 ? grid : 1, batch);
    if (grid > 0)
        for_scheme<false>(gp.L, [&](auto t) { grad_units_kernel<P, t.sc, t.s><<<g, 256, 0, st>>>(gp, xu); });
    grad_finish_kernel<P><<<dim3(1, batch), 64, 0, st>>>(gp, xu);
    return hipGetLastError();
}

#endif

#if !defined(__HIPCC_RTC__)
template <class P, int SC, int S, bool DBG>
hipError_t launch_variant_dbg(const KParams& kp, const double* xu, int grid, int block, size_t lds_bytes, hipStream_t st,
                              hipEvent_t e0, hipEvent_t e1) {
    if (lds_bytes > 64 * 1024) {
        hipError_t e = hipFuncSetAttribute((const void*)cons_jac_kernel<P, SC, S, DBG>, hipFuncAttributeMaxDynamicSharedMemorySize,
                                           (int)lds_bytes);
        if (e != hipSuccess) return e;
    }
    if (e0 || e1) hipExtLaunchKernelGGL((cons_jac_kernel<P, SC, S, DBG>), dim3(grid), dim3(block), lds_bytes, st, e0, e1, 0, kp, xu);
    else cons_jac_kernel<P, SC, S, DBG><<<grid, block, lds_bytes, st>>>(kp, xu);
    return hipGetLastError();
}
template <class P, int SC, int S>
hipError_t launch_variant(const KParams& kp, const double* xu, int grid, int block, size_t lds_bytes, hipStream_t st,
                          hipEvent_t e0, hipEvent_t e1) {
    if (kp.stamps || kp.debug_stop) return launch_variant_dbg<P, SC, S, true>(kp, xu, grid, block, lds_bytes, st, e0, e1);
    return launch_variant_dbg<P, SC, S, false>(kp, xu, grid, block, lds_bytes, st, e0, e1);
}

template <class P>
hipError_t launch_cons_jac(const KParams& kp, const double* xu, int grid, int block, size_t lds_bytes, hipStream_t st,
                           hipEvent_t e0, hipEvent_t e1) {
    hipError_t e = hipErrorInvalidValue;
    for_scheme<true>(kp.L, [&](auto t) { e = launch_variant<P, t.sc, t.s>(kp, xu, grid, block, lds_bytes, st, e0, e1); });
    return e;
}

template <class P, int SC, int S>
int occupancy_variant(int block, size_t lds_bytes) {
    int nb = 0;
    if (lds_bytes > 64 * 1024 &&
        hipFuncSetAttribute((const void*)cons_jac_kernel<P, SC, S, false>, hipFuncAttributeMaxDynamicSharedMemorySize, (int)lds_bytes) != hipSuccess)
        return 0;
    if (hipOccupancyMaxActiveBlocksPerMultiprocessor(&nb, cons_jac_kernel<P, SC, S, false>, block, lds_bytes) != hipSuccess) return 0;
    return nb;
}
template <class P, int SC, int S>
hipError_t launch_variant_batch(const KParams& kp, const double* xu, const BatchLd& bl, int grid, int block, size_t lds_bytes, hipStream_t st,
                                int batch) {
    if (lds_bytes > 64 * 1024) {
        hipError_t e = hipFuncSetAttribute((const void*)cons_jac_batch_kernel<P, SC, S>, hipFuncAttributeMaxDynamicSharedMemorySize, (int)lds_bytes);
        if (e != hipSuccess) return e;
    }
    cons_jac_batch_kernel<P, SC, S><<<dim3(grid, batch), block, lds_bytes, st>>>(kp, xu, bl);
    return hipGetLastError();
}
template <class P>
hipError_t launch_cons_jac_batch(const KParams& kp, const double* xu, const BatchLd& bl, int grid, int block, size_t lds_bytes,
                                 hipStream_t st, int batch) {
    hipError_t e = hipErrorInvalidValue;
    for_scheme<true>(kp.L, [&](auto t) { e = launch_variant_batch<P, t.sc, t.s>(kp, xu, bl, grid, block, lds_bytes, st, batch); });
    return e;
}

template <class P>
int occupancy_cons_jac(const KParams& kp, int block, size_t lds_bytes) {
    int nb = 0;
    for_scheme<true>(kp.L, [&](auto t) { nb = occupancy_variant<P, t.sc, t.s>(block, lds_bytes); });
    return nb;
}

template <class P>
hipError_t launch_obj(const ObjParams& op, const double* xu, int grid, int block, hipStream_t st, int batch) {
    const dim3 g(grid > 0 ? grid : 1, batch);
    if (grid > 0)
        for_scheme<false>(op.L, [&](auto t) { obj_partial_kernel<P, t.sc><<<g, block, 0, st>>>(op, xu); });
    obj_finish_kernel<P><<<dim3(1, batch), 64, 0, st>>>(op, xu);
    return hipGetLastError();
}

#define CTD_INSTANTIATE_LAUNCHERS(P)                                                                                       \
    template hipError_t launch_cons_jac<P>(const KParams&, const double*, int, int, size_t, hipStream_t, hipEvent_t, \
                                           hipEvent_t);                                                                    \
    template hipError_t launch_cons_jac_batch<P>(const KParams&, const double*, const BatchLd&, int, int, size_t, hipStream_t, int); \
    template hipError_t launch_obj<P>(const ObjParams&, const double*, int, int, hipStream_t, int);                  \
    template int occupancy_cons_jac<P>(const KParams&, int, size_t);                                                 \
    template hipError_t launch_grad<P>(const GradParams&, const double*, int, hipStream_t, int);
#define CTD_EXTERN_LAUNCHERS(P)                                                                                            \
    extern template hipError_t launch_cons_jac<P>(const KParams&, const double*, int, int, size_t, hipStream_t,      \
                                                  hipEvent_t, hipEvent_t);                                                 \
    extern template hipError_t launch_cons_jac_batch<P>(const KParams&, const double*, const BatchLd&, int, int, size_t, hipStream_t, \
                                                        int);                                                                      \
    extern template hipError_t launch_obj<P>(const ObjParams&, const double*, int, int, hipStream_t, int);          \
    extern template int occupancy_cons_jac<P>(const KParams&, int, size_t);                                         \
    extern template hipError_t launch_grad<P>(const GradParams&, const double*, int, hipStream_t, int);

#endif

}
```

Measured before the change: 166,000 evals/s.

## Add lean kernel variant with compile-time layout and Butcher constants, no halo paths

Adds a LEAN template instantiation of the fused constraint+Jacobian kernel. It folds layout sizes (blk, cu, cb, eqs) and the Gauss-Legendre Butcher coefficients into compile-time constants instead of reading them from kernel arguments. It also drops the halo/xnear branches and uses branchless edge-step selection. The lean path is chosen at launch when there is no halo and no early steps, and ctd_create checks that the static layout matches the model. The aim is fewer scalar loads, divisions and branches per slot, at the cost of doubling the kernel instantiations and more code size.

Result: faster. 179,600 evals/s, median of 6 (+8.2%).

```diff
diff --git a/ctdirect.jl_amd/csrc/ctd_engine.hip b/ctdirect.jl_amd/csrc/ctd_engine.hip
--- a/ctdirect.jl_amd/csrc/ctd_engine.hip
+++ b/ctdirect.jl_amd/csrc/ctd_engine.hip
@@ -63,6 +63,7 @@
     bool own_stream = false;
     int64_t step_begin = 0, step_end = 0;
     int tile = 0, block = 256;
+    int lean_ok = 1;
     KParams kp;
     size_t lds_bytes = 0;
     int grid = 0;
@@ -409,6 +410,14 @@
     }
     if (st) return fail(nullptr, st, err);
     const Model& mo = h->model;
+    if (!runtime_ocp(mo.problem)) {
+        const char* bad = nullptr;
+        for_problem(mo.problem, [&](auto tag) {
+            using P = typename decltype(tag)::type;
+            for_scheme<true>(mo.L, [&](auto t) { bad = static_layout_mismatch<P, t.sc, t.s>(mo.L); });
+        });
+        if (bad) return fail(nullptr, CTD_EINVAL, std::string("ctd_create: the static layout of the kernel instantiation differs from the model's layout in field '") + bad + "'");
+    }
     if (mo.L.cs > 3 && desc->device >= 0 && !runtime_ocp(mo.problem))
         return fail(nullptr, CTD_EINVAL, "ctd_create: control_steps > 3 needs an OCP registered at run time (ctd_register_ocp); the compiled registry holds the midpoint kernels for 1, 2 and 3 controls per step");
     h->step_begin = desc->step_begin;
@@ -417,6 +426,7 @@
     if (h->step_begin < 0 || h->step_end > mo.L.N || h->step_begin >= h->step_end)
         return fail(nullptr, CTD_EINVAL, "ctd_create: shard [step_begin, step_end) is not inside [0, N)");
     h->tile = env_int("CTD_TILE", 0);
+    h->lean_ok = env_int("CTD_LEAN", 1) ? 1 : 0;
     if (h->tile <= 0) h->tile = default_tile(mo, h->step_end - h->step_begin);
     int maxb = 256;
     for_problem(mo.problem, [&](auto tag) { maxb = decltype(tag)::type::MAXB; });
@@ -959,7 +969,7 @@
     }
     for_problem(h->model.problem, [&](auto tag) {
         using P = typename decltype(tag)::type;
-        e = launch_cons_jac<P>(kp, x_dev, h->grid, h->block, h->lds_bytes, h->stream, te0, te1);
+        e = launch_cons_jac<P>(kp, x_dev, h->grid, h->block, h->lds_bytes, h->stream, te0, te1, h->lean_ok);
     });
     if (e != hipSuccess) return fail(h, CTD_EHIP, std::string("kernel launch: ") + hipGetErrorString(e));
     return CTD_OK;
diff --git a/ctdirect.jl_amd/csrc/ctd_kernel_body.hpp b/ctdirect.jl_amd/csrc/ctd_kernel_body.hpp
--- a/ctdirect.jl_amd/csrc/ctd_kernel_body.hpp
+++ b/ctdirect.jl_amd/csrc/ctd_kernel_body.hpp
@@ -49,7 +49,9 @@
     const double* xu;
 };
 
+template <bool LEAN = false>
 CTD_HD const XHalo* block_halo(const KParams& kp, const BlockCtx& cx) {
+    if constexpr (LEAN) return nullptr;
     if (!kp.halo) return nullptr;
     if (cx.is_edge) return kp.halo;
     return (cx.lo < kp.step_begin || cx.b + kp.HH >= kp.step_end) ? kp.halo : nullptr;
@@ -61,12 +63,21 @@
     const int64_t g = (lds_bytes + 1279) / 1280 * 1280;
     return g > 0 ? (int)((160 * 1024) / g) : 32;
 }
-CTD_HD int code_doubles(const KParams& kp) { return codes_staged(kp) ? (kp.Lseg + kp.L.nv * kp.vr + 1) / 2 : 0; }
-
-CTD_HD int64_t slot_index(const KParams& kp, const BlockCtx& cx, int k) {
-    return cx.is_edge ? kp.edge_steps[k] : cx.lo + k;
-}
-
+CTD_HD int code_doubles(const KParams& kp, int nv = -1) { return codes_staged(kp) ? (kp.Lseg + (nv < 0 ? kp.L.nv : nv) * kp.vr + 1) / 2 : 0; }
+
+template <bool LEAN = false> CTD_HD int64_t edge_step(const KParams& kp, int k) {
+    if constexpr (LEAN) {
+        int64_t st = kp.edge_steps[0];
+#pragma unroll
+        for (int e = 1; e < kMaxEdgeSlots; ++e) st = (k == e) ? kp.edge_steps[e] : st;
+        return st;
+    } else return kp.edge_steps[k];
+}
+template <bool LEAN = false> CTD_HD int64_t slot_index(const KParams& kp, const BlockCtx& cx, int k) {
+    return cx.is_edge ? edge_step<LEAN>(kp, k) : cx.lo + k;
+}
+
+template <bool LEAN = false>
 CTD_HD BlockCtx make_ctx(const KParams& kp, int block, double* lds) {
     BlockCtx cx;
     cx.direct = 0;
@@ -100,20 +111,22 @@
         cx.rec = cx.tau + cap + 2;
     }
     cx.xu = nullptr;
-    cx.halo = block_halo(kp, cx);
+    cx.halo = block_halo<LEAN>(kp, cx);
     return cx;
 }
 
-CTD_HD BlockCtx make_direct_ctx(const KParams& kp, int block, double* lds, const double* xu) {
+template <bool LEAN = false>
+CTD_HD BlockCtx make_direct_ctx(const KParams& kp, int block, double* lds, const double* xu, int blk = -1, int nv = -1) {
     BlockCtx cx;
     const Layout& L = kp.L;
+    if (blk < 0) blk = L.blk;
     cx.direct = 1;
     cx.codes = kp.tmpl;
     cx.vcodes = kp.vtmpl;
-    cx.in_stride = L.blk;
+    cx.in_stride = blk;
     cx.v = const_cast<double*>(xu) + L.v_off;
     cx.tau = nullptr;
-    cx.rec = lds + code_doubles(kp);
+    cx.rec = lds + code_doubles(kp, nv);
     cx.xu = xu;
     cx.halo = nullptr;
     cx.edge_part = 0;
@@ -123,7 +136,7 @@
         cx.nslots = kp.n_edge_slots;
         cx.a = cx.b = cx.lo = 0;
         cx.in = const_cast<double*>(xu);
-        cx.halo = kp.halo;
+        if constexpr (!LEAN) cx.halo = kp.halo;
         return cx;
     }
     const int tile = block - kp.has_edge;
@@ -132,32 +145,36 @@
     cx.b = cx.a + kp.T < kp.step_end ? cx.a + kp.T : kp.step_end;
     cx.lo = cx.a - kp.HL;
     cx.nslots = (int)(cx.b - cx.a) + kp.HL + kp.HH;
-    cx.in = const_cast<double*>(xu) + cx.lo * (int64_t)L.blk;
-    cx.halo = block_halo(kp, cx);
+    cx.in = const_cast<double*>(xu) + cx.lo * (int64_t)blk;
+    cx.halo = block_halo<LEAN>(kp, cx);
     return cx;
 }
 
-CTD_HD const double* slot_base(const KParams& kp, const BlockCtx& cx, int k) {
+template <bool LEAN = false> CTD_HD const double* slot_base(const KParams& kp, const BlockCtx& cx, int k) {
     if (cx.direct && cx.halo) {
         const int64_t g = slot_index(kp, cx, k) * (int64_t)cx.in_stride;
         return xnear(kp.near, cx.xu, g) + g;
     }
-    if (cx.direct && cx.is_edge) return cx.in + kp.edge_steps[k] * (int64_t)cx.in_stride;
+    if (cx.direct && cx.is_edge) return cx.in + edge_step<LEAN>(kp, k) * (int64_t)cx.in_stride;
     return cx.in + k * cx.in_stride;
 }
+template <bool LEAN = false>
 CTD_HD const double* slot_next(const KParams& kp, const BlockCtx& cx, int k) {
+    if constexpr (LEAN) { if (cx.direct) return slot_base<LEAN>(kp, cx, k) + cx.in_stride; }
     if (cx.direct && cx.halo) {
         const int64_t g = (slot_index(kp, cx, k) + 1) * (int64_t)cx.in_stride;
         return xnear(kp.near, cx.xu, g) + g;
     }
-    return slot_base(kp, cx, k) + ((cx.direct || cx.is_edge) ? kp.L.blk : cx.in_stride);
-}
+    return slot_base<LEAN>(kp, cx, k) + ((cx.direct || cx.is_edge) ? kp.L.blk : cx.in_stride);
+}
+template <bool LEAN = false>
 CTD_HD const double* slot_prev(const KParams& kp, const BlockCtx& cx, int k) {
+    if constexpr (LEAN) { if (cx.direct) return slot_base<LEAN>(kp, cx, k) - cx.in_stride; }
     if (cx.direct && cx.halo) {
         const int64_t g = (slot_index(kp, cx, k) - 1) * (int64_t)cx.in_stride;
         return xnear(kp.near, cx.xu, g) + g;
     }
-    return slot_base(kp, cx, k) - ((cx.direct || cx.is_edge) ? kp.L.blk : cx.in_stride);
+    return slot_base<LEAN>(kp, cx, k) - ((cx.direct || cx.is_edge) ? kp.L.blk : cx.in_stride);
 }
 
 inline int64_t lds_doubles(const KParams& kp) {
@@ -174,8 +191,8 @@
     if (i > kp.L.N) i = kp.L.N;
     return kp.tau ? kp.tau[i] : (double)i / (double)kp.L.N;
 }
-CTD_HD double slot_tau(const KParams& kp, const BlockCtx& cx, int k, int d) {
-    if (cx.direct) return tau_global(kp, slot_index(kp, cx, k) + d);
+template <bool LEAN = false> CTD_HD double slot_tau(const KParams& kp, const BlockCtx& cx, int k, int d) {
+    if (cx.direct) return tau_global(kp, slot_index<LEAN>(kp, cx, k) + d);
     return cx.is_edge ? cx.tau[2 * k + d] : cx.tau[k + d];
 }
 CTD_HD double final_tau(const KParams& kp, const BlockCtx& cx) {
@@ -228,6 +245,77 @@
 
 template <class P, int SC> struct DirectTile { static constexpr bool value = Dirs<P>::FUSED && SC != SC_TRAPEZE; };
 
+constexpr double kSqrt3 = 1.7320508075688772, kSqrt15 = 3.872983346207417;
+template <class P, int SC, int S> struct StaticLayout {
+    static constexpr int n = P::NX, m = P::NU, nv = P::NV, p = P::NPATH, bc = P::NBC;
+    static constexpr int s = SC == SC_IRK ? S : 0;
+    static constexpr int eqs = SC == SC_IRK ? n * (1 + S) : n;
+    static constexpr int cb = eqs + p;
+    CTD_HD static constexpr int cu(bool stagewise) { return SC == SC_TRAPEZE ? m : ((SC == SC_MIDPOINT || stagewise) ? m * S : m); }
+    CTD_HD static constexpr int blk(bool stagewise) { return n + cu(stagewise) + (SC == SC_IRK ? S * n : 0); }
+    CTD_HD static constexpr double a(int j, int l) {
+        if (SC != SC_IRK || j >= S || l >= S) return 0.0;
+        if (S == 1) return 0.5;
+        if (S == 2) return j == l ? 0.25 : (j == 0 ? 0.25 - kSqrt3 / 6 : 0.25 + kSqrt3 / 6);
+        switch (3 * j + l) {
+            case 0: return 5.0 / 36.0;                case 1: return 2.0 / 9 - kSqrt15 / 15;   case 2: return 5.0 / 36 - kSqrt15 / 30;
+            case 3: return 5.0 / 36.0 + kSqrt15 / 24; case 4: return 2.0 / 9.0;                case 5: return 5.0 / 36.0 - kSqrt15 / 24;
+            case 6: return 5.0 / 36 + kSqrt15 / 30;   case 7: return 2.0 / 9 + kSqrt15 / 15;   default: return 5.0 / 36.0;
+        }
+    }
+    CTD_HD static constexpr double b(int j) {
+        if (SC != SC_IRK || j >= S) return 0.0;
+        if (S == 1) return 1.0;
+        if (S == 2) return 0.5;
+        return j == 1 ? 4.0 / 9.0 : 5.0 / 18.0;
+    }
+    CTD_HD static constexpr double c(int j) {
+        if (SC != SC_IRK || j >= S) return 0.0;
+        if (S == 1) return 0.5;
+        if (S == 2) return j == 0 ? 0.5 - kSqrt3 / 6 : 0.5 + kSqrt3 / 6;
+        return j == 0 ? 0.5 - 0.1 * kSqrt15 : (j == 1 ? 0.5 : 0.5 + 0.1 * kSqrt15);
+    }
+};
+template <class P, int SC, int S> inline const char* static_layout_mismatch(const Layout& L) {
+    using SL = StaticLayout<P, SC, S>;
+    if (L.sc != SC) return "sc";
+    if (L.s != SL::s) return "s";
+    if (L.n != SL::n) return "n";
+    if (L.m != SL::m) return "m";
+    if (L.nv != SL::nv) return "nv";
+    if (L.p != SL::p) return "p";
+    if (L.bc != SL::bc) return "bc";
+    if (L.cu != SL::cu(L.stagewise != 0)) return "cu";
+    if (L.blk != SL::blk(L.stagewise != 0)) return "blk";
+    if (L.eqs != SL::eqs) return "eqs";
+    if (L.cb != SL::cb) return "cb";
+    for (int j = 0; j < 3; ++j) {
+        for (int l = 0; l < 3; ++l)
+            if (!(L.a[3 * j + l] == SL::a(j, l))) return "a";
+        if (!(L.b[j] == SL::b(j))) return "b";
+        if (!(L.c[j] == SL::c(j))) return "c";
+    }
+    return nullptr;
+}
+template <class P, int SC, int S, bool LEAN> struct LV {
+    using SL = StaticLayout<P, SC, S>;
+    CTD_HD static int cu(const KParams& kp) { if constexpr (LEAN) return kp.L.stagewise ? SL::cu(true) : SL::cu(false); else return kp.L.cu; }
+    CTD_HD static int blk(const KParams& kp) { if constexpr (LEAN) return kp.L.stagewise ? SL::blk(true) : SL::blk(false); else return kp.L.blk; }
+    CTD_HD static int cb(const KParams& kp) { if constexpr (LEAN) return SL::cb; else return kp.L.cb; }
+    CTD_HD static int eqs(const KParams& kp) { if constexpr (LEAN) return SL::eqs; else return kp.L.eqs; }
+    CTD_HD static uint32_t div_cb(const KParams& kp, uint32_t x) { if constexpr (LEAN) return x / (uint32_t)SL::cb; else return fast_div(x, kp.div_cb); }
+    CTD_HD static double a(const KParams& kp, int j, int l) { if constexpr (LEAN) return SL::a(j, l); else return kp.L.a[3 * j + l]; }
+    CTD_HD static double b(const KParams& kp, int j) { if constexpr (LEAN) return SL::b(j); else return kp.L.b[j]; }
+    CTD_HD static double a_pick(const KParams& kp, int j, int l) {
+        if constexpr (LEAN) { const double t[3] = {SL::a(0, l), SL::a(S > 1 ? 1 : 0, l), SL::a(S > 2 ? 2 : 0, l)}; return butcher_pick<S>(t, j, 1, 0); }
+        else return butcher_a<S>(kp.L, j, l);
+    }
+    CTD_HD static double c_pick(const KParams& kp, int j) {
+        if constexpr (LEAN) { const double t[3] = {SL::c(0), SL::c(S > 1 ? 1 : 0), SL::c(S > 2 ? 2 : 0)}; return butcher_pick<S>(t, j, 1, 0); }
+        else return butcher_c<S>(kp.L, j);
+    }
+};
+
 CTD_HD void load_codes(const KParams& kp, const BlockCtx& cx, int tid, int nthr) {
     if (!codes_staged(kp)) return;
     uint32_t* dst = const_cast<uint32_t*>(cx.codes);
@@ -236,7 +324,7 @@
     for (int e = tid; e < nvc; e += nthr) dst[kp.Lseg + e] = kp.vtmpl[e];
 }
 
-template <class P, int SC, int S, bool LOAD_V = true>
+template <class P, int SC, int S, bool LOAD_V = true, bool LEAN = false>
 CTD_HD void phase_load(const KParams& kp, const BlockCtx& cx, const double* __restrict__ xu, int tid, int nthr) {
     const Layout& L = kp.L;
     if (cx.is_edge) {
@@ -246,7 +334,7 @@
             int64_t g = kp.edge_steps[k] * L.blk + o;
             if (o >= L.blk + L.n + L.m)
                 g = (kp.edge_steps[k] >= 1 ? kp.edge_steps[k] - 1 : 0) * (int64_t)L.blk + L.n + (o - (L.blk + L.n + L.m));
-            cx.in[e] = (g < L.v_off) ? (cx.halo ? xnear(kp.near, xu, g) : xu)[g] : 0.0;
+            cx.in[e] = (g < L.v_off) ? ((!LEAN && cx.halo) ? xnear(kp.near, xu, g) : xu)[g] : 0.0;
         }
         for (int e = tid; e <= 2 * cx.nslots; e += nthr)
             cx.tau[e] = (e == 2 * cx.nslots) ? tau_global(kp, L.N) : tau_global(kp, kp.edge_steps[e >> 1] + (e & 1));
@@ -260,7 +348,7 @@
         auto at = [&](int e) -> double& { const int eo = eo0 + e; return cx.in[eo + (int)fast_div((uint32_t)eo, kp.div_blk) * padw]; };
         const bool codes = LOAD_V && codes_staged(kp);
         const int nvc = kp.L.nv * kp.vr;
-        if (cx.halo) {
+        if (!LEAN && cx.halo) {
             for (int e = tid; e < cnt; e += nthr) at(e) = xnear(kp.near, xu, g0 + e)[g0 + e];
             if (LOAD_V && tid < kMaxNV) cx.v[tid] = (tid < P::NV) ? xu[L.v_off + tid] : 0.0;
             if (codes) {
@@ -329,43 +417,44 @@
     for (int e = tid + nthr; e <= cx.nslots + 1; e += nthr) cx.tau[e] = tau_global(kp, cx.lo + e);
 }
 
-template <class P> CTD_HD void fill_const_coefs(const KParams& kp, double* C) {
+template <class P, int SC = SC_TRAPEZE, int S = 1, bool LEAN = false> CTD_HD void fill_const_coefs(const KParams& kp, double* C) {
 #pragma unroll
     for (int e = 0; e < kNC; ++e) C[e] = 0.0;
     C[C_ONE] = 1.0; C[C_NEG1] = -1.0;
 #pragma unroll
-    for (int j = 0; j < 3; ++j) C[C_B + j] = kp.L.b[j];
-}
-
-template <class P, int SC, int S>
+    for (int j = 0; j < 3; ++j) C[C_B + j] = LV<P, SC, S, LEAN>::b(kp, j);
+}
+
+template <class P, int SC, int S, bool LEAN = false>
 CTD_HD void fin_lead(const KParams& kp, const BlockCtx& cx, int k, int row = -1) {
+    using V = LV<P, SC, S, LEAN>;
     constexpr int n = P::NX, nv = P::NV;
     const Layout& L = kp.L;
     constexpr RecLayout R = RL<P, SC, S>::R;
-    const int64_t i = slot_index(kp, cx, k);
+    const int64_t i = slot_index<LEAN>(kp, cx, k);
     double* rec = cx.rec + k * R.stride;
     double* C = rec + R.oC;
-    if (row <= 0) fill_const_coefs<P>(kp, C);
+    if (row <= 0) fill_const_coefs<P, SC, S, LEAN>(kp, C);
     if (i < 0 || i >= L.N) return;
-    const double tau0 = slot_tau(kp, cx, k, 0), tau1 = slot_tau(kp, cx, k, 1);
+    const double tau0 = slot_tau<LEAN>(kp, cx, k, 0), tau1 = slot_tau<LEAN>(kp, cx, k, 1);
     const double h = time_of<P>(kp, cx.v, tau1) - time_of<P>(kp, cx.v, tau0);
     if (SC == SC_IRK) {
-        const double* base = slot_base(kp, cx, k);
-        const double* nxt = slot_next(kp, cx, k);
-        const double* K = base + n + L.cu;
+        const double* base = slot_base<LEAN>(kp, cx, k);
+        const double* nxt = slot_next<LEAN>(kp, cx, k);
+        const double* K = base + n + V::cu(kp);
         if (row <= 0) {
 #pragma unroll
             for (int j = 0; j < S; ++j) {
 #pragma unroll
-                for (int l = 0; l < S; ++l) C[C_HA + 3 * j + l] = -(h * L.a[3 * j + l]);
-                C[C_HB + j] = -(h * L.b[j]);
+                for (int l = 0; l < S; ++l) C[C_HA + 3 * j + l] = -(h * V::a(kp, j, l));
+                C[C_HB + j] = -(h * V::b(kp, j));
             }
         }
         if (row >= 0) {
             const int r = row;
-            double sumbk = L.b[0] * K[r];
-#pragma unroll
-            for (int j = 1; j < S; ++j) sumbk = sumbk + L.b[j] * K[j * n + r];
+            double sumbk = V::b(kp, 0) * K[r];
+#pragma unroll
+            for (int j = 1; j < S; ++j) sumbk = sumbk + V::b(kp, j) * K[j * n + r];
             rec[R.oR + r] = nxt[r] - (base[r] + h * sumbk);
 #pragma unroll
             for (int kk = 0; kk < nv; ++kk) {
@@ -376,9 +465,9 @@
         }
 #pragma unroll
         for (int r = 0; r < n; ++r) {
-            double sumbk = L.b[0] * K[r];
-#pragma unroll
-            for (int j = 1; j < S; ++j) sumbk = sumbk + L.b[j] * K[j * n + r];
+            double sumbk = V::b(kp, 0) * K[r];
+#pragma unroll
+            for (int j = 1; j < S; ++j) sumbk = sumbk + V::b(kp, j) * K[j * n + r];
             rec[R.oR + r] = nxt[r] - (base[r] + h * sumbk);
 #pragma unroll
             for (int kk = 0; kk < nv; ++kk) {
@@ -394,19 +483,20 @@
     }
 }
 
-template <class P, int SC, int S>
+template <class P, int SC, int S, bool LEAN = false>
 CTD_HD void fin_stage(const KParams& kp, const BlockCtx& cx, int k, int j, double* ev, int r0 = 0, int rstep = 1) {
+    using V = LV<P, SC, S, LEAN>;
     constexpr int n = P::NX, nv = P::NV;
     auto mine = [&](int r) { return rstep == 1 || (r % rstep) == r0; };
     constexpr bool FREE = Dirs<P>::FREE;
     const Layout& L = kp.L;
     constexpr RecLayout R = RL<P, SC, S>::R;
-    const int64_t i = slot_index(kp, cx, k);
+    const int64_t i = slot_index<LEAN>(kp, cx, k);
     if (i < 0) return;
     if (SC == SC_TRAPEZE ? (i > L.N) : (i >= L.N)) return;
     double* rec = cx.rec + k * R.stride;
-    const double* base = slot_base(kp, cx, k);
-    const double tau0 = slot_tau(kp, cx, k, 0), tau1 = slot_tau(kp, cx, k, 1);
+    const double* base = slot_base<LEAN>(kp, cx, k);
+    const double tau0 = slot_tau<LEAN>(kp, cx, k, 0), tau1 = slot_tau<LEAN>(kp, cx, k, 1);
     double dti[nv > 0 ? nv : 1], dh[nv > 0 ? nv : 1];
 #pragma unroll
     for (int kk = 0; kk < nv; ++kk) {
@@ -414,7 +504,7 @@
         dh[kk] = FREE ? dtime_of<P>(tau1, kk) - dti[kk] : 0.0;
     }
     if (SC == SC_IRK) {
-        const double* K = base + n + L.cu;
+        const double* K = base + n + V::cu(kp);
 #pragma unroll
         for (int r = 0; r < n; ++r)
             if (mine(r)) rec[R.oR + n + j * n + r] = K[j * n + r] - ev[R.of + r];
@@ -425,10 +515,10 @@
             for (int c = 0; c < n; ++c) {
                 double acc = 0.0;
 #pragma unroll
-                for (int l = 0; l < S; ++l) acc = acc + (dh[kk] * butcher_a<S>(L, j, l)) * K[l * n + c];
+                for (int l = 0; l < S; ++l) acc = acc + (dh[kk] * V::a_pick(kp, j, l)) * K[l * n + c];
                 dx[c] = acc;
             }
-            const double dtij = dti[kk] + butcher_c<S>(L, j) * dh[kk];
+            const double dtij = dti[kk] + V::c_pick(kp, j) * dh[kk];
 #pragma unroll
             for (int r = 0; r < n; ++r) {
                 if (!mine(r)) continue;
@@ -444,7 +534,7 @@
         }
     } else if (SC == SC_MIDPOINT) {
         const double h = (time_of<P>(kp, cx.v, tau1) - time_of<P>(kp, cx.v, tau0)) / (double)S;
-        const double* nxt = slot_next(kp, cx, k);
+        const double* nxt = slot_next<LEAN>(kp, cx, k);
 #pragma unroll
         for (int r = 0; r < n; ++r) {
             if (!mine(r)) continue;
@@ -547,30 +637,31 @@
     }
 }
 
-template <class P, int S> CTD_HD void node_control(const KParams& kp, const double* base, double* u) {
+template <class P, int S, int SC = SC_IRK, bool LEAN = false> CTD_HD void node_control(const KParams& kp, const double* base, double* u) {
     const Layout& L = kp.L;
+    using V = LV<P, SC, S, LEAN>;
     if (L.stagewise) {
 #pragma unroll
-        for (int c = 0; c < P::NU; ++c) u[c] = L.b[0] * base[P::NX + c];
+        for (int c = 0; c < P::NU; ++c) u[c] = V::b(kp, 0) * base[P::NX + c];
 #pragma unroll
         for (int j = 1; j < S; ++j)
 #pragma unroll
-            for (int c = 0; c < P::NU; ++c) u[c] = u[c] + L.b[j] * base[P::NX + j * P::NU + c];
+            for (int c = 0; c < P::NU; ++c) u[c] = u[c] + V::b(kp, j) * base[P::NX + j * P::NU + c];
     } else {
 #pragma unroll
         for (int c = 0; c < P::NU; ++c) u[c] = base[P::NX + c];
     }
 }
 
-template <class P, int S> CTD_HD void path_control(const KParams& kp, const BlockCtx& cx, int k, int64_t i, double* u) {
+template <class P, int S, int SC = SC_IRK, bool LEAN = false> CTD_HD void path_control(const KParams& kp, const BlockCtx& cx, int k, int64_t i, double* u) {
     const Layout& L = kp.L;
-    const double* base = slot_base(kp, cx, k);
+    const double* base = slot_base<LEAN>(kp, cx, k);
     if (L.euler == 2 && i >= 1 && (cx.is_edge || k >= 1)) {
-        const double* up = (cx.is_edge && !cx.direct) ? base + L.blk + P::NX + P::NU : slot_prev(kp, cx, k) + P::NX;
+        const double* up = (cx.is_edge && !cx.direct) ? base + L.blk + P::NX + P::NU : slot_prev<LEAN>(kp, cx, k) + P::NX;
 #pragma unroll
         for (int c = 0; c < P::NU; ++c) u[c] = up[c];
     } else {
-        node_control<P, S>(kp, base, u);
+        node_control<P, S, SC, LEAN>(kp, base, u);
     }
 }
 
@@ -665,16 +756,17 @@
     }
 }
 
-template <class P, int SC, int S, bool SPLIT = false>
+template <class P, int SC, int S, bool SPLIT = false, bool LEAN = false>
 CTD_HD void eval_dynamics(const KParams& kp, const BlockCtx& cx, int k, int j, int q, double* ev) {
+    using V = LV<P, SC, S, LEAN>;
     constexpr int n = P::NX, m = P::NU, nv = P::NV;
     const Layout& L = kp.L;
     constexpr RecLayout R = RL<P, SC, S>::R;
-    const int64_t i = slot_index(kp, cx, k);
+    const int64_t i = slot_index<LEAN>(kp, cx, k);
     if (i < 0) return;
     if (SC == SC_TRAPEZE ? (i > L.N) : (i >= L.N)) return;
-    const double* base = slot_base(kp, cx, k);
-    const double ti = time_of<P>(kp, cx.v, slot_tau(kp, cx, k, 0));
+    const double* base = slot_base<LEAN>(kp, cx, k);
+    const double ti = time_of<P>(kp, cx.v, slot_tau<LEAN>(kp, cx, k, 0));
     double xv[n > 0 ? n : 1], uv[m > 0 ? m : 1];
     double t;
     if (SC == SC_TRAPEZE) {
@@ -684,8 +776,8 @@
 #pragma unroll
         for (int c = 0; c < m; ++c) uv[c] = base[n + c];
     } else if (SC == SC_MIDPOINT) {
-        const double tip1 = time_of<P>(kp, cx.v, slot_tau(kp, cx, k, 1));
-        const double* nxt = slot_next(kp, cx, k);
+        const double tip1 = time_of<P>(kp, cx.v, slot_tau<LEAN>(kp, cx, k, 1));
+        const double* nxt = slot_next<LEAN>(kp, cx, k);
         if (L.euler == 0) {
             t = 0.5 * (ti + tip1);
 #pragma unroll
@@ -698,14 +790,14 @@
 #pragma unroll
         for (int c = 0; c < m; ++c) uv[c] = base[n + c];
     } else {
-        const double h = time_of<P>(kp, cx.v, slot_tau(kp, cx, k, 1)) - ti;
-        t = ti + butcher_c<S>(L, j) * h;
-        const double* K = base + n + L.cu;
+        const double h = time_of<P>(kp, cx.v, slot_tau<LEAN>(kp, cx, k, 1)) - ti;
+        t = ti + V::c_pick(kp, j) * h;
+        const double* K = base + n + V::cu(kp);
 #pragma unroll
         for (int c = 0; c < n; ++c) {
             double x = base[c];
 #pragma unroll
-            for (int l = 0; l < S; ++l) x = x + h * butcher_a<S>(L, j, l) * K[l * n + c];
+            for (int l = 0; l < S; ++l) x = x + h * V::a_pick(kp, j, l) * K[l * n + c];
             xv[c] = x;
         }
         const double* U = base + n + (L.stagewise ? j * m : 0);
@@ -820,22 +912,22 @@
     }
 }
 
-template <class P, int SC, int S, bool REG = false>
+template <class P, int SC, int S, bool REG = false, bool LEAN = false>
 CTD_HD void eval_step_path(const KParams& kp, const BlockCtx& cx, int k, int q) {
     constexpr int n = P::NX, m = P::NU, np = P::NPATH;
     constexpr RecLayout R = RL<P, SC, S>::R;
     constexpr int eqs = RL<P, SC, S>::cb - P::NPATH;
     const Layout& L = kp.L;
-    const int64_t i = slot_index(kp, cx, k);
+    const int64_t i = slot_index<LEAN>(kp, cx, k);
     if (i < 0 || i >= L.N) return;
-    const double* base = slot_base(kp, cx, k);
+    const double* base = slot_base<LEAN>(kp, cx, k);
     double uv[m > 0 ? m : 1];
-    path_control<P, S>(kp, cx, k, i, uv);
+    path_control<P, S, SC, LEAN>(kp, cx, k, i, uv);
     double xv[n > 0 ? n : 1];
 #pragma unroll
     for (int c = 0; c < n; ++c) xv[c] = base[c];
     double* rec = cx.rec + k * R.stride;
-    const double tau = slot_tau(kp, cx, k, 0);
+    const double tau = slot_tau<LEAN>(kp, cx, k, 0);
     if constexpr (REG) {
         double lrec[R.oR + eqs + (np > 0 ? np : 1)];
 #pragma unroll
@@ -847,7 +939,7 @@
 #pragma unroll
         for (int r = 0; r < np; ++r) rec[R.oR + eqs + r] = lrec[R.oR + eqs + r];
     } else {
-        eval_path<P, SC, S>(kp, rec, time_of<P>(kp, cx.v, tau), xv, uv, cx.v, q, R.oR + L.eqs);
+        eval_path<P, SC, S>(kp, rec, time_of<P>(kp, cx.v, tau), xv, uv, cx.v, q, R.oR + LV<P, SC, S, LEAN>::eqs(kp));
         if (Dirs<P>::FUSED) fin_path<P, SC, S>(kp, rec, tau);
     }
 }
@@ -1016,7 +1108,7 @@
     return (((r_dyn + r_path) << lgT) + 63) & ~63;
 }
 
-template <class P, int SC, int S, bool REG = false, int NB = 1, bool B = false>
+template <class P, int SC, int S, bool REG = false, int NB = 1, bool B = false, bool LEAN = false>
 CTD_HD void phase_eval(const KParams& kp, const BlockCtx& cx, int tid, int nthr, const EmitPreT<NB>* epre = nullptr,
                        const BatchLd bl = BatchLd{}) {
     constexpr bool FUSED = Dirs<P>::FUSED;
@@ -1039,19 +1131,19 @@
                     if (k < ns) {
                         double* ev = cx.rec + k * R.stride + R.oEval + j * R.eval_sz;
                         if constexpr (parts) {
-                            eval_dynamics<P, SC, S, true>(kp, cx, k, j, wave, ev);
-                            fin_stage<P, SC, S>(kp, cx, k, j, ev, wave, NP);
+                            eval_dynamics<P, SC, S, true, LEAN>(kp, cx, k, j, wave, ev);
+                            fin_stage<P, SC, S, LEAN>(kp, cx, k, j, ev, wave, NP);
                         } else {
-                            eval_dynamics<P, SC, S>(kp, cx, k, j, 0, ev);
-                            fin_stage<P, SC, S>(kp, cx, k, j, ev);
+                            eval_dynamics<P, SC, S, false, LEAN>(kp, cx, k, j, 0, ev);
+                            fin_stage<P, SC, S, LEAN>(kp, cx, k, j, ev);
                         }
                     }
                 } else if (l >= 32) {
                     const int a = wave - (parts ? 0 : 1), t = l - 32;
-                    if (a == 0) { if (t < r_path * 8 && (t & 7) < ns) eval_step_path<P, SC, S>(kp, cx, t & 7, t >> 3); }
+                    if (a == 0) { if (t < r_path * 8 && (t & 7) < ns) eval_step_path<P, SC, S, false, LEAN>(kp, cx, t & 7, t >> 3); }
                     else if (a == 1) {
                         if (t < n_fp) eval_final_path<P, SC, S>(kp, cx, t);
-                        else if (t >= 8 && t < 10) fill_const_coefs<P>(kp, cx.rec + (t == 8 ? kp.edge_fp : kp.edge_b) * R.stride + R.oC);
+                        else if (t >= 8 && t < 10) fill_const_coefs<P, SC, S, LEAN>(kp, cx.rec + (t == 8 ? kp.edge_fp : kp.edge_b) * R.stride + R.oC);
                     } else if (a == 2) { if (t < n_b) eval_boundary<P, SC, S>(kp, cx, t); }
                 }
                 for (int k = tid; k < ns + 2; k += nthr) cx.rec[k * R.stride] = 1.0;
@@ -1093,13 +1185,13 @@
             if (kind == 0) {
                 const int j = role / Dirs<P>::NCH_DYN, q = role % Dirs<P>::NCH_DYN;
                 double* ev = cx.rec + k * R.stride + R.oEval + j * R.eval_sz;
-                eval_dynamics<P, SC, S>(kp, cx, k, j, q, ev);
-                if (FUSED) fin_stage<P, SC, S>(kp, cx, k, j, ev);
-            } else if (kind == 1) eval_step_path<P, SC, S>(kp, cx, k, role);
-            else if (kind == 2) fin_lead<P, SC, S>(kp, cx, k);
+                eval_dynamics<P, SC, S, false, LEAN>(kp, cx, k, j, q, ev);
+                if (FUSED) fin_stage<P, SC, S, LEAN>(kp, cx, k, j, ev);
+            } else if (kind == 1) eval_step_path<P, SC, S, false, LEAN>(kp, cx, k, role);
+            else if (kind == 2) fin_lead<P, SC, S, LEAN>(kp, cx, k);
             else if (kind == 3) eval_final_path<P, SC, S>(kp, cx, role);
             else if (kind == 4) eval_boundary<P, SC, S>(kp, cx, role);
-            else fill_const_coefs<P>(kp, cx.rec + (role == 0 ? kp.edge_fp : kp.edge_b) * R.stride + R.oC);
+            else fill_const_coefs<P, SC, S, LEAN>(kp, cx.rec + (role == 0 ? kp.edge_fp : kp.edge_b) * R.stride + R.oC);
         }
         for (int k = tid; k < ns + 2; k += nthr) cx.rec[k * R.stride] = 1.0;
         return;
@@ -1112,25 +1204,25 @@
             const int wave = tid >> 6, l = tid & 63;
             const bool fold = fin_folded<P, SC, S>(cx);
             auto fin_path_slot = [&](int k) {
-                const int64_t i = slot_index(kp, cx, k);
-                if (i >= 0 && i < kp.L.N) fin_path<P, SC, S>(kp, cx.rec + k * R.stride, slot_tau(kp, cx, k, 0));
+                const int64_t i = slot_index<LEAN>(kp, cx, k);
+                if (i >= 0 && i < kp.L.N) fin_path<P, SC, S>(kp, cx.rec + k * R.stride, slot_tau<LEAN>(kp, cx, k, 0));
             };
             if (wave < NP) {
 #if !defined(CTD_ABL) || CTD_ABL != 2
                 if (l < nd) {
                     const int j = l / ns, k = l - j * ns;
                     double* ev = cx.rec + k * R.stride + R.oEval + j * R.eval_sz;
-                    eval_dynamics<P, SC, S, true>(kp, cx, k, j, wave, ev);
-                    if (fold) fin_stage<P, SC, S>(kp, cx, k, j, ev, wave, NP);
+                    eval_dynamics<P, SC, S, true, LEAN>(kp, cx, k, j, wave, ev);
+                    if (fold) fin_stage<P, SC, S, LEAN>(kp, cx, k, j, ev, wave, NP);
                 }
 #endif
                 CTD_SUB(kp, 2);
 #if !defined(CTD_ABL) || CTD_ABL != 3
                 if (SC == SC_IRK) {
                     if (l < nd)
-                        for (int t = l * NP + wave; t < ns * P::NX; t += nd * NP) fin_lead<P, SC, S>(kp, cx, t / P::NX, t % P::NX);
+                        for (int t = l * NP + wave; t < ns * P::NX; t += nd * NP) fin_lead<P, SC, S, LEAN>(kp, cx, t / P::NX, t % P::NX);
                 } else if (l < ns && wave == NP - 1) {
-                    fin_lead<P, SC, S>(kp, cx, l);
+                    fin_lead<P, SC, S, LEAN>(kp, cx, l);
                 }
 #endif
                 CTD_SUB(kp, 3);
@@ -1138,7 +1230,7 @@
                 if (l >= nd && l < nd + ns) {
                     constexpr int PW = NP > 1 ? 1 : 0;
                     if (SymPath<P>::value ? wave == PW : wave < r_path) {
-                        eval_step_path<P, SC, S>(kp, cx, l - nd, SymPath<P>::value ? 0 : wave);
+                        eval_step_path<P, SC, S, false, LEAN>(kp, cx, l - nd, SymPath<P>::value ? 0 : wave);
                         if (fold) fin_path_slot(l - nd);
                     }
                 }
@@ -1152,7 +1244,7 @@
     }
     const int lg = ns <= 1 ? 0 : 32 - __builtin_clz((unsigned)(ns - 1));
     const int mask = (1 << lg) - 1;
-    if constexpr (FUSED && SC == SC_IRK) {
+    if constexpr (FUSED && SC == SC_IRK && !LEAN) {
         if (kp.n_early > 0 && epre != nullptr) {
             int lgT = 0;
             while ((1 << lgT) < kp.T) ++lgT;
@@ -1168,25 +1260,25 @@
                             double evr[R.eval_sz];
 #pragma unroll
                             for (int e = 0; e < R.eval_sz; ++e) evr[e] = 0.0;
-                            eval_dynamics<P, SC, S>(kp, cx, k, j, q, evr);
-                            fin_stage<P, SC, S>(kp, cx, k, j, evr);
-                            const int64_t i = slot_index(kp, cx, k);
+                            eval_dynamics<P, SC, S, false, LEAN>(kp, cx, k, j, q, evr);
+                            fin_stage<P, SC, S, LEAN>(kp, cx, k, j, evr);
+                            const int64_t i = slot_index<LEAN>(kp, cx, k);
                             if (i >= 0 && i < kp.L.N) {
 #pragma unroll
                                 for (int e = 0; e < R.eval_sz; ++e) ev[e] = evr[e];
                             }
                         } else {
-                            eval_dynamics<P, SC, S>(kp, cx, k, j, q, ev);
-                            fin_stage<P, SC, S>(kp, cx, k, j, ev);
+                            eval_dynamics<P, SC, S, false, LEAN>(kp, cx, k, j, q, ev);
+                            fin_stage<P, SC, S, LEAN>(kp, cx, k, j, ev);
                         }
                     } else {
-                        eval_step_path<P, SC, S, REG>(kp, cx, k, role - r_dyn);
+                        eval_step_path<P, SC, S, REG, LEAN>(kp, cx, k, role - r_dyn);
                     }
                 }
             } else if ((tid >> 6) == (leadbase >> 6)) {
                 const int k = tid - leadbase;
                 if (k < ns) {
-                    fin_lead<P, SC, S>(kp, cx, k);
+                    fin_lead<P, SC, S, LEAN>(kp, cx, k);
                     cx.rec[k * R.stride] = 1.0;
                 }
 #if defined(__HIP_DEVICE_COMPILE__)
@@ -1213,29 +1305,29 @@
 #pragma unroll
                 for (int e = 0; e < R.eval_sz; ++e) evr[e] = 0.0;
                 CTD_SUB(kp, 1);
-                eval_dynamics<P, SC, S>(kp, cx, k, j, q, evr);
+                eval_dynamics<P, SC, S, false, LEAN>(kp, cx, k, j, q, evr);
                 CTD_SUB(kp, 2);
-                fin_stage<P, SC, S>(kp, cx, k, j, evr);
+                fin_stage<P, SC, S, LEAN>(kp, cx, k, j, evr);
                 CTD_SUB(kp, 3);
-                const int64_t i = slot_index(kp, cx, k);
+                const int64_t i = slot_index<LEAN>(kp, cx, k);
                 if (i >= 0 && i < kp.L.N) {
 #pragma unroll
                     for (int e = 0; e < R.eval_sz; ++e) ev[e] = evr[e];
                 }
                 CTD_SUB(kp, 4);
             } else {
-                eval_dynamics<P, SC, S>(kp, cx, k, j, q, ev);
-                if (FUSED || (fold_g && q == 0)) fin_stage<P, SC, S>(kp, cx, k, j, ev);
+                eval_dynamics<P, SC, S, false, LEAN>(kp, cx, k, j, q, ev);
+                if (FUSED || (fold_g && q == 0)) fin_stage<P, SC, S, LEAN>(kp, cx, k, j, ev);
             }
         } else if (role < r_dyn + r_path) {
-            eval_step_path<P, SC, S, REG>(kp, cx, k, role - r_dyn);
+            eval_step_path<P, SC, S, REG, LEAN>(kp, cx, k, role - r_dyn);
             if (fold_g) {
-                const int64_t i = slot_index(kp, cx, k);
-                if (i >= 0 && i < kp.L.N) fin_path<P, SC, S>(kp, cx.rec + k * R.stride, slot_tau(kp, cx, k, 0));
+                const int64_t i = slot_index<LEAN>(kp, cx, k);
+                if (i >= 0 && i < kp.L.N) fin_path<P, SC, S>(kp, cx.rec + k * R.stride, slot_tau<LEAN>(kp, cx, k, 0));
             }
         } else {
             CTD_SUB(kp, 1);
-            fin_lead<P, SC, S>(kp, cx, k);
+            fin_lead<P, SC, S, LEAN>(kp, cx, k);
             CTD_SUB(kp, 4);
         }
     }
@@ -1312,7 +1404,7 @@
 #endif
     static constexpr int value = (seg + 255) / 256 < 1 ? 1 : ((seg + 255) / 256 > CTD_PRE_MAX ? CTD_PRE_MAX : (seg + 255) / 256);
 };
-template <class P, int NB = 1>
+template <class P, int NB = 1, bool LEAN = false>
 CTD_HD EmitPreT<NB> emit_prefetch(const KParams& kp, const BlockCtx& cx, int tid, int nthr) {
     EmitPreT<NB> pre;
     pre.b = 0u;
@@ -1335,7 +1427,7 @@
     }
     const int Ls = kp.Lseg;
     pre.kpos = 0; pre.eb = 0u; pre.ek = 0;
-    if (kp.n_early > 0) {
+    if (!LEAN && kp.n_early > 0) {
         const int q = tid - (int)fast_div((uint32_t)tid, kp.div_late) * kp.n_late;
         pre.kpos = kp.pos[q];
         pre.b = kp.tmpl[pre.kpos];
@@ -1368,7 +1460,7 @@
     return pre;
 }
 
-template <class P, int SC, int S, int NB = 1, bool B = false>
+template <class P, int SC, int S, int NB = 1, bool B = false, bool LEAN = false>
 CTD_HD void phase_emit_impl(const KParams& kp, const BlockCtx& cx, int tid, int nthr, const EmitPreT<NB> pre_v, const bool hp,
                             const BatchLd bl = BatchLd{}) {
     const Layout& L = kp.L;
@@ -1403,14 +1495,15 @@
     CTD_SUBE(kp, 0);
     const int stride = R.stride;
     if (kp.c) {
-        const int cb = L.cb;
+        using V = LV<P, SC, S, LEAN>;
+        const int cb = V::cb(kp);
         double* out = out_c<B>(kp, bl) + cx.a * (int64_t)cb;
-        const int par = (int)fast_div((uint32_t)nthr, kp.div_cb);
+        const int par = (int)V::div_cb(kp, (uint32_t)nthr);
         if (par >= 1) {
             if (tid < par * cb) {
-                const int g = (int)fast_div((uint32_t)tid, kp.div_cb), r = tid - g * cb;
+                const int g = (int)V::div_cb(kp, (uint32_t)tid), r = tid - g * cb;
                 const double* src = cx.rec + (slot0 + g) * stride + R.oR + r;
-                if (r >= kp.c_early)
+                if (LEAN || r >= kp.c_early)
                     for (int s = g; s < nsteps; s += par, src += par * stride) emit_store(&out[s * cb + r], *src, kp.wt_store);
             }
         } else {
@@ -1430,7 +1523,7 @@
             const int nreg = (int)(rb - ra);
             double* out = out_vals<B>(kp, bl) + kp.seg_base + (ra - kp.reg_first) * (int64_t)Ls;
             const int sl0 = (int)(ra - cx.lo);
-            const bool late_only = kp.n_early > 0;
+            const bool late_only = !LEAN && kp.n_early > 0;
             const int Lw = late_only ? kp.n_late : Ls;
             const int par = (int)fast_div((uint32_t)nthr, late_only ? kp.div_late : kp.div_Lseg);
             if (par >= 1) {
@@ -1510,7 +1603,7 @@
                     const double* pc = cx.rec + (slot0 + g) * stride + R.oC + code_ci(code);
                     const double* pd = cx.rec + (slot0 + g) * stride + code_di(code);
                     const int adv = par * stride;
-                    if (k >= kp.vr_early)
+                    if (LEAN || k >= kp.vr_early)
                         for (int s = g; s < nsteps; s += par, pc += adv, pd += adv) emit_store(&out[s * vr + k], (*pc) * (*pd), kp.wt_store);
                 }
             } else {
@@ -1525,11 +1618,11 @@
     }
     CTD_SUBE(kp, 3);
 }
-template <class P, int SC, int S, int NB = 1, bool B = false>
+template <class P, int SC, int S, int NB = 1, bool B = false, bool LEAN = false>
 CTD_HD void phase_emit(const KParams& kp, const BlockCtx& cx, int tid, int nthr, const EmitPreT<NB>* pre = nullptr,
                        const BatchLd bl = BatchLd{}) {
-    if (pre != nullptr) phase_emit_impl<P, SC, S, NB, B>(kp, cx, tid, nthr, *pre, pre->have != 0, bl);
-    else phase_emit_impl<P, SC, S, NB, B>(kp, cx, tid, nthr, EmitPreT<NB>{}, false, bl);
+    if (pre != nullptr) phase_emit_impl<P, SC, S, NB, B, LEAN>(kp, cx, tid, nthr, *pre, pre->have != 0, bl);
+    else phase_emit_impl<P, SC, S, NB, B, LEAN>(kp, cx, tid, nthr, EmitPreT<NB>{}, false, bl);
 }
 
 }
diff --git a/ctdirect.jl_amd/csrc/ctd_kernels.hpp b/ctdirect.jl_amd/csrc/ctd_kernels.hpp
--- a/ctdirect.jl_amd/csrc/ctd_kernels.hpp
+++ b/ctdirect.jl_amd/csrc/ctd_kernels.hpp
@@ -27,9 +27,18 @@
     }
 }
 
-template <int S>
+template <int S, bool LEAN = false>
 __device__ __forceinline__ void ctd_pin_kernargs(const KParams& kp, const double* xu) {
 #if defined(__HIP_DEVICE_COMPILE__)
+    if constexpr (LEAN) {
+        asm volatile("" ::"s"(kp.has_edge), "s"(kp.ntiles), "s"(kp.T), "s"(kp.HL), "s"(kp.HH), "s"(kp.step_begin),
+                     "s"(kp.step_end), "s"(kp.L.N), "s"(kp.L.v_off), "s"(kp.L.stagewise), "s"(kp.L.euler), "s"(kp.tau), "s"(kp.L.t0),
+                     "s"(kp.L.tf), "s"(xu), "s"(blockDim.x));
+        asm volatile("" ::"s"(kp.tmpl), "s"(kp.vtmpl), "s"(kp.Lseg), "s"(kp.vr), "s"(kp.div_Lseg.M), "s"(kp.div_vr.M),
+                     "s"(kp.div_Lseg.d), "s"(kp.div_vr.d), "s"(kp.seg_base), "s"(kp.reg_first), "s"(kp.reg_last),
+                     "s"(kp.vcol_base[0]), "s"(kp.c), "s"(kp.vals));
+        return;
+    }
     asm volatile("" ::"s"(kp.has_edge), "s"(kp.ntiles), "s"(kp.T), "s"(kp.HL), "s"(kp.HH), "s"(kp.step_begin),
                  "s"(kp.step_end), "s"(kp.L.blk), "s"(kp.L.N), "s"(kp.L.v_off), "s"(kp.L.cu), "s"(kp.L.stagewise), "s"(kp.L.nv),
                  "s"(kp.L.cb), "s"(kp.L.eqs), "s"(kp.L.euler), "s"(kp.tau), "s"(kp.L.t0), "s"(kp.L.tf), "s"(xu), "s"(blockDim.x));
@@ -42,33 +51,39 @@
 #endif
 }
 
+template <bool LEAN = false>
 __device__ __forceinline__ void ctd_pin_emit_kernargs(const KParams& kp) {
 #if defined(__HIP_DEVICE_COMPILE__)
-    asm volatile("" ::"s"(kp.c), "s"(kp.vals), "s"(kp.L.cb), "s"(kp.Lseg), "s"(kp.vr), "s"(kp.div_cb.M), "s"(kp.div_Lseg.M), "s"(kp.div_vr.M),
-                 "s"(kp.div_cb.d), "s"(kp.div_Lseg.d), "s"(kp.div_vr.d), "s"(kp.seg_base), "s"(kp.reg_first), "s"(kp.reg_last),
-                 "s"(kp.vcol_base[0]), "s"(kp.n_early), "s"(kp.c_early), "s"(kp.vr_early), "s"(kp.n_late), "s"(kp.div_late.M), "s"(kp.div_late.d));
+    if constexpr (LEAN)
+        asm volatile("" ::"s"(kp.c), "s"(kp.vals), "s"(kp.Lseg), "s"(kp.vr), "s"(kp.div_Lseg.M), "s"(kp.div_vr.M),
+                     "s"(kp.div_Lseg.d), "s"(kp.div_vr.d), "s"(kp.seg_base), "s"(kp.reg_first), "s"(kp.reg_last),
+                     "s"(kp.vcol_base[0]));
+    else
+        asm volatile("" ::"s"(kp.c), "s"(kp.vals), "s"(kp.L.cb), "s"(kp.Lseg), "s"(kp.vr), "s"(kp.div_cb.M), "s"(kp.div_Lseg.M), "s"(kp.div_vr.M),
+                     "s"(kp.div_cb.d), "s"(kp.div_Lseg.d), "s"(kp.div_vr.d), "s"(kp.seg_base), "s"(kp.reg_first), "s"(kp.reg_last),
+                     "s"(kp.vcol_base[0]), "s"(kp.n_early), "s"(kp.c_early), "s"(kp.vr_early), "s"(kp.n_late), "s"(kp.div_late.M), "s"(kp.div_late.d));
 #endif
 }
 
-template <class P, int SC, int S, bool DBG, bool B = false>
+template <class P, int SC, int S, bool DBG, bool B = false, bool LEAN = false>
 __device__ __forceinline__ void cons_jac_body(const KParams& kp, const double* __restrict__ xu, int block, double* ctd_lds,
                                               const BatchLd bl = BatchLd{}) {
     if constexpr (B) xu += batch_member() * bl.ldx;
-    ctd_pin_kernargs<SC == SC_IRK ? S : 0>(kp, xu);
+    ctd_pin_kernargs<SC == SC_IRK ? S : 0, LEAN>(kp, xu);
     ctd_stamp<DBG>(kp, 0);
     if (DBG && kp.debug_stop == 1) return;
     const int tid = (int)threadIdx.x, nthr = (int)blockDim.x;
     if constexpr (DirectTile<P, SC>::value) {
-        const BlockCtx cx = make_direct_ctx(kp, block, ctd_lds, xu);
-        const EmitPre pre = emit_prefetch<P>(kp, cx, tid, nthr);
+        const BlockCtx cx = make_direct_ctx<LEAN>(kp, block, ctd_lds, xu, LV<P, SC, S, LEAN>::blk(kp), LEAN ? P::NV : -1);
+        const EmitPre pre = emit_prefetch<P, 1, LEAN>(kp, cx, tid, nthr);
         ctd_stamp<DBG>(kp, 1);
-        phase_eval<P, SC, S, RegEval<P, SC, S>::value, 1, B>(kp, cx, tid, nthr, &pre, bl);
-        ctd_pin_emit_kernargs(kp);
+        phase_eval<P, SC, S, RegEval<P, SC, S>::value, 1, B, LEAN>(kp, cx, tid, nthr, &pre, bl);
+        ctd_pin_emit_kernargs<LEAN>(kp);
         __syncthreads();
         ctd_stamp<DBG>(kp, 2);
         ctd_stamp<DBG>(kp, 3);
         if (DBG && kp.debug_stop >= 2 && kp.debug_stop <= 4) return;
-        phase_emit<P, SC, S, 1, B>(kp, cx, tid, nthr, &pre, bl);
+        phase_emit<P, SC, S, 1, B, LEAN>(kp, cx, tid, nthr, &pre, bl);
         ctd_stamp<DBG>(kp, 4);
         if (DBG && kp.stamps) {
             __builtin_amdgcn_s_waitcnt(0);
@@ -77,19 +92,19 @@
         }
         return;
     }
-    BlockCtx cx = make_ctx(kp, block, ctd_lds);
+    BlockCtx cx = make_ctx<LEAN>(kp, block, ctd_lds);
     constexpr int NB = EmitN<P, SC, S>::value;
     EmitPreT<NB> pre = {};
     const bool use_pre = !cx.is_edge && !codes_staged(kp);
-    if (use_pre) pre = emit_prefetch<P, NB>(kp, cx, tid, nthr);
-    phase_load<P, SC, S>(kp, cx, xu, tid, nthr);
+    if (use_pre) pre = emit_prefetch<P, NB, LEAN>(kp, cx, tid, nthr);
+    phase_load<P, SC, S, true, LEAN>(kp, cx, xu, tid, nthr);
     const int nblk = kp.ntiles + kp.has_edge;
     for (;;) {
         __syncthreads();
         ctd_stamp<DBG>(kp, 1);
         if (DBG && kp.debug_stop == 2) return;
-        phase_eval<P, SC, S, false, 1, B>(kp, cx, tid, nthr, nullptr, bl);
-        ctd_pin_emit_kernargs(kp);
+        phase_eval<P, SC, S, false, 1, B, LEAN>(kp, cx, tid, nthr, nullptr, bl);
+        ctd_pin_emit_kernargs<LEAN>(kp);
         __syncthreads();
         ctd_stamp<DBG>(kp, 2);
         if (DBG && kp.debug_stop == 3) return;
@@ -108,10 +123,10 @@
         BlockCtx nx = cx;
         TileIn tin{0.0, 0.0, 0.0};
         if (more) {
-            nx = make_ctx(kp, block, ctd_lds);
+            nx = make_ctx<LEAN>(kp, block, ctd_lds);
             tin = load_issue<P>(kp, nx, xu, tid, nthr);
         }
-        phase_emit_impl<P, SC, S, NB, B>(kp, cx, tid, nthr, pre, use_pre, bl);
+        phase_emit_impl<P, SC, S, NB, B, LEAN>(kp, cx, tid, nthr, pre, use_pre, bl);
         ctd_stamp<DBG>(kp, 4);
         if (!more) break;
         load_commit<P, SC, S>(kp, nx, xu, tin, tid, nthr);
@@ -128,10 +143,10 @@
     static constexpr int value = (P::NX <= 12 && !(SC == SC_MIDPOINT && S > 1)) ? 4 : 1;
 };
 
-template <class P, int SC, int S, bool DBG>
+template <class P, int SC, int S, bool DBG, bool LEAN = false>
 __global__ void __launch_bounds__(P::MAXB, (MinWaves<P, SC, S>::value)) cons_jac_kernel(const KParams kp, const double* __restrict__ xu) {
     extern __shared__ double ctd_lds[];
-    cons_jac_body<P, SC, S, DBG>(kp, xu, (int)blockIdx.x, ctd_lds);
+    cons_jac_body<P, SC, S, DBG, false, LEAN>(kp, xu, (int)blockIdx.x, ctd_lds);
 }
 template <class P, int SC, int S>
 __global__ void __launch_bounds__(P::MAXB, (MinWaves<P, SC, S>::value)) cons_jac_batch_kernel(const KParams kp, const double* __restrict__ xu,
@@ -601,30 +616,38 @@
 #endif
 
 #if !defined(__HIPCC_RTC__)
-template <class P, int SC, int S, bool DBG>
+template <class P, int SC, int S, bool DBG, bool LEAN>
 hipError_t launch_variant_dbg(const KParams& kp, const double* xu, int grid, int block, size_t lds_bytes, hipStream_t st,
                               hipEvent_t e0, hipEvent_t e1) {
     if (lds_bytes > 64 * 1024) {
-        hipError_t e = hipFuncSetAttribute((const void*)cons_jac_kernel<P, SC, S, DBG>, hipFuncAttributeMaxDynamicSharedMemorySize,
+        hipError_t e = hipFuncSetAttribute((const void*)cons_jac_kernel<P, SC, S, DBG, LEAN>, hipFuncAttributeMaxDynamicSharedMemorySize,
                                            (int)lds_bytes);
         if (e != hipSuccess) return e;
     }
-    if (e0 || e1) hipExtLaunchKernelGGL((cons_jac_kernel<P, SC, S, DBG>), dim3(grid), dim3(block), lds_bytes, st, e0, e1, 0, kp, xu);
-    else cons_jac_kernel<P, SC, S, DBG><<<grid, block, lds_bytes, st>>>(kp, xu);
+    if (e0 || e1) hipExtLaunchKernelGGL((cons_jac_kernel<P, SC, S, DBG, LEAN>), dim3(grid), dim3(block), lds_bytes, st, e0, e1, 0, kp, xu);
+    else cons_jac_kernel<P, SC, S, DBG, LEAN><<<grid, block, lds_bytes, st>>>(kp, xu);
     return hipGetLastError();
 }
 template <class P, int SC, int S>
 hipError_t launch_variant(const KParams& kp, const double* xu, int grid, int block, size_t lds_bytes, hipStream_t st,
-                          hipEvent_t e0, hipEvent_t e1) {
-    if (kp.stamps || kp.debug_stop) return launch_variant_dbg<P, SC, S, true>(kp, xu, grid, block, lds_bytes, st, e0, e1);
-    return launch_variant_dbg<P, SC, S, false>(kp, xu, grid, block, lds_bytes, st, e0, e1);
+                          hipEvent_t e0, hipEvent_t e1, int lean_ok) {
+    const bool dbg = kp.stamps || kp.debug_stop;
+    constexpr bool kHasLean = DirectTile<P, SC>::value || SC == SC_IRK;
+    if constexpr (kHasLean) {
+        if (lean_ok && kp.halo == nullptr && kp.n_early == 0) {
+            if (dbg) return launch_variant_dbg<P, SC, S, true, true>(kp, xu, grid, block, lds_bytes, st, e0, e1);
+            return launch_variant_dbg<P, SC, S, false, true>(kp, xu, grid, block, lds_bytes, st, e0, e1);
+        }
+    }
+    if (dbg) return launch_variant_dbg<P, SC, S, true, false>(kp, xu, grid, block, lds_bytes, st, e0, e1);
+    return launch_variant_dbg<P, SC, S, false, false>(kp, xu, grid, block, lds_bytes, st, e0, e1);
 }
 
 template <class P>
 hipError_t launch_cons_jac(const KParams& kp, const double* xu, int grid, int block, size_t lds_bytes, hipStream_t st,
-                           hipEvent_t e0, hipEvent_t e1) {
+                           hipEvent_t e0, hipEvent_t e1, int lean_ok) {
     hipError_t e = hipErrorInvalidValue;
-    for_scheme<true>(kp.L, [&](auto t) { e = launch_variant<P, t.sc, t.s>(kp, xu, grid, block, lds_bytes, st, e0, e1); });
+    for_scheme<true>(kp.L, [&](auto t) { e = launch_variant<P, t.sc, t.s>(kp, xu, grid, block, lds_bytes, st, e0, e1, lean_ok); });
     return e;
 }
 
@@ -673,14 +696,14 @@
 
 #define CTD_INSTANTIATE_LAUNCHERS(P)                                                                                       \
     template hipError_t launch_cons_jac<P>(const KParams&, const double*, int, int, size_t, hipStream_t, hipEvent_t, \
-                                           hipEvent_t);                                                                    \
+                                           hipEvent_t, int);                                                                 \
     template hipError_t launch_cons_jac_batch<P>(const KParams&, const double*, const BatchLd&, int, int, size_t, hipStream_t, int); \
     template hipError_t launch_obj<P>(const ObjParams&, const double*, int, int, hipStream_t, int);                  \
     template int occupancy_cons_jac<P>(const KParams&, int, size_t);                                                 \
     template hipError_t launch_grad<P>(const GradParams&, const double*, int, hipStream_t, int);
 #define CTD_EXTERN_LAUNCHERS(P)                                                                                            \
     extern template hipError_t launch_cons_jac<P>(const KParams&, const double*, int, int, size_t, hipStream_t,      \
-                                                  hipEvent_t, hipEvent_t);                                                 \
+                                                  hipEvent_t, hipEvent_t, int);                                              \
     extern template hipError_t launch_cons_jac_batch<P>(const KParams&, const double*, const BatchLd&, int, int, size_t, hipStream_t, \
                                                         int);                                                                      \
     extern template hipError_t launch_obj<P>(const ObjParams&, const double*, int, int, hipStream_t, int);          \
```
